# mobiusml/gemlite

Hardware: AMD Instinct MI355X
Metric: HBM GB/s (algorithmic bytes) vs roofline at M=1 [value], TFLOP/s vs bf16 MFMA roofline at M=256 [roofline.m256]; A16W4 gs=128 4096x4096 (higher is better)
Workload: dtype fp16; 1 GPU; A16W4 gs=128 4096x4096 M=1 fp16; step = 64 distinct layers (cache-cold rotation), hipGraph replay; replicas=1

## Files before the change

gemlite_amd/_hip.py:

```python
from __future__ import annotations

import ctypes as C
import os
import threading

import torch

_HERE = os.path.dirname(os.path.abspath(__file__))
LIB_PATH = os.path.join(_HERE, "csrc", "libgemlite_hip.so")
ABI_VERSION = 1

OK, ERR_BAD_ARGUMENT, ERR_UNSUPPORTED, ERR_BAD_SHAPE, ERR_WORKSPACE, ERR_LAUNCH, ERR_NO_DEVICE, ERR_NO_FUSED_QUANT = 0, -1, -2, -3, -4, -5, -6, -7


class ForwardArgs(C.Structure):

    _fields_ = [
        ("struct_size", C.c_uint32),
        ("matmul_type", C.c_int32),
        ("x", C.c_void_p),
        ("w_q", C.c_void_p),
        ("scales", C.c_void_p),
        ("zeros", C.c_void_p),
        ("scales_x", C.c_void_p),
        ("out", C.c_void_p),
        ("workspace", C.c_void_p),
        ("workspace_bytes", C.c_uint64),
        ("M", C.c_int64),
        ("N", C.c_int64),
        ("K", C.c_int64),
        ("W_nbits", C.c_int32),
        ("group_size", C.c_int32),
        ("unpack_mask", C.c_int32),
        ("elements_per_sample", C.c_int32),
        ("w_pack_bits", C.c_int32),
        ("w_dtype", C.c_int32),
        ("input_dtype", C.c_int32),
        ("output_dtype", C.c_int32),
        ("acc_dtype", C.c_int32),
        ("meta_dtype", C.c_int32),
        ("zeros_dtype", C.c_int32),
        ("channel_scale_mode", C.c_int32),
        ("W_group_mode", C.c_int32),
        ("zero_is_scalar", C.c_int32),
        ("data_contiguous", C.c_int32),
        ("type_id", C.c_int32),
        ("stride_xm", C.c_int64),
        ("stride_xk", C.c_int64),
        ("stride_wk", C.c_int64),
        ("stride_wn", C.c_int64),
        ("stride_om", C.c_int64),
        ("stride_on", C.c_int64),
        ("stride_meta_g", C.c_int64),
        ("stride_meta_n", C.c_int64),
        ("stride_sx_m", C.c_int64),
        ("tuning", C.c_int32 * 4),
    ]


class ForwardExt(C.Structure):

    _fields_ = [
        ("struct_size", C.c_uint32),
        ("bias_dtype", C.c_int32),
        ("bias", C.c_void_p),
    ]


class QuantizeArgs(C.Structure):

    _fields_ = [
        ("struct_size", C.c_uint32),
        ("w_dtype", C.c_int32),
        ("w", C.c_void_p),
        ("N", C.c_int64),
        ("K", C.c_int64),
        ("ld_w", C.c_int64),
        ("W_nbits", C.c_int32),
        ("group_size", C.c_int32),
        ("pack_bits", C.c_int32),
        ("meta_dtype", C.c_int32),
        ("q_out", C.c_void_p),
        ("ld_q", C.c_int64),
        ("scales", C.c_void_p),
        ("zeros", C.c_void_p),
        ("stride_meta_g", C.c_int64),
        ("stride_meta_n", C.c_int64),
        ("fold_zeros", C.c_int32),
        ("reserved", C.c_int32),
    ]


class QuantizeHqqArgs(C.Structure):

    _fields_ = [
        ("struct_size", C.c_uint32),
        ("iters", C.c_int32),
        ("q", QuantizeArgs),
        ("lp_norm", C.c_float),
        ("beta", C.c_float),
        ("kappa", C.c_float),
        ("reserved", C.c_int32),
    ]


class QuantizeMxArgs(C.Structure):

    _fields_ = [
        ("struct_size", C.c_uint32),
        ("w_dtype", C.c_int32),
        ("w", C.c_void_p),
        ("N", C.c_int64),
        ("K", C.c_int64),
        ("ld_w", C.c_int64),
        ("format", C.c_int32),
        ("pack_nibbles", C.c_int32),
        ("q_out", C.c_void_p),
        ("ld_q", C.c_int64),
        ("scales", C.c_void_p),
        ("stride_scale_g", C.c_int64),
        ("stride_scale_n", C.c_int64),
        ("reserved", C.c_int64),
    ]


class QuantizeRowsArgs(C.Structure):

    _fields_ = [
        ("struct_size", C.c_uint32),
        ("w_dtype", C.c_int32),
        ("w", C.c_void_p),
        ("N", C.c_int64),
        ("K", C.c_int64),
        ("ld_w", C.c_int64),
        ("format", C.c_int32),
        ("scale_rule", C.c_int32),
        ("q_out", C.c_void_p),
        ("ld_q", C.c_int64),
        ("scales", C.c_void_p),
        ("stride_s", C.c_int64),
        ("scale_dtype", C.c_int32),
        ("reserved", C.c_int32),
    ]


QUANT_ROWS_WAVE_MAX_K = 1024
QUANT_ROWS_RESIDENT_MAX_K = 16384


class DequantizeArgs(C.Structure):

    _fields_ = [
        ("struct_size", C.c_uint32),
        ("out_dtype", C.c_int32),
        ("w_q", C.c_void_p),
        ("scales", C.c_void_p),
        ("zeros", C.c_void_p),
        ("out", C.c_void_p),
        ("N", C.c_int64),
        ("K", C.c_int64),
        ("stride_wk", C.c_int64),
        ("stride_wn", C.c_int64),
        ("stride_meta_g", C.c_int64),
        ("stride_meta_n", C.c_int64),
        ("ld_out", C.c_int64),
        ("W_nbits", C.c_int32),
        ("group_size", C.c_int32),
        ("elements_per_sample", C.c_int32),
        ("w_pack_bits", C.c_int32),
        ("w_dtype", C.c_int32),
        ("input_dtype", C.c_int32),
        ("meta_dtype", C.c_int32),
        ("zeros_dtype", C.c_int32),
        ("zero_is_scalar", C.c_int32),
        ("W_group_mode", C.c_int32),
        ("channel_scale_mode", C.c_int32),
        ("post_scale", C.c_float),
        ("reserved", C.c_int64),
    ]


BIAS_NOT_ADDED = 1

_lib = None
_lib_lock = threading.Lock()


class GemliteHipError(RuntimeError):
    pass


def load():
    global _lib
    if _lib is not None:
        return _lib
    with _lib_lock:
        if _lib is not None:
            return _lib
        if not os.path.exists(LIB_PATH):
            raise GemliteHipError(
                f"{LIB_PATH} not found: build it with `python -c 'import __graft_entry__ as g; g.build()'` "
                "or `make -C gemlite_amd/csrc`.  gemlite_amd has no non-HIP fallback."
            )
        lib = C.CDLL(LIB_PATH)
        lib.gemlite_hip_abi_version.restype = C.c_int
        lib.gemlite_hip_build_info.restype = C.c_char_p
        lib.gemlite_hip_status_string.restype = C.c_char_p
        lib.gemlite_hip_status_string.argtypes = [C.c_int]
        lib.gemlite_hip_last_hip_error.restype = C.c_int
        for name in ("gemlite_hip_query", "gemlite_hip_forward"):
            getattr(lib, name).restype = C.c_int
        lib.gemlite_hip_query.argtypes = [C.POINTER(ForwardArgs)]
        lib.gemlite_hip_forward.argtypes = [C.POINTER(ForwardArgs), C.c_void_p]
        lib.gemlite_hip_workspace_bytes.restype = C.c_uint64
        lib.gemlite_hip_workspace_bytes.argtypes = [C.POINTER(ForwardArgs)]
        lib.gemlite_hip_kernel_name.restype = C.c_char_p
        lib.gemlite_hip_kernel_name.argtypes = [C.POINTER(ForwardArgs)]
        lib.gemlite_hip_set_profile_events.restype = None
        lib.gemlite_hip_set_profile_events.argtypes = [C.c_void_p, C.c_void_p]
        lib.gemlite_hip_launch_noop.restype = C.c_int
        lib.gemlite_hip_launch_noop.argtypes = [C.c_int32, C.c_int32, C.c_void_p]
        lib.gemlite_hip_capture_group_max.restype = C.c_int
        lib.gemlite_hip_capture_group_max.argtypes = []
        lib.gemlite_hip_capture_group_stats.restype = None
        lib.gemlite_hip_capture_group_stats.argtypes = [C.POINTER(C.c_uint64), C.POINTER(C.c_uint64)]
        lib.gemlite_hip_capture_group_compatible.restype = C.c_int
        lib.gemlite_hip_capture_group_compatible.argtypes = [C.POINTER(ForwardArgs), C.POINTER(ForwardArgs)]
        lib.gemlite_hip_capture_group_grid_y.restype = C.c_int
        lib.gemlite_hip_capture_group_grid_y.argtypes = [C.c_int32, C.c_int32]
        lib.gemlite_hip_capture_group_wave_split.restype = None
        lib.gemlite_hip_capture_group_wave_split.argtypes = [C.c_int32, C.c_int32, C.POINTER(C.c_int32 * 3)]
        lib.gemlite_hip_capture_group_last_form.restype = C.c_int
        lib.gemlite_hip_capture_group_last_form.argtypes = []
        lib.gemlite_hip_capture_group_geometry.restype = C.c_int
        lib.gemlite_hip_capture_group_geometry.argtypes = [C.c_int32, C.c_int32, C.c_int32, C.c_int32, C.c_int32, C.POINTER(C.c_int32 * 4)]
        lib.gemlite_hip_capture_group_tile_of.restype = C.c_int
        lib.gemlite_hip_capture_group_tile_of.argtypes = [C.c_int32, C.c_int32, C.c_int32, C.c_int32]
        lib.gemlite_hip_capture_group_form.restype = C.c_int
        lib.gemlite_hip_capture_group_form.argtypes = [C.c_int32, C.c_int32, C.c_int64]
        lib.gemlite_hip_capture_group_shared_x_lds_bytes.restype = C.c_int64
        lib.gemlite_hip_capture_group_shared_x_lds_bytes.argtypes = [C.c_int64]
        lib.gemlite_hip_forward_ex.restype = C.c_int
        lib.gemlite_hip_forward_ex.argtypes = [C.POINTER(ForwardArgs), C.POINTER(ForwardExt), C.c_void_p]
        lib.gemlite_hip_bias_fused.restype = C.c_int
        lib.gemlite_hip_bias_fused.argtypes = [C.POINTER(ForwardArgs), C.POINTER(ForwardExt)]
        lib.gemlite_hip_kernel_name_ex.restype = C.c_char_p
        lib.gemlite_hip_kernel_name_ex.argtypes = [C.POINTER(ForwardArgs), C.POINTER(ForwardExt)]
        lib.gemlite_hip_capture_group_compatible_ex.restype = C.c_int
        lib.gemlite_hip_capture_group_compatible_ex.argtypes = [C.POINTER(ForwardArgs), C.POINTER(ForwardExt), C.POINTER(ForwardArgs),
                                                                 C.POINTER(ForwardExt)]
        lib.gemlite_hip_scale_activations_per_token.restype = C.c_int
        lib.gemlite_hip_scale_activations_per_token.argtypes = [
            C.c_void_p, C.c_void_p, C.c_void_p, C.c_int64, C.c_int64, C.c_int64, C.c_int32, C.c_int32, C.c_void_p]
        for name in ("gemlite_hip_scale_activations_mxfp8", "gemlite_hip_scale_activations_mxfp4",
                     "gemlite_hip_scale_activations_nvfp4"):
            getattr(lib, name).restype = C.c_int
            getattr(lib, name).argtypes = [C.c_void_p, C.c_void_p, C.c_void_p, C.c_int64, C.c_int64, C.c_int64, C.c_int32,
                                           C.c_void_p]
        lib.gemlite_hip_pack_over_cols.restype = C.c_int
        lib.gemlite_hip_pack_over_cols.argtypes = [
            C.c_void_p, C.c_void_p, C.c_int64, C.c_int64, C.c_int64, C.c_int32, C.c_int32, C.c_void_p]
        lib.gemlite_hip_unpack_over_cols.restype = C.c_int
        lib.gemlite_hip_unpack_over_cols.argtypes = [
            C.c_void_p, C.c_void_p, C.c_int64, C.c_int64, C.c_int32, C.c_int32, C.c_void_p]
        lib.gemlite_hip_quantize_groups.restype = C.c_int
        lib.gemlite_hip_quantize_groups.argtypes = [C.POINTER(QuantizeArgs), C.c_void_p]
        lib.gemlite_hip_quantize_groups_hqq.restype = C.c_int
        lib.gemlite_hip_quantize_groups_hqq.argtypes = [C.POINTER(QuantizeHqqArgs), C.c_void_p]
        lib.gemlite_hip_quantize_mx.restype = C.c_int
        lib.gemlite_hip_quantize_mx.argtypes = [C.POINTER(QuantizeMxArgs), C.c_void_p]
        lib.gemlite_hip_quantize_rows.restype = C.c_int
        lib.gemlite_hip_quantize_rows.argtypes = [C.POINTER(QuantizeRowsArgs), C.c_void_p]
        lib.gemlite_hip_dequantize.restype = C.c_int
        lib.gemlite_hip_dequantize.argtypes = [C.POINTER(DequantizeArgs), C.c_void_p]
        if lib.gemlite_hip_abi_version() != ABI_VERSION:
            raise GemliteHipError("libgemlite_hip.so ABI version mismatch; rebuild it")
        _lib = lib
    return _lib


EXPORTED_SYMBOLS = (
    "gemlite_hip_abi_version", "gemlite_hip_build_info", "gemlite_hip_status_string", "gemlite_hip_last_hip_error",
    "gemlite_hip_query", "gemlite_hip_workspace_bytes", "gemlite_hip_forward", "gemlite_hip_kernel_name",
    "gemlite_hip_set_profile_events", "gemlite_hip_launch_noop", "gemlite_hip_scale_activations_per_token",
    "gemlite_hip_scale_activations_mxfp8", "gemlite_hip_scale_activations_mxfp4", "gemlite_hip_scale_activations_nvfp4",
    "gemlite_hip_pack_over_cols",
    "gemlite_hip_unpack_over_cols",
    "gemlite_hip_capture_group_max", "gemlite_hip_capture_group_stats", "gemlite_hip_capture_group_compatible",
    "gemlite_hip_capture_group_grid_y", "gemlite_hip_capture_group_wave_split",
    "gemlite_hip_capture_group_last_form", "gemlite_hip_capture_group_form", "gemlite_hip_capture_group_shared_x_lds_bytes",
    "gemlite_hip_capture_group_geometry", "gemlite_hip_capture_group_tile_of",
    "gemlite_hip_forward_ex", "gemlite_hip_bias_fused", "gemlite_hip_kernel_name_ex", "gemlite_hip_capture_group_compatible_ex",
    "gemlite_hip_quantize_groups", "gemlite_hip_quantize_mx", "gemlite_hip_dequantize", "gemlite_hip_quantize_groups_hqq",
    "gemlite_hip_quantize_rows",
)


def forward_ext(bias_ptr: int, bias_dtype: int) -> ForwardExt:
    e = ForwardExt()
    e.struct_size = C.sizeof(ForwardExt)
    e.bias_dtype = int(bias_dtype)
    e.bias = bias_ptr
    return e


def status_string(code: int) -> str:
    return load().gemlite_hip_status_string(int(code)).decode()


def raise_for_status(code: int, what: str):
    if code == OK:
        return
    msg = f"{what}: {status_string(code)}"
    if code == ERR_UNSUPPORTED or code == ERR_BAD_SHAPE:
        raise NotImplementedError(msg)
    if code == ERR_LAUNCH:
        msg += f" (hipError_t={load().gemlite_hip_last_hip_error()})"
    err = GemliteHipError(msg)
    err.status = code
    raise err


def require_gpu_tensor(t: torch.Tensor, name: str):
    if not t.is_cuda:
        raise GemliteHipError(
            f"gemlite_amd: `{name}` lives on {t.device}; the HIP backend only runs on an MI355X device "
            "(there is deliberately no CPU fallback)")


_workspaces: dict = {}
_ws_lock = threading.Lock()


def workspace(device: torch.device, stream_handle: int, nbytes: int) -> torch.Tensor:
    key = (device.index if device.index is not None else torch.cuda.current_device(), int(stream_handle))
    ws = _workspaces.get(key)
    if ws is None or ws.numel() < nbytes:
        with _ws_lock:
            ws = _workspaces.get(key)
            if ws is None or ws.numel() < nbytes:
                size = max(int(nbytes), 1 << 20)
                size = 1 << (size - 1).bit_length()
                ws = torch.zeros(size, dtype=torch.uint8, device=device)
                _workspaces[key] = ws
    return ws


class on_device:
    __slots__ = ("_guard",)

    def __init__(self, device: torch.device):
        idx = device.index
        self._guard = torch.cuda.device(idx) if (idx is not None and idx != torch.cuda.current_device()) else None

    def __enter__(self):
        if self._guard is not None:
            self._guard.__enter__()
        return self

    def __exit__(self, *exc):
        if self._guard is not None:
            self._guard.__exit__(*exc)
        return False


def current_stream_handle(device: torch.device) -> int:
    return torch.cuda.current_stream(device).cuda_stream
```

gemlite_amd/csrc/api.hip:

```cpp
#include <hip/hip_runtime.h>
#include <stdio.h>
#include <string.h>

#include <atomic>
#include <mutex>
#include <set>
#include <string>

#include "gl_common.h"
#include "gl_coopquant.h"

namespace gl {
bool plan_gemv_wn(const gemlite_hip_forward_args& a, WnParams& p, LaunchPlan& lp);
bool plan_gemv_mfma(const gemlite_hip_forward_args& a, WnParams& p, LaunchPlan& lp);
bool plan_gemv_a8wn(const gemlite_hip_forward_args& a, WnParams& p, LaunchPlan& lp, bool fq = false);
bool plan_a8wn_rows(const gemlite_hip_forward_args& a, WnParams& p, LaunchPlan& lp);
bool plan_gemm_wn_stream(const gemlite_hip_forward_args& a, WnParams& p, LaunchPlan& lp);
bool plan_gemm_wn_direct(const gemlite_hip_forward_args& a, WnParams& p, LaunchPlan& lp);
bool plan_gemm_wn_rows(const gemlite_hip_forward_args& a, WnParams& p, LaunchPlan& lp);
bool plan_gemm_a8w8(const gemlite_hip_forward_args& a, LaunchPlan& lp);
bool plan_gemm_a8w8_mma(const gemlite_hip_forward_args& a, GenericParams& g, LaunchPlan& lp);
bool plan_a8w8_rows(const gemlite_hip_forward_args& a, LaunchPlan& lp, bool fq = false);
bool plan_a16w8_rows(const gemlite_hip_forward_args& a, LaunchPlan& lp);
bool a16w8_rows_lds_pays(const gemlite_hip_forward_args& a);
bool plan_gemm_a8w8_sq(const gemlite_hip_forward_args& a, GenericParams& g, LaunchPlan& lp);
bool plan_gemm_a8w8_sq128(const gemlite_hip_forward_args& a, GenericParams& g, LaunchPlan& lp);
bool plan_gemm_wn_tiled(const gemlite_hip_forward_args& a, WnParams& p, LaunchPlan& lp);
bool plan_gemm_wn_mma(const gemlite_hip_forward_args& a, WnParams& p, LaunchPlan& lp);
bool plan_gemm_mx_mma(const gemlite_hip_forward_args& a, GenericParams& g, LaunchPlan& lp);
bool plan_gemm_mx_sq(const gemlite_hip_forward_args& a, GenericParams& g, LaunchPlan& lp);
bool plan_gemm_wn_mma_mx(const gemlite_hip_forward_args& a, WnParams& p, LaunchPlan& lp, int mode = 0);
bool plan_mx_gemv(const gemlite_hip_forward_args& a, GenericParams& g, LaunchPlan& lp);
bool plan_gemm_mx_tile(const gemlite_hip_forward_args& a, GenericParams& g, LaunchPlan& lp);
const void* mx_generic_kernel_fn();
const void* act_quant_mx_kernel_fn(int mode);
bool plan_mx_rows(const gemlite_hip_forward_args& a, GenericParams& g, LaunchPlan& lp, bool any_m = false, bool fq = false);
bool plan_nvfp4_rows(const gemlite_hip_forward_args& a, GenericParams& g, LaunchPlan& lp, bool fq = false);
const void* nvfp4_expand_f16_kernel_fn();
const void* generic_kernel_fn();
const void* kmajor_kernel_fn(int mb);
const void* kmajor_w8a16_kernel_fn(int mb);
const void* kmajor_fused_quant_kernel_fn(int qdt);
const void* a8w8_decode_kernel_fn(int qdt, bool fused);
const void* a16w8_decode_kernel_fn(int x_dt, int w_dt);
const void* act_quant_kernel_fn();
const void* act_quant_vec_kernel_fn(int in_dt, int out_dt, int64_t K, int64_t stride_xm, const void* x, const void* y);
const void* pack_kernel_fn();
const void* pack32_kernel_fn();
const void* unpack_kernel_fn();
const void* quantize_groups_kernel_fn(bool onepass);
const void* quantize_hqq_kernel_fn(bool onepass);
const void* quantize_mx_kernel_fn(int format);
const void* quantize_rows_kernel_fn(int format, int64_t K);
const void* dequantize_words_kernel_fn(int nbits);
const void* dequantize_rows_kernel_fn(int fmt);
const void* dequantize_any_kernel_fn();
int capture_group_limit();
void capture_group_stats(uint64_t* seen, uint64_t* joined);
bool capture_group_compatible(const gemlite_hip_forward_args& a, const LaunchPlan& la, const gemlite_hip_forward_args& b, const LaunchPlan& lb);
bool capture_group_try_join(const gemlite_hip_forward_args& a, const LaunchPlan& lp, hipStream_t st, int resident, int dev);
bool capture_group_shared_x_enabled();
int capture_group_last_form();
Decode3TilesWanted capture_group_tiles_wanted(int tiles, int members, int resident);
int ensure_lds(const void* fn, size_t lds, int dev);
void capture_group_note_launch(const gemlite_hip_forward_args& a, const LaunchPlan& lp, hipStream_t st);

}

using namespace gl;

const char* gl::pw_label(const char* name, int pack_bits) {
    if (pack_bits == 32) return name;
    static std::mutex mu;
    static std::set<std::string>* names = new std::set<std::string>();
    std::string s(name);
    s.insert(s.size() - 1, pack_bits == 8 ? ",b8" : ",b16");
    std::lock_guard<std::mutex> lock(mu);
    return names->insert(s).first->c_str();
}

const char* gl::bias_label(const char* name) {
    static std::mutex mu;
    static std::set<std::string>* names = new std::set<std::string>();
    std::string s(name);
    s.insert(s.size() - 1, ",bias");
    std::lock_guard<std::mutex> lock(mu);
    return names->insert(s).first->c_str();
}

static thread_local int tl_last_hip_error = 0;
static thread_local void* tl_evt_start = nullptr;
static thread_local void* tl_evt_stop = nullptr;

static int dtype_size(int dt) {
    switch (dt) {
        case GEMLITE_DT_FP32: case GEMLITE_DT_INT32: case GEMLITE_DT_UINT32: return 4;
        case GEMLITE_DT_FP16: case GEMLITE_DT_BF16: case GEMLITE_DT_INT16: case GEMLITE_DT_UINT16: return 2;
        case GEMLITE_DT_INT64: return 8;
        case GEMLITE_DT_FP8E4: case GEMLITE_DT_FP8E5: case GEMLITE_DT_INT8: case GEMLITE_DT_UINT8: return 1;
        default: return 0;
    }
}

enum Kind { K_NONE = 0, K_GEMV_WN, K_STREAM_WN, K_TILED_WN, K_KMAJOR, K_A8_MMA, K_A8_FQ, K_NV_MMA, K_GENERIC };

struct Resolved {
    Kind kind = K_NONE;
    LaunchPlan lp{};
    WnParams wn{};
    GenericParams gp{};
    int status = GEMLITE_OK;
    uint64_t nv_x16_bytes = 0;
};

static Epilogue make_epilogue(const gemlite_hip_forward_args& a) {
    Epilogue e{};
    e.out = a.out;
    e.scales_w = a.scales;
    e.scales_x = (const float*)a.scales_x;
    e.stride_om = a.stride_om;
    e.stride_on = a.stride_on;
    e.stride_sx_m = a.stride_sx_m;
    e.out_dt = a.output_dtype;
    e.meta_dt = a.meta_dtype;
    e.c_mode = a.channel_scale_mode;
    return e;
}

static bool is_mx_input(int dt);
static bool wants_fused_quant(const gemlite_hip_forward_args* a) {
    if (is_mx_input(a->type_id / 100)) return false;
    return a->M >= 1 && a->elements_per_sample == 1 && !a->scales_x &&
           (a->channel_scale_mode == 2 || a->channel_scale_mode == 3) && a->W_group_mode == 0 &&
           (a->input_dtype == GEMLITE_DT_FP16 || a->input_dtype == GEMLITE_DT_BF16) &&
           (a->w_dtype == GEMLITE_DT_INT8 || a->w_dtype == GEMLITE_DT_FP8E4 || a->w_dtype == GEMLITE_DT_FP8E5);
}

static int fused_quant_packed_dtype(const gemlite_hip_forward_args* a) {
    if (a->M != 1 || a->elements_per_sample <= 1 || a->scales_x) return 0;
    if (!(a->channel_scale_mode == 2 || a->channel_scale_mode == 3)) return 0;
    if (!(a->input_dtype == GEMLITE_DT_FP16 || a->input_dtype == GEMLITE_DT_BF16)) return 0;
    const int layer_dt = a->type_id / 100;
    return (layer_dt == GEMLITE_DT_FP8E4 || layer_dt == GEMLITE_DT_INT8) && a->type_id % 100 == a->W_nbits ? layer_dt : 0;
}

static bool is_mx_input(int dt);
static int fused_quant_mx_dtype(const gemlite_hip_forward_args* a) {
    if (a->M != 1 || a->scales_x || !(a->channel_scale_mode == 4 || a->channel_scale_mode == 2)) return 0;
    if (!(a->input_dtype == GEMLITE_DT_FP16 || a->input_dtype == GEMLITE_DT_BF16)) return 0;
    const int layer_dt = a->type_id / 100;
    if (a->channel_scale_mode == 2 && layer_dt != GEMLITE_DT_MXFP8) return 0;
    return (layer_dt == GEMLITE_DT_MXFP8 || layer_dt == GEMLITE_DT_MXFP4 || layer_dt == GEMLITE_DT_NVFP4) && a->type_id % 100 == a->W_nbits ? layer_dt : 0;
}

static bool is_mx_input(int dt) { return dt >= GEMLITE_DT_MXFP16 && dt <= GEMLITE_DT_NVFP4; }

static int validate_mx(const gemlite_hip_forward_args* a) {
    const bool nv = a->input_dtype == GEMLITE_DT_NVFP4;
    if (a->group_size != (nv ? 16 : 32)) return GEMLITE_ERR_UNSUPPORTED;
    if (a->K % 32 != 0) return GEMLITE_ERR_BAD_SHAPE;
    if (!a->scales) return GEMLITE_ERR_BAD_ARGUMENT;
    if (!(a->output_dtype == GEMLITE_DT_FP32 || a->output_dtype == GEMLITE_DT_FP16 || a->output_dtype == GEMLITE_DT_BF16))
        return GEMLITE_ERR_UNSUPPORTED;
    const bool w8 = a->W_nbits == 8 && a->elements_per_sample == 1 && a->w_dtype == GEMLITE_DT_FP8E4;
    const bool w4 = a->W_nbits == 4 && a->elements_per_sample == 2 && a->w_pack_bits == 8;
    if (!w8 && !w4) return GEMLITE_ERR_UNSUPPORTED;
    const bool x16 = a->input_dtype == GEMLITE_DT_MXFP16 || a->input_dtype == GEMLITE_DT_MXBF16;
    if ((a->input_dtype == GEMLITE_DT_MXFP4 || nv) && !w4) return GEMLITE_ERR_UNSUPPORTED;
    if (x16 ? a->channel_scale_mode != 0 : !(a->channel_scale_mode == 4 || (a->channel_scale_mode == 2 && !nv))) return GEMLITE_ERR_UNSUPPORTED;
    if (!x16 && !a->scales_x) return GEMLITE_ERR_BAD_ARGUMENT;
    if (a->stride_xk != 1) return GEMLITE_ERR_UNSUPPORTED;
    if (a->M > 65535 && a->M > 0x7FFFFFFF) return GEMLITE_ERR_BAD_SHAPE;
    return GEMLITE_OK;
}

static int validate(const gemlite_hip_forward_args* a) {
    if (!a || a->struct_size != sizeof(gemlite_hip_forward_args)) return GEMLITE_ERR_BAD_ARGUMENT;
    if (!a->x || !a->w_q || !a->out) return GEMLITE_ERR_BAD_ARGUMENT;
    if (a->M <= 0 || a->N <= 0 || a->K <= 0) return GEMLITE_ERR_BAD_ARGUMENT;
    if (a->M > 0x7FFFFFFF || a->N > 0x7FFFFFFF || a->K > 0x7FFFFFFF) return GEMLITE_ERR_BAD_SHAPE;
    if (is_mx_input(a->input_dtype)) return validate_mx(a);
    if (const int mxdt = fused_quant_mx_dtype(a)) {
        gemlite_hip_forward_args b = *a;
        b.input_dtype = mxdt;
        b.scales_x = (const void*)(uintptr_t)0x1000;
        return validate_mx(&b);
    }
    if (a->W_group_mode < 0 || a->W_group_mode > 4) return GEMLITE_ERR_UNSUPPORTED;
    if (a->channel_scale_mode < 0 || a->channel_scale_mode > 3) return GEMLITE_ERR_UNSUPPORTED;
    if (a->elements_per_sample < 1) return GEMLITE_ERR_BAD_ARGUMENT;
    if (a->K % a->elements_per_sample != 0) return GEMLITE_ERR_BAD_SHAPE;
    if (a->input_dtype == GEMLITE_DT_FP8E4NUZ || a->input_dtype == GEMLITE_DT_FP8E5NUZ) return GEMLITE_ERR_UNSUPPORTED;
    if (a->input_dtype > GEMLITE_DT_FP8E5NUZ) return GEMLITE_ERR_UNSUPPORTED;
    if (dtype_size(a->input_dtype) == 0) return GEMLITE_ERR_UNSUPPORTED;
    if (!(a->output_dtype == GEMLITE_DT_FP32 || a->output_dtype == GEMLITE_DT_FP16 || a->output_dtype == GEMLITE_DT_BF16))
        return GEMLITE_ERR_UNSUPPORTED;
    const bool need_s = a->W_group_mode >= 2 || a->channel_scale_mode == 1 || a->channel_scale_mode == 3;
    const bool need_z = a->W_group_mode == 1 || a->W_group_mode >= 3;
    if (need_s && !a->scales) return GEMLITE_ERR_BAD_ARGUMENT;
    if (need_z && !a->zeros) return GEMLITE_ERR_BAD_ARGUMENT;
    if ((a->channel_scale_mode == 2 || a->channel_scale_mode == 3) && !a->scales_x && !wants_fused_quant(a) && !fused_quant_packed_dtype(a)) return GEMLITE_ERR_BAD_ARGUMENT;
    if (a->elements_per_sample > 1) {
        if (a->w_pack_bits != 8 && a->w_pack_bits != 16 && a->w_pack_bits != 32 && a->w_pack_bits != 64)
            return GEMLITE_ERR_BAD_ARGUMENT;
        if (a->W_nbits * a->elements_per_sample != a->w_pack_bits) return GEMLITE_ERR_BAD_ARGUMENT;
    } else if (dtype_size(a->w_dtype) == 0) {
        return GEMLITE_ERR_UNSUPPORTED;
    }
    const bool grouped = a->W_group_mode >= 2 || (need_z && !a->zero_is_scalar);
    if (grouped && a->group_size <= 0) return GEMLITE_ERR_BAD_SHAPE;
    if (a->input_dtype == GEMLITE_DT_INT8 && a->W_group_mode >= 2) return GEMLITE_ERR_UNSUPPORTED;
    return GEMLITE_OK;
}

static GenericParams mx_params(const gemlite_hip_forward_args& a);
static void resolve_mx_plan(const gemlite_hip_forward_args& a, Resolved& r, const GenericParams& g);
static void resolve_mx(const gemlite_hip_forward_args& a, Resolved& r) {
    GenericParams g = mx_params(a);
    r.gp = g;
    resolve_mx_plan(a, r, g);
}
static GenericParams mx_params(const gemlite_hip_forward_args& a) {
    GenericParams g{};
    g.x = a.x; g.w = a.w_q; g.scales = a.scales; g.zeros = nullptr;
    g.epi = make_epilogue(a);
    if (a.channel_scale_mode == 4) g.epi.c_mode = 0;
    g.M = (int)a.M; g.N = (int)a.N; g.K = (int)a.K;
    g.nbits = a.W_nbits; g.e = a.elements_per_sample; g.pack_bits = a.w_pack_bits;
    g.w_dt = a.w_dtype; g.x_dt = a.input_dtype;
    g.group_size = a.group_size;
    g.stride_xm = a.stride_xm; g.stride_xk = a.stride_xk; g.stride_wk = a.stride_wk; g.stride_wn = a.stride_wn;
    g.stride_meta_g = a.stride_meta_g; g.stride_meta_n = a.stride_meta_n;
    g.mx_x = a.input_dtype == GEMLITE_DT_MXFP16 ? MX_F16 : (a.input_dtype == GEMLITE_DT_MXBF16 ? MX_BF16 : (a.input_dtype == GEMLITE_DT_MXFP8 ? MX_FP8 : MX_FP4));
    g.mx_w = a.W_nbits == 8 ? MX_FP8 : MX_FP4;
    g.mx_scale_e4m3 = a.input_dtype == GEMLITE_DT_NVFP4 ? 1 : 0;
    g.sx_blocks = a.channel_scale_mode == 4 ? a.scales_x : nullptr;
    g.stride_sx_blk_m = a.stride_sx_m;
    g.mx_post = a.input_dtype == GEMLITE_DT_NVFP4 ? 0.0025f : 1.0f;
    g.splitk = 1;
    return g;
}
static void resolve_mx_plan(const gemlite_hip_forward_args& a, Resolved& r, const GenericParams& g) {
    if ((a.tuning[0] == 4 || (a.tuning[0] == 0 && a.tuning[1] == 0 && a.tuning[2] == 0)) && plan_mx_rows(a, r.gp, r.lp)) { r.kind = K_KMAJOR; return; }
    const bool mx16 = a.input_dtype == GEMLITE_DT_MXFP16 || a.input_dtype == GEMLITE_DT_MXBF16;
    const bool a16_over = mx16 && a.M >= 2 && a.M <= 64 && a.N % 128 == 0 && a.K % 128 == 0 &&
                          (int64_t)a.M * a.N * a.K > ((int64_t)a.N * a.K <= (32ll << 20) ? 570000000ll : 250000000ll);
    if (mx16 && a.M <= 64 && (a.tuning[0] == 4 || (a.tuning[0] == 0 && a.tuning[1] == 0 && a.tuning[2] == 0 && !a16_over)) &&
        plan_a16w8_rows(a, r.lp)) { r.kind = K_KMAJOR; return; }
    const bool sq_few = a.M >= 2 && a.M <= 64 && ((g.mx_x == MX_FP4 && g.mx_w == MX_FP4) || a.N / 64 >= 128);
    const bool mx_w4 = g.mx_w == MX_FP4;
    const int64_t sq_tiles = (a.N / 64) * ((a.M + 63) / 64);
    const int64_t sq_slots = (sq_tiles + 511) / 512 * 512;
    bool slices_fill = false;
    for (int64_t sk = 1, t128 = (a.N / 128) * ((a.M + 127) / 128), cus = gl::resident_block_limit(); sk <= 3 && sk * 1024 <= a.K && !slices_fill; ++sk) {
        const int64_t rounds = (t128 * sk + cus - 1) / cus;
        slices_fill = rounds <= 2 && t128 * sk * 10 >= rounds * cus * 9;
    }
    const bool long_k_slices = a.M > 128 && a.K > 8192 && a.N % 128 == 0 && sq_tiles > 256 && sq_tiles <= 720 && sq_tiles * 10 < sq_slots * 7 && slices_fill &&
                               (!mx_w4 || ((int64_t)a.N * a.K > (1ll << 26) && g.mx_x == MX_FP8));
    const bool sq_auto = sq_few || (a.M > 64 && !long_k_slices && (a.M <= 512 || (a.M <= 1024 && (!mx_w4 || (int64_t)a.N * a.K <= (1ll << 24)))));
    if ((a.tuning[0] == 6 || (a.tuning[0] == 0 && a.tuning[1] == 0 && a.tuning[2] == 0 && sq_auto)) && plan_gemm_mx_sq(a, r.gp, r.lp)) { r.kind = K_A8_MMA; return; }
    if ((a.tuning[0] == 5 || (a.tuning[0] == 0 && !a16_over)) && a.tuning[1] == 0 && a.tuning[2] == 0 && plan_mx_gemv(a, r.gp, r.lp)) { r.kind = K_KMAJOR; return; }
    if (plan_gemm_mx_tile(a, r.gp, r.lp)) { r.kind = K_A8_MMA; return; }
    if ((a.tuning[0] == 0 || a.tuning[0] == 2) && plan_gemm_mx_mma(a, r.gp, r.lp)) { r.kind = K_A8_MMA; return; }
    if ((a.tuning[0] == 0 || a.tuning[0] == 2) && (a.input_dtype == GEMLITE_DT_MXFP16 || a.input_dtype == GEMLITE_DT_MXBF16)) {
        WnParams p{};
        p.x = a.x; p.w = (const uint32_t*)a.w_q; p.scales = a.scales; p.zeros = nullptr;
        p.epi = g.epi;
        p.epi.meta_dt = p.epi.out_dt;
        p.M = (int)a.M; p.N = (int)a.N; p.K = (int)a.K;
        p.group_size = 32;
        p.stride_xm = a.stride_xm; p.stride_xk = a.stride_xk; p.stride_wk = 1;
        p.flags = caller_flags(a);
        if (plan_gemm_wn_mma_mx(a, p, r.lp)) { r.kind = K_TILED_WN; r.wn = p; return; }
    }
    if (a.tuning[0] == 0 && plan_mx_rows(a, r.gp, r.lp, true)) { r.kind = K_KMAJOR; return; }
    if ((a.tuning[0] == 0 || a.tuning[0] == 4) && a.tuning[1] == 0 && a.tuning[2] == 0 && plan_nvfp4_rows(a, r.gp, r.lp)) { r.kind = K_KMAJOR; return; }
    if (a.input_dtype == GEMLITE_DT_NVFP4 && a.channel_scale_mode == 4 && (a.tuning[0] == 0 || a.tuning[0] == 2) &&
        ((uintptr_t)a.x % 8) == 0 && a.stride_xm % 8 == 0 && a.K % 128 == 0 && (int64_t)a.M * a.K < (1ll << 30)) {
        gemlite_hip_forward_args b = a;
        b.input_dtype = GEMLITE_DT_MXFP16;
        b.x = (const void*)(uintptr_t)0x1000;
        b.stride_xm = a.K;
        WnParams p{};
        p.x = nullptr; p.w = (const uint32_t*)a.w_q; p.scales = a.scales; p.zeros = nullptr;
        p.epi = g.epi;
        p.epi.c_mode = 2;
        p.epi.scales_x = nullptr;
        p.epi.stride_sx_m = 1;
        p.epi.meta_dt = p.epi.out_dt;
        p.M = (int)a.M; p.N = (int)a.N; p.K = (int)a.K;
        p.group_size = 16;
        p.stride_xm = a.K; p.stride_xk = 1; p.stride_wk = 1;
        p.flags = caller_flags(a);
        if (plan_gemm_wn_mma_mx(b, p, r.lp, 1)) {
            r.kind = K_NV_MMA;
            r.wn = p;
            r.nv_x16_bytes = (uint64_t)(((int64_t)a.M * a.K * 2 + 255) & ~(int64_t)255);
            r.lp.ws_bytes = COUNTER_BYTES + r.lp.slab_bytes + r.nv_x16_bytes + (uint64_t)((a.M * 4 + 255) & ~(int64_t)255);
            return;
        }
    }
    if (a.tuning[0] == 0 && a.tuning[1] == 0 && a.tuning[2] == 0) {
        gemlite_hip_forward_args f = a;
        f.tuning[0] = 4;
        if (a16_over && plan_a16w8_rows(f, r.lp)) { r.kind = K_KMAJOR; return; }
        if (a.input_dtype == GEMLITE_DT_NVFP4 && plan_nvfp4_rows(f, r.gp, r.lp)) { r.kind = K_KMAJOR; return; }
    }
    if (a.M > 65535) { r.status = GEMLITE_ERR_BAD_SHAPE; return; }
    r.kind = K_GENERIC;
    r.lp.fn = mx_generic_kernel_fn();
    r.lp.name = "mx_generic_kernel";
    r.lp.grid = dim3((unsigned)((a.N + 255) / 256), (unsigned)a.M, 1);
    r.lp.block = dim3(256, 1, 1);
}

static bool a8w8_sq_pays(const gemlite_hip_forward_args& a) {
    if (a.N % 64 != 0) return false;
    if (a.M <= 64) return a.M >= 2 && a.N / 64 >= 128 && a.N / 64 <= 512;
    const int64_t tiles = (a.N / 64) * ((a.M + 63) / 64);
    if (a.K >= 14336 && a.M <= 128 && tiles <= 128 && a.N % 128 == 0) return false;
    return tiles <= 256 || (tiles <= 512 && a.K <= 8192);
}

static bool rows5_narrow_layer_pays(int64_t M, int64_t tiles, int64_t K) {
    if (tiles < 64) return false;
    if (K <= 4096) return M >= (K <= 2048 ? 4 : 8);
    return M >= (tiles >= 128 ? 16 : 17) && M <= 32;
}
static bool rows5_pays_w2(int64_t M, int64_t N, int64_t K, int gs_shift) {
    if (M < 2 || M > 64 || N % 16 != 0 || K % 512 != 0 || K > 16384) return false;
    const int64_t tiles = N / 16;
    if (tiles > gl::resident_block_limit()) return false;
    const bool g64_two_tiles = gs_shift == 6 && M >= 17 && M <= 32;
    if (tiles < 192 && !(g64_two_tiles && tiles >= 32) && !rows5_narrow_layer_pays(M, tiles, K)) return false;
    if (gs_shift == 6 && M > 32) return false;
    if (gs_shift < 6) return false;
    if (M < (K <= 2048 ? 8 : 2)) return false;
    const int64_t bytes = tiles * ((M + 15) / 16 * 16) * K * 2;
    return bytes <= (192ll << 20) || (M <= 32 && bytes <= (256ll << 20));
}
static bool rows5_pays(int64_t M, int64_t N, int64_t K, int gs_shift) {
    if (M < 2 || M > 64 || N % 16 != 0 || K > 12288) return false;
    const int64_t tiles = N / 16, resident = gl::resident_block_limit();
    if (tiles > resident) {
        if (N % 32 != 0 || tiles / 2 > resident || gs_shift < 6) return false;
        if (K <= 2048 ? M < 8 : (M < 17 || M > 32)) return false;
        if (gs_shift == 6 && (K > 4096 || M > 32)) return false;
        return (tiles / 2) * ((M + 15) / 16 * 16) * K * 2 <= (176ll << 20);
    }
    const bool g64_two_tiles = gs_shift == 6 && M >= 17 && M <= 32;
    if (tiles < 192 && !(g64_two_tiles && tiles >= 32) && !rows5_narrow_layer_pays(M, tiles, K)) return false;
    const int64_t min_m = (K > 2048 && K <= 4096) ? 8 : 2;
    if (M < min_m) return false;
    return tiles * ((M + 15) / 16 * 16) * K * 2 <= (176ll << 20);
}

static bool a8w8_sq128_pays(const gemlite_hip_forward_args& a) {
    if (a.M <= 64 || a.N % 128 != 0) return false;
    const int64_t tiles = (a.N / 128) * ((a.M + 127) / 128);
    if (a.K < 4096) return tiles >= 136 && tiles <= gl::resident_block_limit() && (a.N / 64) * ((a.M + 63) / 64) > 512;
    return tiles >= 144 && tiles <= gl::resident_block_limit();
}

static void resolve(const gemlite_hip_forward_args& a, Resolved& r) {
    r.status = validate(&a);
    if (r.status != GEMLITE_OK) return;
    if (is_mx_input(a.input_dtype)) { resolve_mx(a, r); return; }
    if (const int mxdt = fused_quant_mx_dtype(&a)) {
        r.status = GEMLITE_ERR_NO_FUSED_QUANT;
        if (a.tuning[0] != 0 || a.tuning[1] != 0 || a.tuning[2] != 0 || a.matmul_type != GEMLITE_MATMUL_AUTO) return;
        if (a.stride_xk != 1 || ((uintptr_t)a.x % 16) != 0) return;
        gemlite_hip_forward_args b = a;
        b.input_dtype = mxdt;
        b.x = (const void*)(uintptr_t)0x1000;
        b.scales_x = (const void*)(uintptr_t)0x1000;
        b.stride_xm = mxdt == GEMLITE_DT_MXFP8 ? a.K : a.K / 2;
        b.stride_sx_m = mxdt == GEMLITE_DT_NVFP4 ? a.K / 16 : a.K / 32;
        GenericParams g = mx_params(b);
        LaunchPlan lp{};
        if (!(mxdt == GEMLITE_DT_NVFP4 ? plan_nvfp4_rows(b, g, lp, true) : plan_mx_rows(b, g, lp, false, true))) return;
        g.x = a.x;
        g.x_dt = a.input_dtype;
        g.sx_blocks = a.channel_scale_mode == 4 ? a.x : nullptr;
        r.status = GEMLITE_OK;
        r.kind = K_KMAJOR; r.gp = g; r.lp = lp;
        return;
    }
    const bool packed = a.elements_per_sample > 1;
    const bool x16 = a.input_dtype == GEMLITE_DT_FP16 || a.input_dtype == GEMLITE_DT_BF16;
    const bool per_group_meta = a.W_group_mode >= 2 || ((a.W_group_mode == 1) && !a.zero_is_scalar &&
                                                        !(a.channel_scale_mode == 1 || a.channel_scale_mode == 3));
    const int eff_group = per_group_meta ? a.group_size : (int)a.K;

    if (const int qdt = fused_quant_packed_dtype(&a)) {
        r.status = GEMLITE_ERR_NO_FUSED_QUANT;
        if (a.tuning[0] != 0 || a.tuning[1] != 0 || a.tuning[2] != 0 || a.matmul_type != GEMLITE_MATMUL_AUTO) return;
        if (a.stride_xk != 1 || ((uintptr_t)a.x % 16) != 0 || a.output_dtype != a.input_dtype || a.w_pack_bits != 32 || a.stride_wn != 1 || a.stride_on != 1) return;
        const bool pgm = a.W_group_mode >= 2 || ((a.W_group_mode == 1) && !a.zero_is_scalar);
        const int eg = pgm ? a.group_size : (int)a.K;
        if (eg <= 0 || a.K % eg != 0 || (a.stride_meta_n != 1 && pgm)) return;
        gemlite_hip_forward_args b = a;
        b.input_dtype = qdt;
        b.x = (const void*)(uintptr_t)0x1000;
        b.scales_x = (const void*)(uintptr_t)0x1000;
        b.stride_xm = a.K;
        WnParams p{};
        p.x = a.x; p.w = (const uint32_t*)a.w_q; p.scales = a.scales; p.zeros = a.zeros;
        p.epi = make_epilogue(a);
        p.M = 1; p.N = (int)a.N; p.K = (int)a.K;
        p.group_size = eg;
        p.w_mode = a.W_group_mode;
        p.meta_dt = a.meta_dtype; p.zeros_dt = a.zeros_dtype; p.zero_is_scalar = a.zero_is_scalar;
        p.stride_xm = a.K; p.stride_xk = 1; p.stride_wk = a.stride_wk;
        p.stride_meta_g = (pgm && eg < a.K) ? a.stride_meta_g : 0;
        p.flags = caller_flags(a);
        p.gs_shift = eg >= a.K ? 31 : ((eg & (eg - 1)) == 0 ? __builtin_ctz((unsigned)eg) : -1);
        LaunchPlan lp{};
        if (p.gs_shift < 0 || !plan_gemv_a8wn(b, p, lp, true)) return;
        r.status = GEMLITE_OK;
        r.kind = K_GEMV_WN; r.wn = p; r.lp = lp;
        return;
    }
    const bool x8 = a.input_dtype == GEMLITE_DT_FP8E4 || a.input_dtype == GEMLITE_DT_INT8;
    if (packed && (a.w_pack_bits == 32 || a.w_pack_bits == 16 || a.w_pack_bits == 8) && (x16 || x8) && a.stride_wn == 1 && a.stride_xk == 1 && a.stride_on == 1 &&
        (a.stride_meta_n == 1 || !per_group_meta) && (a.K % eff_group == 0)) {
        WnParams p{};
        p.x = a.x; p.w = (const uint32_t*)a.w_q; p.scales = a.scales; p.zeros = a.zeros;
        p.epi = make_epilogue(a);
        p.M = (int)a.M; p.N = (int)a.N; p.K = (int)a.K;
        p.group_size = eff_group;
        p.w_mode = a.W_group_mode;
        p.meta_dt = a.meta_dtype; p.zeros_dt = a.zeros_dtype; p.zero_is_scalar = a.zero_is_scalar;
        p.stride_xm = a.stride_xm; p.stride_xk = a.stride_xk; p.stride_wk = a.stride_wk;
        p.stride_meta_g = (per_group_meta && eff_group < a.K) ? a.stride_meta_g : 0;
        p.flags = caller_flags(a);
        p.gs_shift = eff_group >= a.K ? 31
                     : ((eff_group > 0 && (eff_group & (eff_group - 1)) == 0) ? __builtin_ctz((unsigned)eff_group) : -1);
        const int mt = a.matmul_type;
        const bool want_gemv = (mt == GEMLITE_MATMUL_GEMV || mt == GEMLITE_MATMUL_GEMV_REVSPLITK ||
                                mt == GEMLITE_MATMUL_GEMV_SPLITK || (mt == GEMLITE_MATMUL_AUTO && a.M <= 1));
        LaunchPlan lp{};
        if (p.gs_shift < 0) {
            if (eff_group % 32 == 0 && eff_group > 32 && a.K % eff_group == 0 && (int64_t)a.K * eff_group < (1ll << 40) &&
                a.tuning[0] == 0 && (mt == GEMLITE_MATMUL_AUTO || mt == GEMLITE_MATMUL_GEMM || mt == GEMLITE_MATMUL_GEMM_SPLITK)) {
                const uint32_t d = (uint32_t)(eff_group / 32);
                p.gs_magic = (uint32_t)(((1ull << 32) + d - 1) / d);
                if (want_gemv && a.tuning[1] == 0 && a.tuning[2] == 0 && plan_gemv_wn(a, p, lp)) { r.kind = K_GEMV_WN; r.wn = p; r.lp = lp; return; }
                if (plan_gemm_wn_mma(a, p, lp)) { r.kind = K_TILED_WN; r.wn = p; r.lp = lp; return; }
            }
            goto coverage;
        }
        if (x8 && (want_gemv || mt == GEMLITE_MATMUL_AUTO) && a.tuning[1] == 0 && a.tuning[2] == 0 &&
            (a.tuning[0] == 4 || (a.tuning[0] == 0 && a.M >= 2)) && plan_a8wn_rows(a, p, lp)) {
            r.kind = K_GEMV_WN; r.wn = p; r.lp = lp; return;
        }
        if (x8 && a.M <= (a.tuning[0] == 7 ? 4 : 1) && (want_gemv || mt == GEMLITE_MATMUL_AUTO) && (a.tuning[0] == 0 || a.tuning[0] == 7) && a.tuning[1] == 0 && a.tuning[2] == 0 &&
            plan_gemv_a8wn(a, p, lp)) {
            r.kind = K_GEMV_WN; r.wn = p; r.lp = lp; return;
        }
        if (x16 && (a.W_nbits == 4 || a.W_nbits == 2) && (mt == GEMLITE_MATMUL_AUTO || mt == GEMLITE_MATMUL_GEMM_SPLITK || (mt == GEMLITE_MATMUL_GEMM && a.tuning[0] == 9)) &&
            !(caller_flags(a) & GEMLITE_TF_NO_ROWS_KERNEL) && (a.tuning[0] == 9 || (a.tuning[0] == 0 && a.tuning[1] == 0 && a.tuning[2] == 0 && a.M >= 2))) {
            const bool g32_tiles = p.gs_shift == 5 && a.N % 128 == 0 && a.K % 256 == 0 &&
                                   (a.M > 32 || (a.M > 16 && a.K >= 2048 && a.N / 16 > gl::resident_block_limit()));
            const bool only_here = (p.gs_shift == 5 && !g32_tiles) || a.N % 64 != 0;
            const bool in_budget = a.W_nbits == 4 ? rows5_pays(a.M, a.N, a.K, p.gs_shift) : rows5_pays_w2(a.M, a.N, a.K, p.gs_shift);
            bool tiles_take = false;
            if (g32_tiles) {
                WnParams pt = p;
                LaunchPlan lt{};
                tiles_take = plan_gemm_wn_mma(a, pt, lt);
            }
            if (a.tuning[0] == 9 || only_here || (in_budget && !g32_tiles) || (g32_tiles && !tiles_take)) {
                WnParams pr = p;
                LaunchPlan lr{};
                if (plan_gemm_wn_rows(a, pr, lr)) { r.kind = K_STREAM_WN; r.wn = pr; r.lp = lr; return; }
            }
        }
        if (x16 && a.W_nbits == 4 && a.M >= 2 && a.M <= 4 && mt == GEMLITE_MATMUL_AUTO && a.tuning[0] == 0 && a.tuning[1] == 0 && a.tuning[2] == 0 &&
            !(caller_flags(a) & GEMLITE_TF_FORCE_MFMA_GEMV) && a.K >= 12288 && a.N <= 8192 && a.N % 64 == 0 && a.N / 64 >= 40) {
            gemlite_hip_forward_args a2 = a;
            a2.tuning[0] = 4;
            a2.tuning[1] = a.N / 64 >= 128 ? 2 : 4;
            WnParams pd = p;
            LaunchPlan ld{};
            if (plan_gemm_wn_direct(a2, pd, ld)) { r.kind = K_STREAM_WN; r.wn = pd; r.lp = ld; return; }
        }
        if (x16 && !(caller_flags(a) & GEMLITE_TF_NO_MFMA_GEMV) && a.tuning[1] == 0 &&
            ((want_gemv && a.M == 1 && mt != GEMLITE_MATMUL_GEMV_SPLITK) || (a.M >= 2 && a.M <= 4 && mt == GEMLITE_MATMUL_AUTO))) {
            WnParams pm = p;
            LaunchPlan lm{};
            if (plan_gemv_mfma(a, pm, lm)) {
                const int cols = (int)(a.N / lm.grid.x);
                (void)cols;
                const bool wins = a.M >= 2 ? (a.W_nbits != 4 || a.N < 12288) : (a.W_nbits == 2 && a.K % 1024 != 0);
                if ((caller_flags(a) & GEMLITE_TF_FORCE_MFMA_GEMV) || a.tuning[0] != 0 || wins) { r.kind = K_GEMV_WN; r.wn = pm; r.lp = lm; return; }
            }
        }
        if (want_gemv && plan_gemv_wn(a, p, lp)) { r.kind = K_GEMV_WN; r.wn = p; r.lp = lp; return; }
        if (!want_gemv) {
            const bool want_tiled = (mt == GEMLITE_MATMUL_GEMM || (mt == GEMLITE_MATMUL_AUTO && a.M > 32));
            if (want_tiled && a.tuning[0] == 0 && plan_gemm_wn_mma(a, p, lp)) { r.kind = K_TILED_WN; r.wn = p; r.lp = lp; return; }
            if (want_tiled && a.tuning[0] != 1 && plan_gemm_wn_tiled(a, p, lp)) { r.kind = K_TILED_WN; r.wn = p; r.lp = lp; return; }
            const bool long_k = mt == GEMLITE_MATMUL_AUTO && a.W_nbits == 4 && a.tuning[0] == 0 && a.tuning[2] == 0 &&
                                a.M > 16 && a.K >= 8192;
            if (long_k && plan_gemm_wn_mma(a, p, lp)) { r.kind = K_TILED_WN; r.wn = p; r.lp = lp; return; }
            if (a.M <= 32 && a.tuning[2] != 1 && a.tuning[0] != 3 && plan_gemm_wn_direct(a, p, lp)) { r.kind = K_STREAM_WN; r.wn = p; r.lp = lp; return; }
            if (mt == GEMLITE_MATMUL_AUTO && a.M > 16 && a.K >= 2048 && a.tuning[0] == 0 && a.tuning[1] == 0 && a.tuning[2] == 0 && !(caller_flags(a) & GEMLITE_TF_NO_ROWS_KERNEL) &&
                plan_gemm_wn_mma(a, p, lp)) { r.kind = K_TILED_WN; r.wn = p; r.lp = lp; return; }
            if (a.tuning[0] != 3 && plan_gemm_wn_stream(a, p, lp)) { r.kind = K_STREAM_WN; r.wn = p; r.lp = lp; return; }
            if (plan_gemm_wn_mma(a, p, lp)) { r.kind = K_TILED_WN; r.wn = p; r.lp = lp; return; }
        }
        if (want_gemv && mt == GEMLITE_MATMUL_AUTO && plan_gemm_wn_stream(a, p, lp)) {
            r.kind = K_STREAM_WN; r.wn = p; r.lp = lp; return;
        }
        if (want_gemv && plan_gemm_wn_mma(a, p, lp)) { r.kind = K_TILED_WN; r.wn = p; r.lp = lp; return; }
    }

coverage:
    GenericParams g{};
    g.x = a.x; g.w = a.w_q; g.scales = a.scales; g.zeros = a.zeros;
    g.epi = make_epilogue(a);
    g.M = (int)a.M; g.N = (int)a.N; g.K = (int)a.K;
    g.nbits = a.W_nbits; g.e = a.elements_per_sample; g.pack_bits = a.w_pack_bits;
    g.w_dt = a.w_dtype; g.x_dt = a.input_dtype;
    g.group_size = eff_group; g.w_mode = a.W_group_mode;
    g.meta_dt = a.meta_dtype; g.zeros_dt = a.zeros_dtype; g.zero_is_scalar = a.zero_is_scalar;
    g.int_acc = (a.input_dtype == GEMLITE_DT_INT8 && (packed || a.w_dtype == GEMLITE_DT_INT8)) ? 1 : 0;
    g.stride_xm = a.stride_xm; g.stride_xk = a.stride_xk; g.stride_wk = a.stride_wk; g.stride_wn = a.stride_wn;
    g.stride_meta_g = per_group_meta ? a.stride_meta_g : 0;
    g.stride_meta_n = per_group_meta ? a.stride_meta_n : ((a.W_group_mode == 1 && !a.zero_is_scalar) ? 1 : 0);
    r.gp = g;
    if (wants_fused_quant(&a) && a.M >= 2) {
        r.status = GEMLITE_ERR_NO_FUSED_QUANT;
        if (a.tuning[0] != 0 || a.tuning[1] != 0 || a.tuning[2] != 0 || a.matmul_type != GEMLITE_MATMUL_AUTO) return;
        if (a.M > cq::MAX_ROWS || a.stride_xk != 1 || a.K % 16 != 0 || a.stride_xm % 8 != 0 || ((uintptr_t)a.x % 16) != 0) return;
        gemlite_hip_forward_args b = a;
        b.input_dtype = a.w_dtype;
        b.x = (const void*)(uintptr_t)0x1000;
        b.scales_x = (const void*)(uintptr_t)0x1000;
        b.stride_xm = a.K;
        b.stride_sx_m = 1;
        LaunchPlan lp{};
        GenericParams gq = g;
        if (a.M > 64 || !plan_a8w8_rows(b, lp, true)) return;
        gq.x = nullptr; gq.x_dt = a.w_dtype; gq.stride_xm = a.K; gq.stride_xk = 1;
        gq.int_acc = a.w_dtype == GEMLITE_DT_INT8 ? 1 : 0;
        gq.epi.scales_x = nullptr; gq.epi.stride_sx_m = 1;
        gq.cq_x = a.x; gq.cq_stride_xm = a.stride_xm; gq.cq_xdt = a.input_dtype;
        gq.flags = caller_flags(a);
        r.status = GEMLITE_OK;
        r.kind = K_A8_FQ;
        r.gp = gq;
        r.lp = lp;
        return;
    }
    if (wants_fused_quant(&a)) {
        if (a.stride_wk != 1 || a.stride_xk != 1 || a.K % 16 != 0 || a.stride_wn % 16 != 0 || a.K > 65536 ||
            (((uintptr_t)a.w_q | (uintptr_t)a.x) % 16) != 0) { r.status = GEMLITE_ERR_NO_FUSED_QUANT; return; }
        r.kind = K_KMAJOR;
        const bool dec_ok = a.tuning[0] != 7 && a.K % 1024 == 0 && a.N % 16 == 0 && (a.w_dtype == GEMLITE_DT_INT8 || a.N <= 4096 || a.tuning[0] == 8);
        if (dec_ok && a.stride_on == 1 && a.K <= 61440) {
            r.lp.fn = a8w8_decode_kernel_fn(a.w_dtype, true);
            r.lp.name = "a8w8_decode_fused_quant_kernel<tile16,16w>";
            r.lp.grid = dim3((unsigned)(a.N / 16), 1, 1);
            r.lp.block = dim3(1024, 1, 1);
            r.lp.lds_bytes = (size_t)a.K + 64;
            return;
        }
        r.lp.fn = kmajor_fused_quant_kernel_fn(a.w_dtype);
        r.lp.name = "kmajor_fused_quant_kernel";
        r.lp.grid = dim3((unsigned)((a.N + 7) / 8), 1, 1);
        r.lp.block = dim3(512, 1, 1);
        r.lp.lds_bytes = (size_t)((a.K + 15) & ~15) + 64;
        return;
    }
    if (!packed && (a.tuning[0] == 4 || (a.tuning[0] == 0 && a.tuning[1] == 0 && a.tuning[2] == 0 && a.M >= 2)) &&
        a.matmul_type != GEMLITE_MATMUL_GEMV && a.matmul_type != GEMLITE_MATMUL_GEMV_SPLITK &&
        a.matmul_type != GEMLITE_MATMUL_GEMV_REVSPLITK && plan_a8w8_rows(a, r.lp)) {
        r.kind = K_KMAJOR;
        return;
    }
    if (!packed && a.matmul_type != GEMLITE_MATMUL_GEMV && a.matmul_type != GEMLITE_MATMUL_GEMV_SPLITK &&
        a.matmul_type != GEMLITE_MATMUL_GEMV_REVSPLITK &&
        (a.tuning[0] == 10 || (a.tuning[0] == 0 && a.tuning[1] == 0 && a.tuning[2] == 0 && !(caller_flags(a) & GEMLITE_TF_A8W8_WEIGHTS_FROM_MEMORY) && a8w8_sq128_pays(a))) && plan_gemm_a8w8_sq128(a, r.gp, r.lp)) {
        r.kind = K_A8_MMA;
        return;
    }
    if (!packed && a.matmul_type != GEMLITE_MATMUL_GEMV && a.matmul_type != GEMLITE_MATMUL_GEMV_SPLITK &&
        a.matmul_type != GEMLITE_MATMUL_GEMV_REVSPLITK &&
        (a.tuning[0] == 5 || (a.tuning[0] == 0 && a.tuning[1] == 0 && a.tuning[2] == 0 && !(caller_flags(a) & GEMLITE_TF_A8W8_WEIGHTS_FROM_MEMORY) && a8w8_sq_pays(a))) && plan_gemm_a8w8_sq(a, r.gp, r.lp)) {
        r.kind = K_A8_MMA;
        return;
    }
    if (!packed && (a.tuning[0] == 0 || a.tuning[0] == 6) && a.matmul_type != GEMLITE_MATMUL_GEMV && a.matmul_type != GEMLITE_MATMUL_GEMV_SPLITK &&
        a.matmul_type != GEMLITE_MATMUL_GEMV_REVSPLITK && plan_gemm_a8w8_mma(a, r.gp, r.lp)) {
        r.kind = K_A8_MMA;
        return;
    }
    if (!packed && a.tuning[0] != 1 && a.matmul_type != GEMLITE_MATMUL_GEMV && a.matmul_type != GEMLITE_MATMUL_GEMV_SPLITK &&
        a.matmul_type != GEMLITE_MATMUL_GEMV_REVSPLITK && plan_gemm_a8w8(a, r.lp)) {
        r.kind = K_KMAJOR;
        return;
    }
    if (!packed && (a.W_group_mode == 0 || (a.W_group_mode == 2 && eff_group >= a.K && a.scales)) && a.stride_wk == 1 &&
        a.stride_xk == 1 && (a.input_dtype == GEMLITE_DT_FP16 || a.input_dtype == GEMLITE_DT_BF16) &&
        (a.w_dtype == GEMLITE_DT_INT8 || a.w_dtype == GEMLITE_DT_FP8E4 || a.w_dtype == GEMLITE_DT_FP8E5) &&
        a.K % 16 == 0 && a.stride_wn % 16 == 0 && (a.stride_xm * 2) % 16 == 0 && (((uintptr_t)a.w_q | (uintptr_t)a.x) % 16 == 0)) {
        r.kind = K_KMAJOR;
        if (a.M == 1 && a.tuning[0] == 0 && a.K % 1024 == 0 && a.K <= 30720 && a.N % 16 == 0) {
            r.lp.fn = a16w8_decode_kernel_fn(a.input_dtype, a.w_dtype);
            r.lp.name = "a16w8_decode_kernel<tile16,16w>";
            r.lp.grid = dim3((unsigned)(a.N / 16), 1, 1);
            r.lp.block = dim3(1024, 1, 1);
            r.lp.lds_bytes = (size_t)a.K * 2;
            return;
        }
        if (a.tuning[0] == 0 && a16w8_rows_lds_pays(a) && plan_a16w8_rows(a, r.lp)) return;
        if ((a.tuning[0] == 2 || ((a.M > 64 || (a.M >= 2 && (int64_t)a.M * a.N * a.K > 850000000ll)) && a.tuning[0] == 0)) &&
            !(a.W_group_mode == 2 && a.channel_scale_mode != 0)) {
            WnParams p{};
            p.x = a.x; p.w = (const uint32_t*)a.w_q; p.scales = a.scales; p.zeros = nullptr;
            p.epi = make_epilogue(a);
            if (a.W_group_mode == 2) { p.epi.c_mode = 1; p.epi.scales_w = a.scales; }
            p.M = (int)a.M; p.N = (int)a.N; p.K = (int)a.K;
            p.group_size = 32;
            p.stride_xm = a.stride_xm; p.stride_xk = a.stride_xk; p.stride_wk = 1;
            p.flags = caller_flags(a);
            if (plan_gemm_wn_mma_mx(a, p, r.lp, 2)) { r.kind = K_TILED_WN; r.wn = p; return; }
        }
        if (a.tuning[0] != 7 && plan_a16w8_rows(a, r.lp)) return;
        const int mb = a.M == 1 ? 1 : 4;
        r.lp.fn = kmajor_w8a16_kernel_fn(mb);
        r.lp.name = "kmajor_w8a16_kernel";
        r.lp.grid = dim3((unsigned)((a.N + 3) / 4), (unsigned)((a.M + mb - 1) / mb), 1);
        r.lp.block = dim3(256, 1, 1);
        return;
    }
    const int esz = dtype_size(a.w_dtype);
    if (!packed && a.W_group_mode == 0 && a.stride_wk == 1 && a.stride_xk == 1 && a.w_dtype == a.input_dtype &&
        esz > 0 && (a.K % (16 / esz) == 0) && ((a.stride_wn * esz) % 16 == 0) && ((a.stride_xm * esz) % 16 == 0) &&
        (((uintptr_t)a.w_q | (uintptr_t)a.x) % 16 == 0) &&
        !(a.M > 1 && (a.w_dtype == GEMLITE_DT_FP8E4 || a.w_dtype == GEMLITE_DT_FP8E5))) {
        const int mb = a.M == 1 ? 1 : 4;
        r.kind = K_KMAJOR;
        if (a.M == 1 && esz == 1 && a.tuning[0] != 7 && a.K % 1024 == 0 && a.N % 16 == 0 &&
            (a.w_dtype == GEMLITE_DT_INT8 || ((a.w_dtype == GEMLITE_DT_FP8E4 || a.w_dtype == GEMLITE_DT_FP8E5) && (a.N <= 4096 || a.tuning[0] == 8)))) {
            r.lp.fn = a8w8_decode_kernel_fn(a.w_dtype, false);
            r.lp.name = "a8w8_decode_kernel<tile16,16w>";
            r.lp.grid = dim3((unsigned)(a.N / 16), 1, 1);
            r.lp.block = dim3(1024, 1, 1);
            return;
        }
        r.lp.fn = kmajor_kernel_fn(mb);
        r.lp.name = "kmajor_matmul_kernel";
        r.lp.grid = dim3((unsigned)((a.N + 3) / 4), (unsigned)((a.M + mb - 1) / mb), 1);
        r.lp.block = dim3(256, 1, 1);
        return;
    }
    if (a.M > 65535) { r.status = GEMLITE_ERR_BAD_SHAPE; return; }
    r.kind = K_GENERIC;
    r.lp.fn = generic_kernel_fn();
    r.lp.name = "generic_matmul_kernel";
    r.lp.grid = dim3((unsigned)((a.N + 255) / 256), (unsigned)a.M, 1);
    r.lp.block = dim3(256, 1, 1);
}

static int launch(const void* fn, dim3 grid, dim3 block, void** kargs, size_t lds, hipStream_t stream) {
    hipError_t err;
    if (tl_evt_start || tl_evt_stop) {
        err = hipExtLaunchKernel(fn, grid, block, kargs, lds, stream, (hipEvent_t)tl_evt_start, (hipEvent_t)tl_evt_stop, 0);
        tl_evt_start = tl_evt_stop = nullptr;
    } else {
        err = hipLaunchKernel(fn, grid, block, kargs, lds, stream);
    }
    if (err != hipSuccess) {
        tl_last_hip_error = (int)err;
        (void)hipGetLastError();
        return GEMLITE_ERR_LAUNCH;
    }
    return GEMLITE_OK;
}

static std::atomic<int> g_cu_by_dev[64];
static thread_local int tl_plan_dev = -1;
int gl::resident_block_limit() {
    if (tl_plan_dev < 0) return 256;
    const int n = g_cu_by_dev[tl_plan_dev & 63].load(std::memory_order_relaxed);
    return n > 0 ? n : 256;
}

static int check_device(int* dev_out) {
    int dev = -1;
    if (hipGetDevice(&dev) != hipSuccess || dev < 0) { (void)hipGetLastError(); return GEMLITE_ERR_NO_DEVICE; }
    *dev_out = dev;
    static std::atomic<int> state[64];
    const int slot = dev & 63;
    int st = state[slot].load(std::memory_order_relaxed);
    if (st == 0) {
        hipDeviceProp_t prop;
        st = (hipGetDeviceProperties(&prop, dev) == hipSuccess && strncmp(prop.gcnArchName, "gfx950", 6) == 0) ? 1 : 2;
        if (st == 1 && prop.multiProcessorCount > 0) g_cu_by_dev[slot].store(prop.multiProcessorCount, std::memory_order_relaxed);
        state[slot].store(st, std::memory_order_relaxed);
    }
    return st == 1 ? GEMLITE_OK : GEMLITE_ERR_NO_DEVICE;
}

int gl::ensure_lds(const void* fn, size_t lds, int dev) {
    if (lds <= 65536) return GEMLITE_OK;
    struct Done { const void* fn; int dev; };
    static thread_local Done done[32] = {};
    for (const Done& d : done) if (d.fn == fn && d.dev == dev) return GEMLITE_OK;
    hipError_t err = hipFuncSetAttribute(fn, hipFuncAttributeMaxDynamicSharedMemorySize, (int)lds);
    if (err != hipSuccess) { tl_last_hip_error = (int)err; (void)hipGetLastError(); return GEMLITE_ERR_LAUNCH; }
    static thread_local int next = 0;
    done[next] = Done{fn, dev};
    next = (next + 1) & 31;
    return GEMLITE_OK;
}

__global__ void gemlite_noop_kernel() {}

static int validate_ext(const gemlite_hip_forward_ext* e) {
    if (e && e->struct_size != sizeof(gemlite_hip_forward_ext)) return GEMLITE_ERR_BAD_ARGUMENT;
    return GEMLITE_OK;
}

static bool apply_bias(const gemlite_hip_forward_args& a, const gemlite_hip_forward_ext* e, Resolved& r) {
    if (!e || !e->bias || r.status != GEMLITE_OK) return false;
    LaunchPlan& lp = r.lp;
    if ((lp.arg_kind != 1 && lp.arg_kind != 2) || !lp.fn_bias || lp.fn != lp.bias_of) return false;
    if (e->bias_dtype != a.output_dtype || (a.output_dtype != GEMLITE_DT_FP16 && a.output_dtype != GEMLITE_DT_BF16)) return false;
    if (((uintptr_t)e->bias & 1u) != 0) return false;
    if (lp.arg_kind == 1 && (lp.d3.modes & 64u)) return false;
    lp.fn = lp.fn_bias;
    lp.name = bias_label(lp.name);
    lp.bias = (const uint16_t*)e->bias;
    return true;
}

extern "C" {

int gemlite_hip_abi_version(void) { return GEMLITE_HIP_ABI_VERSION; }

const char* gemlite_hip_build_info(void) {
    return "libgemlite_hip gfx950 (CDNA4) abi=1 kernels: gemv_wn, gemv_decode, gemv_mfma, gemv_a8wn, gemm_wn_rows, gemm_wn_direct, gemm_wn_stream, gemm_wn_mma, gemm_wn_tiled, gemm_a8w8, "
           "gemm_mx, mx_rows, nvfp4_f16, kmajor, generic, act_quant_per_token, act_quant_mx, pack/unpack_over_cols, quantize_groups, quantize_mx, dequantize, quantize_hqq, quantize_rows"
#ifdef GL_AB_KERNELS
           " +ab_kernels"
#endif
        ;
}

const char* gemlite_hip_status_string(int status) {
    switch (status) {
        case GEMLITE_OK: return "ok";
        case GEMLITE_ERR_BAD_ARGUMENT: return "bad argument (null pointer, non-positive size or ABI struct_size mismatch)";
        case GEMLITE_ERR_UNSUPPORTED: return "unsupported dtype / bit-width / mode combination";
        case GEMLITE_ERR_BAD_SHAPE: return "bad shape (K not divisible by elements_per_sample / group_size, or too large)";
        case GEMLITE_ERR_WORKSPACE: return "workspace missing or too small";
        case GEMLITE_ERR_LAUNCH: return "HIP launch failed (see gemlite_hip_last_hip_error)";
        case GEMLITE_ERR_NO_DEVICE: return "current device is not gfx950";
        case GEMLITE_ERR_NO_FUSED_QUANT: return "no kernel with in-launch activation quantisation for this shape: quantise x first and pass scales_x";
        default: return "unknown status";
    }
}

int gemlite_hip_last_hip_error(void) { return tl_last_hip_error; }

int gemlite_hip_query(const gemlite_hip_forward_args* args) {
    const int v = validate(args);
    if (v != GEMLITE_OK) return v;
    Resolved r;
    resolve(*args, r);
    return r.status;
}

uint64_t gemlite_hip_workspace_bytes(const gemlite_hip_forward_args* args) {
    if (validate(args) != GEMLITE_OK) return 0;
    Resolved r;
    resolve(*args, r);
    return r.status == GEMLITE_OK ? r.lp.ws_bytes : 0;
}

const char* gemlite_hip_kernel_name(const gemlite_hip_forward_args* args) {
    if (validate(args) != GEMLITE_OK) return "invalid";
    Resolved r;
    resolve(*args, r);
    return r.status == GEMLITE_OK ? r.lp.name : "unsupported";
}

void gemlite_hip_set_profile_events(void* start_event, void* stop_event) {
    tl_evt_start = start_event;
    tl_evt_stop = stop_event;
}

int gemlite_hip_capture_group_max(void) { return capture_group_limit(); }

void gemlite_hip_capture_group_stats(uint64_t* seen, uint64_t* joined) { capture_group_stats(seen, joined); }

int gemlite_hip_capture_group_grid_y(int32_t tiles, int32_t members) {
    return (tiles > 0 && members > 0) ? decode3_group_grid_y(tiles, members, 256) : 0;
}

void gemlite_hip_capture_group_wave_split(int32_t layers_in_block, int32_t wave, int32_t out[3]) {
    if (!out) return;
    Decode3WaveSplit s{-1, 0, 0};
    if (layers_in_block >= 1 && layers_in_block <= DECODE3_GMAX && wave >= 0 && wave < 16) s = decode3_wave_split(layers_in_block, wave);
    out[0] = s.layer; out[1] = s.v0; out[2] = s.v1;
}

int gemlite_hip_capture_group_last_form(void) { return capture_group_last_form(); }

int gemlite_hip_capture_group_geometry(int32_t tiles, int32_t members, int32_t resident, int32_t tb_want, int32_t span_want, int32_t out[4]) {
    if (!out || tiles < 1 || members < 1 || members > DECODE3_GMAX || resident < 1 || tb_want < 0 || tb_want > 4 || tb_want == 3) return -1;
    Decode3TilesWanted want{tb_want, span_want != 0};
    if (tb_want == 0) want = capture_group_tiles_wanted(tiles, members, resident);
    const Decode3GroupGeometry geo = decode3_group_geometry(tiles, members, resident, want.tb, want.span);
    out[0] = geo.tb; out[1] = geo.grid_x; out[2] = geo.grid_y; out[3] = geo.span ? 1 : 0;
    return 0;
}

int gemlite_hip_capture_group_tile_of(int32_t tiles, int32_t tb, int32_t span, int32_t block) {
    if (tiles < 1 || (tb != 1 && tb != 2 && tb != 4) || tiles % tb || block < 0 || block >= tiles / tb) return -1;
    return decode3_group_first_tile(block, tiles / tb, tb, span != 0, (tiles & 15) == 0);
}

int gemlite_hip_capture_group_form(int32_t members, int32_t same_x, int64_t K) {
    if (members < 1 || members > DECODE3_GMAX || K <= 0 || (K & 255)) return -1;
    return decode3_group_form(members, same_x != 0, K / 256, capture_group_shared_x_enabled());
}

int64_t gemlite_hip_capture_group_shared_x_lds_bytes(int64_t K) {
    return (K > 0 && !(K & 255)) ? decode3_shared_x_lds_bytes(K / 256) : 0;
}

int gemlite_hip_capture_group_compatible(const gemlite_hip_forward_args* a, const gemlite_hip_forward_args* b) {
    if (validate(a) != GEMLITE_OK || validate(b) != GEMLITE_OK) return 0;
    Resolved ra, rb;
    resolve(*a, ra);
    resolve(*b, rb);
    if (ra.status != GEMLITE_OK || rb.status != GEMLITE_OK) return 0;
    return capture_group_compatible(*a, ra.lp, *b, rb.lp) ? 1 : 0;
}

int gemlite_hip_bias_fused(const gemlite_hip_forward_args* args, const gemlite_hip_forward_ext* ext) {
    const int v = validate(args);
    if (v != GEMLITE_OK) return v;
    if (validate_ext(ext) != GEMLITE_OK) return GEMLITE_ERR_BAD_ARGUMENT;
    Resolved r;
    resolve(*args, r);
    if (r.status != GEMLITE_OK) return r.status;
    return apply_bias(*args, ext, r) ? 1 : 0;
}

const char* gemlite_hip_kernel_name_ex(const gemlite_hip_forward_args* args, const gemlite_hip_forward_ext* ext) {
    if (validate(args) != GEMLITE_OK || validate_ext(ext) != GEMLITE_OK) return "invalid";
    Resolved r;
    resolve(*args, r);
    (void)apply_bias(*args, ext, r);
    return r.status == GEMLITE_OK ? r.lp.name : "unsupported";
}

int gemlite_hip_capture_group_compatible_ex(const gemlite_hip_forward_args* a, const gemlite_hip_forward_ext* ea,
                                             const gemlite_hip_forward_args* b, const gemlite_hip_forward_ext* eb) {
    if (validate(a) != GEMLITE_OK || validate(b) != GEMLITE_OK || validate_ext(ea) != GEMLITE_OK || validate_ext(eb) != GEMLITE_OK) return 0;
    Resolved ra, rb;
    resolve(*a, ra);
    resolve(*b, rb);
    if (ra.status != GEMLITE_OK || rb.status != GEMLITE_OK) return 0;
    (void)apply_bias(*a, ea, ra);
    (void)apply_bias(*b, eb, rb);
    return capture_group_compatible(*a, ra.lp, *b, rb.lp) ? 1 : 0;
}

int gemlite_hip_launch_noop(int32_t blocks, int32_t threads, void* stream) {
    if (blocks <= 0 || threads <= 0 || threads > 1024) return GEMLITE_ERR_BAD_ARGUMENT;
    void* none[1] = {nullptr};
    return launch((const void*)gemlite_noop_kernel, dim3((unsigned)blocks, 1, 1), dim3((unsigned)threads, 1, 1), none, 0,
                  (hipStream_t)stream);
}

static int launch_resolved(const gemlite_hip_forward_args* args, Resolved& r, int dev, int resident, hipStream_t st);

int gemlite_hip_forward(const gemlite_hip_forward_args* args, void* stream) { return gemlite_hip_forward_ex(args, nullptr, stream); }

int gemlite_hip_forward_ex(const gemlite_hip_forward_args* args, const gemlite_hip_forward_ext* ext, void* stream) {
    const int v = validate(args);
    if (v != GEMLITE_OK) return v;
    if (validate_ext(ext) != GEMLITE_OK) return GEMLITE_ERR_BAD_ARGUMENT;
    int dev = 0;
    const int dv = check_device(&dev);
    Resolved r;
    tl_plan_dev = dv == GEMLITE_OK ? dev : -1;
    resolve(*args, r);
    const int resident = gl::resident_block_limit();
    tl_plan_dev = -1;
    if (r.status != GEMLITE_OK) return r.status;
    if (dv != GEMLITE_OK) return dv;
    const bool bias_left = ext && ext->bias && !apply_bias(*args, ext, r);
    const int rc = launch_resolved(args, r, dev, resident, (hipStream_t)stream);
    return (rc == GEMLITE_OK && bias_left) ? GEMLITE_BIAS_NOT_ADDED : rc;
}

static int launch_resolved(const gemlite_hip_forward_args* args, Resolved& r, int dev, int resident, hipStream_t st) {
    if (r.kind == K_GEMV_WN || r.kind == K_STREAM_WN || r.kind == K_TILED_WN) {
        if (r.lp.ws_bytes > 0) {
            if (!args->workspace || args->workspace_bytes < r.lp.ws_bytes) return GEMLITE_ERR_WORKSPACE;
            r.wn.counters = (unsigned*)args->workspace;
            r.wn.slabs = (float*)((char*)args->workspace + COUNTER_BYTES);
        } else if (args->workspace && args->workspace_bytes >= COUNTER_BYTES) {
            r.wn.counters = (unsigned*)args->workspace;
        }
        const int e = ensure_lds(r.lp.fn, r.lp.lds_bytes, dev);
        if (e != GEMLITE_OK) return e;
        if (r.lp.arg_kind == 1) {
            Decode3Args& d = r.lp.d3;
            d.counters = r.wn.counters;
            Decode3BiasTail btail{r.lp.bias};
            void* dargs[] = {(void*)&d.w, (void*)&d.x, (void*)&d.s, (void*)&d.z, (void*)&d.out, (void*)&d.sw4, (void*)&d.mstride2,
                             (void*)&d.nch_total, (void*)&d.modes, r.lp.bias ? (void*)&btail : (void*)&d.counters};
            const bool plain = tl_evt_start || tl_evt_stop;
            if (!plain && capture_group_try_join(*args, r.lp, st, resident, dev)) return GEMLITE_OK;
            const int rc = launch(r.lp.fn, r.lp.grid, r.lp.block, dargs, 0, st);
            if (!plain && rc == GEMLITE_OK) capture_group_note_launch(*args, r.lp, st);
            return rc;
        }
        if (r.lp.arg_kind == 2) {
            Rows5Args& d = r.lp.r5;
            void* dargs[] = {(void*)&d.w, (void*)&d.x, (void*)&d.s, (void*)&d.z, (void*)&d.out, (void*)&d.sw4, (void*)&d.mstride2,
                             (void*)&d.nch_total, (void*)&d.modes, (void*)&d.M, (void*)&d.sxm2, (void*)&d.som, (void*)&r.lp.bias};
            const bool plain = tl_evt_start || tl_evt_stop;
            if (!plain && capture_group_try_join(*args, r.lp, st, resident, dev)) return GEMLITE_OK;
            const int rc = launch(r.lp.fn, r.lp.grid, r.lp.block, dargs, r.lp.lds_bytes, st);
            if (!plain && rc == GEMLITE_OK) capture_group_note_launch(*args, r.lp, st);
            return rc;
        }
        void* kargs[] = {(void*)&r.wn};
        return launch(r.lp.fn, r.lp.grid, r.lp.block, kargs, r.lp.lds_bytes, st);
    }
    if (r.kind == K_A8_MMA) {
        if (r.lp.ws_bytes > 0) {
            if (!args->workspace || args->workspace_bytes < r.lp.ws_bytes) return GEMLITE_ERR_WORKSPACE;
            r.gp.counters = (unsigned*)args->workspace;
            r.gp.slabs = (float*)((char*)args->workspace + COUNTER_BYTES);
        }
        const int e = ensure_lds(r.lp.fn, r.lp.lds_bytes, dev);
        if (e != GEMLITE_OK) return e;
        void* kargs[] = {(void*)&r.gp};
        return launch(r.lp.fn, r.lp.grid, r.lp.block, kargs, r.lp.lds_bytes, st);
    }
    if (r.kind == K_NV_MMA) {
        if (!args->workspace || args->workspace_bytes < r.lp.ws_bytes) return GEMLITE_ERR_WORKSPACE;
        char* base = (char*)args->workspace;
        uint16_t* x16 = (uint16_t*)(base + COUNTER_BYTES + r.lp.slab_bytes);
        float* post = (float*)((char*)x16 + r.nv_x16_bytes);
        r.wn.counters = (unsigned*)base;
        r.wn.slabs = (float*)(base + COUNTER_BYTES);
        r.wn.x = x16;
        r.wn.epi.scales_x = post;
        const uint8_t* xq = (const uint8_t*)args->x;
        const uint8_t* sx = (const uint8_t*)args->scales_x;
        int M = (int)args->M, K = (int)args->K;
        int64_t sxm = args->stride_xm, ssm = args->stride_sx_m;
        float post_v = r.gp.mx_post;
        void* eargs[] = {(void*)&xq, (void*)&sx, (void*)&x16, (void*)&post, (void*)&M, (void*)&K, (void*)&sxm, (void*)&ssm, (void*)&post_v};
        const int64_t nblk = ((int64_t)M * (K / 16) + 255) / 256;
        void* es = tl_evt_start; void* ee = tl_evt_stop;
        tl_evt_stop = nullptr;
        int rc = launch(nvfp4_expand_f16_kernel_fn(), dim3((unsigned)nblk, 1, 1), dim3(256, 1, 1), eargs, 0, st);
        if (rc != GEMLITE_OK) return rc;
        (void)es;
        tl_evt_start = nullptr; tl_evt_stop = ee;
        const int e = ensure_lds(r.lp.fn, r.lp.lds_bytes, dev);
        if (e != GEMLITE_OK) return e;
        void* kargs[] = {(void*)&r.wn};
        return launch(r.lp.fn, r.lp.grid, r.lp.block, kargs, r.lp.lds_bytes, st);
    }
    if (r.kind == K_A8_FQ) {
        if (!args->workspace || args->workspace_bytes < r.lp.ws_bytes) return GEMLITE_ERR_WORKSPACE;
        char* payload = (char*)args->workspace + COUNTER_BYTES;
        r.gp.counters = (unsigned*)args->workspace;
        r.gp.x = payload;
        r.gp.epi.scales_x = (const float*)(payload + cq::xq_bytes(args->M, args->K));
        const int e = ensure_lds(r.lp.fn, r.lp.lds_bytes, dev);
        if (e != GEMLITE_OK) return e;
        void* kargs[] = {(void*)&r.gp};
        return launch(r.lp.fn, r.lp.grid, r.lp.block, kargs, r.lp.lds_bytes, st);
    }
    void* kargs[] = {(void*)&r.gp};
    {
        const int e = ensure_lds(r.lp.fn, r.lp.lds_bytes, dev);
        if (e != GEMLITE_OK) return e;
    }
    return launch(r.lp.fn, r.lp.grid, r.lp.block, kargs, r.lp.lds_bytes, st);
}

int gemlite_hip_scale_activations_per_token(const void* x, void* y, float* scales, int64_t M, int64_t K,
                                            int64_t stride_xm, int32_t in_dtype, int32_t out_dtype, void* stream) {
    if (!x || !y || !scales || M <= 0 || K <= 0) return GEMLITE_ERR_BAD_ARGUMENT;
    if (!(in_dtype == GEMLITE_DT_FP16 || in_dtype == GEMLITE_DT_BF16 || in_dtype == GEMLITE_DT_FP32)) return GEMLITE_ERR_UNSUPPORTED;
    if (!(out_dtype == GEMLITE_DT_INT8 || out_dtype == GEMLITE_DT_FP8E4 || out_dtype == GEMLITE_DT_FP8E5)) return GEMLITE_ERR_UNSUPPORTED;
    if (M > 0x7FFFFFFF) return GEMLITE_ERR_BAD_SHAPE;
    int in_dt = in_dtype, out_dt = out_dtype;
    if (const void* vec = act_quant_vec_kernel_fn(in_dt, out_dt, K, stride_xm, x, y)) {
        int k32 = (int)K;
        void* vargs[] = {(void*)&x, (void*)&y, (void*)&scales, (void*)&k32, (void*)&stride_xm};
        return launch(vec, dim3((unsigned)M, 1, 1), dim3(256, 1, 1), vargs, 0, (hipStream_t)stream);
    }
    void* kargs[] = {(void*)&x, (void*)&y, (void*)&scales, (void*)&K, (void*)&stride_xm, (void*)&in_dt, (void*)&out_dt};
    return launch(act_quant_kernel_fn(), dim3((unsigned)M, 1, 1), dim3(256, 1, 1), kargs, 0, (hipStream_t)stream);
}

static int scale_activations_mx(int mode, const void* x, void* y, uint8_t* scales, int64_t M, int64_t K, int64_t stride_xm,
                                int32_t in_dtype, void* stream) {
    const int64_t G = mode == 2 ? 16 : 32;
    if (!x || !y || !scales || M <= 0 || K <= 0) return GEMLITE_ERR_BAD_ARGUMENT;
    if (!(in_dtype == GEMLITE_DT_FP16 || in_dtype == GEMLITE_DT_BF16 || in_dtype == GEMLITE_DT_FP32)) return GEMLITE_ERR_UNSUPPORTED;
    if (K % 32 != 0) return GEMLITE_ERR_BAD_SHAPE;
    if (((uintptr_t)y % 16) != 0) return GEMLITE_ERR_BAD_ARGUMENT;
    int64_t m_pad = (M + G - 1) / G * G;
    const int64_t total = m_pad * (K / G);
    if (total > 0x7FFFFFFFll * 256) return GEMLITE_ERR_BAD_SHAPE;
    int in_dt = in_dtype;
    void* kargs[] = {(void*)&x, (void*)&y, (void*)&scales, (void*)&M, (void*)&m_pad, (void*)&K, (void*)&stride_xm, (void*)&in_dt};
    return launch(act_quant_mx_kernel_fn(mode), dim3((unsigned)((total + 255) / 256), 1, 1), dim3(256, 1, 1), kargs, 0, (hipStream_t)stream);
}

int gemlite_hip_scale_activations_mxfp8(const void* x, void* y, uint8_t* scales, int64_t M, int64_t K, int64_t stride_xm,
                                        int32_t in_dtype, void* stream) {
    return scale_activations_mx(0, x, y, scales, M, K, stride_xm, in_dtype, stream);
}
int gemlite_hip_scale_activations_mxfp4(const void* x, uint8_t* y, uint8_t* scales, int64_t M, int64_t K, int64_t stride_xm,
                                        int32_t in_dtype, void* stream) {
    return scale_activations_mx(1, x, y, scales, M, K, stride_xm, in_dtype, stream);
}
int gemlite_hip_scale_activations_nvfp4(const void* x, uint8_t* y, uint8_t* scales, int64_t M, int64_t K, int64_t stride_xm,
                                        int32_t in_dtype, void* stream) {
    return scale_activations_mx(2, x, y, scales, M, K, stride_xm, in_dtype, stream);
}

static int check_pack(int64_t N, int64_t K, int32_t nbits, int32_t pack_bits) {
    if (N <= 0 || K <= 0) return GEMLITE_ERR_BAD_ARGUMENT;
    if (!(nbits == 1 || nbits == 2 || nbits == 4 || nbits == 8)) return GEMLITE_ERR_UNSUPPORTED;
    if (!(pack_bits == 8 || pack_bits == 16 || pack_bits == 32 || pack_bits == 64) || pack_bits < nbits) return GEMLITE_ERR_UNSUPPORTED;
    if (K % (pack_bits / nbits) != 0) return GEMLITE_ERR_BAD_SHAPE;
    if ((K / (pack_bits / nbits)) * N > 0x7FFFFFFFll * 256) return GEMLITE_ERR_BAD_SHAPE;
    return GEMLITE_OK;
}

int gemlite_hip_pack_over_cols(const uint8_t* w_q, void* out, int64_t N, int64_t K, int64_t ld_in, int32_t W_nbits,
                               int32_t pack_bits, void* stream) {
    if (!w_q || !out) return GEMLITE_ERR_BAD_ARGUMENT;
    const int c = check_pack(N, K, W_nbits, pack_bits);
    if (c != GEMLITE_OK) return c;
    const int64_t total = (K / (pack_bits / W_nbits)) * N;
    int nb = W_nbits, pb = pack_bits;
    if (pack_bits == 32 && K % (32 / W_nbits) == 0 && (N + 63) / 64 <= 0x7FFFFFFF && (K + 255) / 256 <= 65535) {
        void* targs[] = {(void*)&w_q, (void*)&out, (void*)&N, (void*)&K, (void*)&ld_in, (void*)&nb};
        return launch(pack32_kernel_fn(), dim3((unsigned)((N + 63) / 64), (unsigned)((K + 255) / 256), 1), dim3(256, 1, 1), targs, 0, (hipStream_t)stream);
    }
    void* kargs[] = {(void*)&w_q, (void*)&out, (void*)&N, (void*)&K, (void*)&ld_in, (void*)&nb, (void*)&pb};
    return launch(pack_kernel_fn(), dim3((unsigned)((total + 255) / 256), 1, 1), dim3(256, 1, 1), kargs, 0, (hipStream_t)stream);
}

int gemlite_hip_unpack_over_cols(const void* packed, uint8_t* out, int64_t N, int64_t K, int32_t W_nbits,
                                 int32_t pack_bits, void* stream) {
    if (!packed || !out) return GEMLITE_ERR_BAD_ARGUMENT;
    const int c = check_pack(N, K, W_nbits, pack_bits);
    if (c != GEMLITE_OK) return c;
    const int64_t total = (K / (pack_bits / W_nbits)) * N;
    int nb = W_nbits, pb = pack_bits;
    void* kargs[] = {(void*)&packed, (void*)&out, (void*)&N, (void*)&K, (void*)&nb, (void*)&pb};
    return launch(unpack_kernel_fn(), dim3((unsigned)((total + 255) / 256), 1, 1), dim3(256, 1, 1), kargs, 0, (hipStream_t)stream);
}

static int quantize_groups_launch(const gemlite_hip_quantize_args* a, const QuantHqqParams* h, void* stream) {
    if (!a || a->struct_size != sizeof(gemlite_hip_quantize_args)) return GEMLITE_ERR_BAD_ARGUMENT;
    if (!a->w || !a->q_out || !a->scales || !a->zeros) return GEMLITE_ERR_BAD_ARGUMENT;
    if (a->N <= 0 || a->K <= 0 || a->group_size <= 0 || a->ld_w < a->K) return GEMLITE_ERR_BAD_ARGUMENT;
    const int nb = a->W_nbits;
    if (!(nb == 1 || nb == 2 || nb == 4 || nb == 8)) return GEMLITE_ERR_UNSUPPORTED;
    if (!(a->pack_bits == 0 || a->pack_bits == 32)) return GEMLITE_ERR_UNSUPPORTED;
    if (!(a->w_dtype == GEMLITE_DT_FP32 || a->w_dtype == GEMLITE_DT_FP16 || a->w_dtype == GEMLITE_DT_BF16)) return GEMLITE_ERR_UNSUPPORTED;
    if (!(a->meta_dtype == GEMLITE_DT_FP16 || a->meta_dtype == GEMLITE_DT_BF16)) return GEMLITE_ERR_UNSUPPORTED;
    if (a->pack_bits == 0 && a->ld_q < a->K) return GEMLITE_ERR_BAD_ARGUMENT;
    const int64_t g = a->group_size;
    if (g % 32 != 0 || a->K % g != 0) return GEMLITE_ERR_BAD_SHAPE;
    if (a->pack_bits == 32 && a->K % (32 / nb) != 0) return GEMLITE_ERR_BAD_SHAPE;
    int64_t gcd = g, t = 256;
    while (t) { const int64_t r = gcd % t; gcd = t; t = r; }
    QuantGroupsParams p;
    p.w = a->w; p.q_out = a->q_out; p.scales = a->scales; p.zeros = a->zeros;
    p.N = a->N; p.K = a->K; p.ld_w = a->ld_w; p.ld_q = a->ld_q;
    p.stride_meta_g = a->stride_meta_g; p.stride_meta_n = a->stride_meta_n;
    p.span = g / gcd * 256;
    p.w_dt = a->w_dtype; p.meta_dt = a->meta_dtype; p.nbits = nb; p.group = (int)g;
    p.pack32 = a->pack_bits == 32; p.fold = a->fold_zeros != 0;
    const int64_t gx = (a->N + 63) / 64, gy = (a->K + p.span - 1) / p.span;
    if (gx > 0x7FFFFFFF || gy > 65535) return GEMLITE_ERR_BAD_SHAPE;
    if (h) {
        void* hargs[] = {(void*)&p, (void*)h};
        return launch(quantize_hqq_kernel_fn(p.span == 256), dim3((unsigned)gx, (unsigned)gy, 1), dim3(256, 1, 1), hargs, 0, (hipStream_t)stream);
    }
    void* kargs[] = {(void*)&p};
    return launch(quantize_groups_kernel_fn(p.span == 256), dim3((unsigned)gx, (unsigned)gy, 1), dim3(256, 1, 1), kargs, 0, (hipStream_t)stream);
}

int gemlite_hip_quantize_groups(const gemlite_hip_quantize_args* a, void* stream) { return quantize_groups_launch(a, nullptr, stream); }

int gemlite_hip_quantize_groups_hqq(const gemlite_hip_quantize_hqq_args* a, void* stream) {
    if (!a || a->struct_size != sizeof(gemlite_hip_quantize_hqq_args)) return GEMLITE_ERR_BAD_ARGUMENT;
    if (a->iters < 0 || a->iters > 100) return GEMLITE_ERR_BAD_ARGUMENT;
    const float inf = __builtin_inff();
    if (!(a->lp_norm > 0.f && a->lp_norm <= 1.f) || !(a->beta > 0.f && a->beta < inf) || !(a->kappa > 0.f && a->kappa < inf)) return GEMLITE_ERR_BAD_ARGUMENT;
    const QuantHqqParams h{a->iters, a->lp_norm, a->beta, a->kappa};
    return quantize_groups_launch(&a->q, &h, stream);
}

int gemlite_hip_quantize_mx(const gemlite_hip_quantize_mx_args* a, void* stream) {
    if (!a || a->struct_size != sizeof(gemlite_hip_quantize_mx_args)) return GEMLITE_ERR_BAD_ARGUMENT;
    if (!a->w || !a->q_out || !a->scales) return GEMLITE_ERR_BAD_ARGUMENT;
    if (a->N <= 0 || a->K <= 0 || a->ld_w < a->K) return GEMLITE_ERR_BAD_ARGUMENT;
    if (a->format < 0 || a->format > 2) return GEMLITE_ERR_UNSUPPORTED;
    if (!(a->w_dtype == GEMLITE_DT_FP32 || a->w_dtype == GEMLITE_DT_FP16 || a->w_dtype == GEMLITE_DT_BF16)) return GEMLITE_ERR_UNSUPPORTED;
    if (!(a->pack_nibbles == 0 || a->pack_nibbles == 1) || (a->pack_nibbles == 1 && a->format == 0)) return GEMLITE_ERR_UNSUPPORTED;
    if (a->ld_q < (a->pack_nibbles ? a->K / 2 : a->K)) return GEMLITE_ERR_BAD_ARGUMENT;
    if (a->K % 32 != 0) return GEMLITE_ERR_BAD_SHAPE;
    QuantMxParams p;
    p.w = a->w; p.q_out = (uint8_t*)a->q_out; p.scales = (uint8_t*)a->scales;
    p.N = a->N; p.K = a->K; p.ld_w = a->ld_w; p.ld_q = a->ld_q;
    p.stride_scale_g = a->stride_scale_g; p.stride_scale_n = a->stride_scale_n;
    p.w_dt = a->w_dtype; p.pack = a->pack_nibbles;
    const int64_t gx = (a->N + 63) / 64, gy = (a->K + 255) / 256;
    if (gx > 0x7FFFFFFF || gy > 65535) return GEMLITE_ERR_BAD_SHAPE;
    void* kargs[] = {(void*)&p};
    return launch(quantize_mx_kernel_fn(a->format), dim3((unsigned)gx, (unsigned)gy, 1), dim3(256, 1, 1), kargs, 0, (hipStream_t)stream);
}

int gemlite_hip_quantize_rows(const gemlite_hip_quantize_rows_args* a, void* stream) {
    if (!a || a->struct_size != sizeof(gemlite_hip_quantize_rows_args)) return GEMLITE_ERR_BAD_ARGUMENT;
    if (!a->w || !a->q_out || !a->scales) return GEMLITE_ERR_BAD_ARGUMENT;
    if (a->N <= 0 || a->K <= 0 || a->ld_w < a->K || a->ld_q < a->K || a->stride_s <= 0) return GEMLITE_ERR_BAD_ARGUMENT;
    if (a->format < 0 || a->format > 2 || !(a->scale_rule == 0 || a->scale_rule == 1)) return GEMLITE_ERR_UNSUPPORTED;
    if (!(a->w_dtype == GEMLITE_DT_FP32 || a->w_dtype == GEMLITE_DT_FP16 || a->w_dtype == GEMLITE_DT_BF16)) return GEMLITE_ERR_UNSUPPORTED;
    if (!(a->scale_dtype == GEMLITE_DT_FP32 || a->scale_dtype == GEMLITE_DT_FP16 || a->scale_dtype == GEMLITE_DT_BF16)) return GEMLITE_ERR_UNSUPPORTED;
    if (a->N > 0x7FFFFFFF) return GEMLITE_ERR_BAD_SHAPE;
    QuantRowsParams p;
    p.w = a->w; p.q_out = (uint8_t*)a->q_out; p.scales = a->scales;
    p.N = a->N; p.K = a->K; p.ld_w = a->ld_w; p.ld_q = a->ld_q; p.stride_s = a->stride_s;
    p.w_dt = a->w_dtype; p.scale_dt = a->scale_dtype; p.rule = a->scale_rule;
    const int64_t gx = a->K <= GEMLITE_QUANT_ROWS_WAVE_MAX_K ? (a->N + 3) / 4 : a->N;
    void* kargs[] = {(void*)&p};
    return launch(quantize_rows_kernel_fn(a->format, a->K), dim3((unsigned)gx, 1, 1), dim3(256, 1, 1), kargs, 0, (hipStream_t)stream);
}

int gemlite_hip_dequantize(const gemlite_hip_dequantize_args* a, void* stream) {
    if (!a || a->struct_size != sizeof(gemlite_hip_dequantize_args)) return GEMLITE_ERR_BAD_ARGUMENT;
    if (!a->w_q || !a->out) return GEMLITE_ERR_BAD_ARGUMENT;
    if (a->N <= 0 || a->K <= 0 || a->group_size <= 0 || a->elements_per_sample <= 0 || a->ld_out < a->K) return GEMLITE_ERR_BAD_ARGUMENT;
    if (!(a->out_dtype == GEMLITE_DT_FP16 || a->out_dtype == GEMLITE_DT_BF16 || a->out_dtype == GEMLITE_DT_FP32)) return GEMLITE_ERR_UNSUPPORTED;
    const int e = a->elements_per_sample, nb = a->W_nbits;
    DequantParams p{};
    bool grouped = false;
    if (is_mx_input(a->input_dtype)) {
        const bool nv = a->input_dtype == GEMLITE_DT_NVFP4;
        if (!a->scales) return GEMLITE_ERR_BAD_ARGUMENT;
        if (nb == 8) {
            if (nv || a->input_dtype == GEMLITE_DT_MXFP4 || e != 1 || a->w_dtype != GEMLITE_DT_FP8E4) return GEMLITE_ERR_UNSUPPORTED;
            p.fmt = DQ_MXFP8;
        } else if (nb == 4) {
            if (!(e == 1 || (e == 2 && a->w_pack_bits == 8))) return GEMLITE_ERR_UNSUPPORTED;
            p.fmt = nv ? DQ_NVFP4 : DQ_MXFP4;
        } else {
            return GEMLITE_ERR_UNSUPPORTED;
        }
        if (a->group_size != (nv ? 16 : 32)) return GEMLITE_ERR_UNSUPPORTED;
        if (a->K % 32 != 0) return GEMLITE_ERR_BAD_SHAPE;
        p.w_dt = e == 1 && nb == 8 ? GEMLITE_DT_FP8E4 : GEMLITE_DT_UINT8;
        p.pack_bits = e == 2 ? 8 : 0;
        p.group = a->group_size;
    } else {
        if (a->W_group_mode < 0 || a->W_group_mode > 4) return GEMLITE_ERR_UNSUPPORTED;
        if (a->channel_scale_mode < 0 || a->channel_scale_mode > 3) return GEMLITE_ERR_UNSUPPORTED;
        p.w_mode = a->W_group_mode;
        p.chan = a->channel_scale_mode == 1 || a->channel_scale_mode == 3;
        const bool need_s = p.w_mode >= 2 || p.chan, need_z = p.w_mode == 1 || p.w_mode >= 3;
        if ((need_s && !a->scales) || (need_z && !a->zeros)) return GEMLITE_ERR_BAD_ARGUMENT;
        if (e > 1) {
            if (a->w_pack_bits == 64) return GEMLITE_ERR_UNSUPPORTED;
            if (!(nb == 1 || nb == 2 || nb == 4 || nb == 8)) return GEMLITE_ERR_UNSUPPORTED;
            if (!(a->w_pack_bits == 8 || a->w_pack_bits == 16 || a->w_pack_bits == 32) || nb * e != a->w_pack_bits) return GEMLITE_ERR_BAD_ARGUMENT;
        } else {
            const int dt = a->w_dtype;
            if (!(dt == GEMLITE_DT_INT8 || dt == GEMLITE_DT_UINT8 || dt == GEMLITE_DT_FP8E4 || dt == GEMLITE_DT_FP8E5 || dt == GEMLITE_DT_FP16 ||
                  dt == GEMLITE_DT_BF16 || dt == GEMLITE_DT_FP32))
                return GEMLITE_ERR_UNSUPPORTED;
        }
        const auto meta_ok = [](int dt) { return dt == GEMLITE_DT_FP16 || dt == GEMLITE_DT_BF16 || dt == GEMLITE_DT_FP32; };
        if (need_s && !meta_ok(a->meta_dtype)) return GEMLITE_ERR_UNSUPPORTED;
        if (need_z && !(a->zero_is_scalar ? (a->zeros_dtype == GEMLITE_DT_INT32 || meta_ok(a->zeros_dtype)) : meta_ok(a->zeros_dtype))) return GEMLITE_ERR_UNSUPPORTED;
        if (a->K % e != 0) return GEMLITE_ERR_BAD_SHAPE;
        grouped = p.w_mode >= 2 || (need_z && !a->zero_is_scalar);
        if (grouped && a->K % a->group_size != 0) return GEMLITE_ERR_BAD_SHAPE;
        p.fmt = DQ_INT;
        p.w_dt = a->w_dtype;
        p.pack_bits = e > 1 ? a->w_pack_bits : 0;
        p.group = grouped ? a->group_size : (int)(a->K > 0x7FFFFFFF ? 0x7FFFFFFF : a->K);
    }
    if (a->N > 0x7FFFFFFFll * 64 || a->K > 65535ll * 256) return GEMLITE_ERR_BAD_SHAPE;
    p.w = a->w_q; p.scales = a->scales; p.zeros = a->zeros; p.out = a->out;
    p.N = a->N; p.K = a->K; p.stride_wk = a->stride_wk; p.stride_wn = a->stride_wn;
    p.stride_meta_g = a->stride_meta_g; p.stride_meta_n = a->stride_meta_n; p.ld_out = a->ld_out;
    p.nbits = nb; p.e = e;
    p.meta_dt = a->meta_dtype; p.zeros_dt = a->zeros_dtype; p.zero_is_scalar = a->zero_is_scalar != 0;
    p.out_dt = a->out_dtype; p.post = a->post_scale;

    const int osz = a->out_dtype == GEMLITE_DT_FP32 ? 4 : 2;
    const bool out_vec = ((uintptr_t)a->out % 16 == 0) && ((a->ld_out * osz) % 16 == 0) && a->K % 8 == 0;
    const void* fn = nullptr;
    if (out_vec && p.fmt == DQ_INT && e > 1 && a->w_pack_bits == 32 && a->stride_wn == 1 && a->stride_wk >= a->N && (uintptr_t)a->w_q % 4 == 0 &&
        (!grouped || a->group_size % 8 == 0)) {
        fn = dequantize_words_kernel_fn(nb);
    } else if (out_vec && a->stride_wk == 1) {
        const bool bytes8 = (uintptr_t)a->w_q % 8 == 0 && a->stride_wn % 8 == 0, bytes4 = (uintptr_t)a->w_q % 4 == 0 && a->stride_wn % 4 == 0;
        if (p.fmt == DQ_INT) {
            const int dt = a->w_dtype;
            const bool one_byte = e == 1 && (dt == GEMLITE_DT_INT8 || dt == GEMLITE_DT_UINT8 || dt == GEMLITE_DT_FP8E4 || dt == GEMLITE_DT_FP8E5);
            if (one_byte && bytes8 && a->stride_wn >= a->K && (!grouped || a->group_size % 8 == 0)) fn = dequantize_rows_kernel_fn(DQ_INT);
        } else if (e == 2 ? (bytes4 && a->stride_wn >= a->K / 2) : (bytes8 && a->stride_wn >= a->K)) {
            fn = dequantize_rows_kernel_fn(p.fmt);
        }
    }
    void* kargs[] = {(void*)&p};
    if (fn) return launch(fn, dim3((unsigned)((a->N + 63) / 64), (unsigned)((a->K + 255) / 256), 1), dim3(256, 1, 1), kargs, 0, (hipStream_t)stream);
    const int64_t blocks = (a->N * a->K + 255) / 256;
    if (blocks > 0x7FFFFFFF) return GEMLITE_ERR_BAD_SHAPE;
    return launch(dequantize_any_kernel_fn(), dim3((unsigned)blocks, 1, 1), dim3(256, 1, 1), kargs, 0, (hipStream_t)stream);
}

}
```

gemlite_amd/csrc/capture_group.hip:

```cpp
#include <atomic>
#include <cstdlib>
#include <cstring>

#include "gl_common.h"

namespace gl {

const void* gemv_w4_decode3_fn(int tag, bool nt);
const void* gemv_w4_decode3_group_fn(int tag);
const void* gemv_w4_decode3_bias_fn(int tag, bool nt);
const void* gemv_w4_decode3_bias_group_fn(int tag);
const void* gemv_w4_decode3_group_sx_fn(int tag, bool biased);
int ensure_lds(const void* fn, size_t lds, int dev);

namespace {

struct Span {
    uintptr_t lo, hi;
};
struct Footprint {
    Span rd[5];
    Span wr;
};

bool overlap(const Span& a, const Span& b) { return a.lo < b.hi && b.lo < a.hi && a.lo != a.hi && b.lo != b.hi; }

int elt_bytes(int dt) {
    switch (dt) {
        case GEMLITE_DT_FP16: case GEMLITE_DT_BF16: case GEMLITE_DT_INT16: case GEMLITE_DT_UINT16: return 2;
        case GEMLITE_DT_FP32: case GEMLITE_DT_INT32: case GEMLITE_DT_UINT32: return 4;
        default: return 8;
    }
}

Span span2d(const void* p, int64_t esz, int64_t n0, int64_t s0, int64_t n1, int64_t s1) {
    if (!p || n0 <= 0 || n1 <= 0) return Span{0, 0};
    const int64_t e0 = (n0 - 1) * s0, e1 = (n1 - 1) * s1;
    const int64_t lo = (e0 < 0 ? e0 : 0) + (e1 < 0 ? e1 : 0), hi = (e0 > 0 ? e0 : 0) + (e1 > 0 ? e1 : 0) + 1;
    return Span{(uintptr_t)p + (uintptr_t)(lo * esz), (uintptr_t)p + (uintptr_t)(hi * esz)};
}

Footprint footprint(const gemlite_hip_forward_args& a, const LaunchPlan& lp) {
    Footprint f;
    const int64_t e = a.elements_per_sample > 0 ? a.elements_per_sample : 1, gs = a.group_size > 0 ? a.group_size : 1;
    f.rd[0] = span2d(a.x, elt_bytes(a.input_dtype), a.M, a.stride_xm, a.K, a.stride_xk);
    f.rd[1] = span2d(a.w_q, a.w_pack_bits > 0 ? a.w_pack_bits / 8 : elt_bytes(a.w_dtype), (a.K + e - 1) / e, a.stride_wk, a.N, a.stride_wn);
    f.rd[2] = span2d(a.scales, elt_bytes(a.meta_dtype), (a.K + gs - 1) / gs, a.stride_meta_g, a.N, a.stride_meta_n);
    f.rd[3] = a.zero_is_scalar ? span2d(a.zeros, 8, 1, 0, 1, 0)
                               : span2d(a.zeros, elt_bytes(a.zeros_dtype), (a.K + gs - 1) / gs, a.stride_meta_g, a.N, a.stride_meta_n);
    f.rd[4] = span2d(lp.bias, 2, 1, 0, a.N, 1);
    f.wr = span2d(a.out, elt_bytes(a.output_dtype), a.M, a.stride_om, a.N, a.stride_on);
    return f;
}

bool independent(const Footprint& a, const Footprint& b) {
    if (overlap(a.wr, b.wr)) return false;
    for (int i = 0; i < 5; ++i)
        if (overlap(b.wr, a.rd[i]) || overlap(a.wr, b.rd[i])) return false;
    return true;
}

bool same_launch(const LaunchPlan& a, const LaunchPlan& b) {
    if (a.arg_kind == 2 && b.arg_kind == 2)
        return a.fn == b.fn && a.grid.x == b.grid.x && a.grid.y == 1 && b.grid.y == 1 && a.grid.z == 1 && b.grid.z == 1 &&
               a.block.x == b.block.x && a.lds_bytes == b.lds_bytes && a.r5.sw4 == b.r5.sw4 && a.r5.mstride2 == b.r5.mstride2 &&
               a.r5.nch_total == b.r5.nch_total && a.r5.modes == b.r5.modes && a.r5.M == b.r5.M && a.r5.sxm2 == b.r5.sxm2 &&
               a.r5.som == b.r5.som;
    return a.arg_kind == 1 && b.arg_kind == 1 && a.fn == b.fn && a.grid.x == b.grid.x && a.grid.y == 1 && b.grid.y == 1 && a.grid.z == 1 &&
           b.grid.z == 1 && a.block.x == b.block.x && a.d3.sw4 == b.d3.sw4 && a.d3.mstride2 == b.d3.mstride2 &&
           a.d3.nch_total == b.d3.nch_total && a.d3.modes == b.d3.modes && !(a.d3.modes & 64u);
}

const void* rows_group_fn_of(const LaunchPlan& lp) {
    if (lp.arg_kind != 2) return nullptr;
    return lp.bias ? (lp.fn == lp.fn_bias ? lp.fn_bias_group : nullptr) : (lp.fn == lp.bias_of ? lp.fn_group : nullptr);
}

const void* group_fn_of(const void* fn) {
    for (int tag = 0; tag < 2; ++tag)
        for (int nt = 0; nt < 2; ++nt)
            if (fn == gemv_w4_decode3_fn(tag, nt != 0)) return gemv_w4_decode3_group_fn(tag);
    for (int tag = 0; tag < 2; ++tag)
        for (int nt = 0; nt < 2; ++nt)
            if (fn == gemv_w4_decode3_bias_fn(tag, nt != 0)) return gemv_w4_decode3_bias_group_fn(tag);
    return nullptr;
}

const void* group_sx_fn_of(const void* fn) {
    for (int tag = 0; tag < 2; ++tag)
        for (int nt = 0; nt < 2; ++nt) {
            if (fn == gemv_w4_decode3_fn(tag, nt != 0)) return gemv_w4_decode3_group_sx_fn(tag, false);
            if (fn == gemv_w4_decode3_bias_fn(tag, nt != 0)) return gemv_w4_decode3_group_sx_fn(tag, true);
        }
    return nullptr;
}

int env_int(const char* name, int absent) {
    const char* v = getenv(name);
    return (v && *v) ? atoi(v) : absent;
}

std::atomic<uint64_t> g_seen{0}, g_joined{0};

struct Group {
    bool open = false;
    bool capturing = false;
    unsigned long long cap_id = 0;
    hipGraph_t graph = nullptr;
    hipGraphNode_t node = nullptr;
    LaunchPlan lp{};
    const void* fn_group = nullptr;
    const void* fn_group_sx = nullptr;
    bool same_x = true;
    Decode3GroupTable tab{};
    Decode3BiasGroupTable tabb{};
    Rows5GroupTable rtab{};
    Rows5BiasGroupTable rtabb{};
    Footprint fp[DECODE3_GMAX];
    int members = 0;
};
thread_local Group tl_group;
thread_local int tl_last_form = 0;

bool capture_state(hipStream_t st, unsigned long long* id, hipGraph_t* graph, hipGraphNode_t* only_dep) {
    hipStreamCaptureStatus status = hipStreamCaptureStatusNone;
    const hipGraphNode_t* deps = nullptr;
    size_t ndeps = 0;
    *graph = nullptr;
    if (hipStreamGetCaptureInfo_v2(st, &status, id, graph, &deps, &ndeps) != hipSuccess) {
        (void)hipGetLastError();
        return false;
    }
    if (status != hipStreamCaptureStatusActive || !*graph) return false;
    *only_dep = (ndeps == 1 && deps) ? deps[0] : nullptr;
    return true;
}

}

int capture_group_limit() {
    static const int limit = [] {
        if (env_int("GEMLITE_HIP_NO_CAPTURE_GROUPS", 0) != 0) return 1;
        const int n = env_int("GEMLITE_HIP_CAPTURE_GROUP_MAX", DECODE3_GMAX);
        return n < 1 ? 1 : (n > DECODE3_GMAX ? DECODE3_GMAX : n);
    }();
    return limit;
}

bool capture_group_rows_enabled() {
    static const bool on = env_int("GEMLITE_HIP_CAPTURE_GROUP_ROWS", 1) != 0;
    return on;
}

bool capture_group_shared_x_enabled() {
    static const bool on = env_int("GEMLITE_HIP_CAPTURE_GROUP_SHARED_X", 1) != 0;
    return on;
}

Decode3TilesWanted capture_group_tiles_wanted(int tiles, int members, int resident) {
    static const Decode3TilesWanted forced = [] {
        const char* v = getenv("GEMLITE_HIP_CAPTURE_GROUP_TILES");
        if (!v || !*v) return Decode3TilesWanted{0, false};
        const int tb = atoi(v);
        return Decode3TilesWanted{tb >= 4 ? 4 : (tb >= 2 ? 2 : 1), strchr(v, 's') != nullptr};
    }();
    return forced.tb ? forced : decode3_group_tiles_default(tiles, members, resident);
}

int capture_group_last_form() { return tl_last_form; }

void capture_group_stats(uint64_t* seen, uint64_t* joined) {
    if (seen) *seen = g_seen.load(std::memory_order_relaxed);
    if (joined) *joined = g_joined.load(std::memory_order_relaxed);
}

bool capture_group_compatible(const gemlite_hip_forward_args& a, const LaunchPlan& la, const gemlite_hip_forward_args& b, const LaunchPlan& lb) {
    if (!same_launch(la, lb)) return false;
    if (la.arg_kind == 2 ? rows_group_fn_of(la) == nullptr : group_fn_of(la.fn) == nullptr) return false;
    return independent(footprint(a, la), footprint(b, lb));
}

bool capture_group_try_join(const gemlite_hip_forward_args& a, const LaunchPlan& lp, hipStream_t st, int resident, int dev) {
    Group& g = tl_group;
    g.capturing = false;
    const bool rows = lp.arg_kind == 2;
    if (capture_group_limit() < 2 || (rows ? !capture_group_rows_enabled() : (lp.d3.modes & 64u) != 0)) return false;
    unsigned long long id = 0;
    hipGraph_t graph = nullptr;
    hipGraphNode_t dep = nullptr;
    if (!capture_state(st, &id, &graph, &dep)) {
        g.open = false;
        return false;
    }
    g.capturing = true;
    g_seen.fetch_add(1, std::memory_order_relaxed);
    if (!g.open || g.cap_id != id || g.graph != graph || !dep || dep != g.node || g.members >= capture_group_limit() || !same_launch(g.lp, lp))
        return false;
    const Footprint fb = footprint(a, lp);
    for (int i = 0; i < g.members; ++i)
        if (!independent(g.fp[i], fb)) return false;
    const bool biased = g.lp.bias != nullptr;
    if (rows) {
        if (ensure_lds(g.fn_group, g.lp.lds_bytes, dev) != GEMLITE_OK) {
            g.open = false;
            return false;
        }
        Rows5Member& rm = biased ? g.rtabb.m[g.members - 1] : g.rtab.m[g.members - 1];
        if (biased) g.rtabb.bias[g.members] = lp.bias;
        rm.w = lp.r5.w; rm.x = lp.r5.x; rm.s = lp.r5.s; rm.z = lp.r5.z; rm.out = lp.r5.out;
        Rows5Args& r = g.lp.r5;
        void* rargs[] = {(void*)&r.w, (void*)&r.x, (void*)&r.s, (void*)&r.z, (void*)&r.out, (void*)&r.sw4, (void*)&r.mstride2, (void*)&r.nch_total,
                         (void*)&r.modes, (void*)&r.M, (void*)&r.sxm2, (void*)&r.som, biased ? (void*)&g.rtabb : (void*)&g.rtab};
        hipKernelNodeParams rp;
        memset(&rp, 0, sizeof(rp));
        rp.func = (void*)g.fn_group;
        rp.gridDim = dim3(g.lp.grid.x, (unsigned)(g.members + 1), 1);
        rp.blockDim = g.lp.block;
        rp.sharedMemBytes = (unsigned)g.lp.lds_bytes;
        rp.kernelParams = rargs;
        rp.extra = nullptr;
        if (hipGraphKernelNodeSetParams(g.node, &rp) != hipSuccess) {
            (void)hipGetLastError();
            g.open = false;
            return false;
        }
        g.fp[g.members++] = fb;
        tl_last_form = 3;
        g_joined.fetch_add(1, std::memory_order_relaxed);
        return true;
    }
    Decode3Member& m = biased ? g.tabb.m[g.members - 1] : g.tab.m[g.members - 1];
    if (biased) g.tabb.bias[g.members] = lp.bias;
    m.w = lp.d3.w; m.x = lp.d3.x; m.s = lp.d3.s; m.z = lp.d3.z; m.out = lp.d3.out;
    Decode3Args& d = g.lp.d3;
    const int members = g.members + 1, tiles = (int)g.lp.grid.x;
    const Decode3TilesWanted want = capture_group_tiles_wanted(tiles, members, resident);
    const Decode3GroupGeometry geo = decode3_group_geometry(tiles, members, resident, want.tb, want.span);
    uint32_t modes = decode3_group_modes(d.modes, members, geo.grid_y, geo.tb, geo.span);
    void* kargs[] = {(void*)&d.w, (void*)&d.x, (void*)&d.s, (void*)&d.z, (void*)&d.out, (void*)&d.sw4, (void*)&d.mstride2,
                     (void*)&d.nch_total, (void*)&modes, biased ? (void*)&g.tabb : (void*)&g.tab};
    const bool same_x = g.same_x && lp.d3.x == d.x;
    int form = decode3_group_form(members, same_x, d.nch_total, capture_group_shared_x_enabled() && g.fn_group_sx != nullptr);
    const size_t lds = form == 2 ? (size_t)decode3_shared_x_lds_bytes(d.nch_total) : 0;
    if (form == 2 && ensure_lds(g.fn_group_sx, (size_t)DECODE3_SHARED_X_MAX_LDS, dev) != GEMLITE_OK) form = 1;
    hipKernelNodeParams np;
    memset(&np, 0, sizeof(np));
    np.func = (void*)(form == 2 ? g.fn_group_sx : g.fn_group);
    np.gridDim = dim3((unsigned)geo.grid_x, (unsigned)geo.grid_y, 1);
    np.blockDim = g.lp.block;
    np.sharedMemBytes = form == 2 ? (unsigned)lds : 0;
    np.kernelParams = kargs;
    np.extra = nullptr;
    if (hipGraphKernelNodeSetParams(g.node, &np) != hipSuccess) {
        (void)hipGetLastError();
        g.open = false;
        return false;
    }
    g.fp[g.members++] = fb;
    g.same_x = same_x;
    tl_last_form = form;
    g_joined.fetch_add(1, std::memory_order_relaxed);
    return true;
}

void capture_group_note_launch(const gemlite_hip_forward_args& a, const LaunchPlan& lp, hipStream_t st) {
    Group& g = tl_group;
    if (!g.capturing) return;
    g.capturing = false;
    g.open = false;
    const void* fn_group = lp.arg_kind == 2 ? rows_group_fn_of(lp) : group_fn_of(lp.fn);
    if (!fn_group || (lp.arg_kind != 1 && lp.arg_kind != 2) || lp.grid.y != 1 || lp.grid.z != 1) return;
    unsigned long long id = 0;
    hipGraph_t graph = nullptr;
    hipGraphNode_t dep = nullptr;
    if (!capture_state(st, &id, &graph, &dep) || !dep) return;
    hipGraphNodeType type = hipGraphNodeTypeEmpty;
    if (hipGraphNodeGetType(dep, &type) != hipSuccess) { (void)hipGetLastError(); return; }
    if (type != hipGraphNodeTypeKernel) return;
    g.cap_id = id;
    g.graph = graph;
    g.node = dep;
    g.lp = lp;
    g.fn_group = fn_group;
    g.fn_group_sx = lp.arg_kind == 1 ? group_sx_fn_of(lp.fn) : nullptr;
    g.same_x = true;
    tl_last_form = 0;
    memset(&g.tab, 0, sizeof(g.tab));
    memset(&g.tabb, 0, sizeof(g.tabb));
    g.tabb.bias[0] = lp.bias;
    memset(&g.rtab, 0, sizeof(g.rtab));
    memset(&g.rtabb, 0, sizeof(g.rtabb));
    g.rtabb.bias[0] = lp.bias;
    g.fp[0] = footprint(a, lp);
    g.members = 1;
    g.open = true;
}

}
```

gemlite_amd/csrc/gemv_decode.hip:

```cpp
#include <type_traits>

#include "gl_common.h"
#include "gl_async.h"

#ifndef GL_DECODE3_ABLATION
#define GL_DECODE3_ABLATION 0
#endif
#ifndef GL_DECODE3_DOT2_ZERO
#define GL_DECODE3_DOT2_ZERO 0
#endif

namespace gl {

namespace dec3 {

template <int CTRL>
__device__ __forceinline__ uint32_t dpp_mov(uint32_t v) {
    return (uint32_t)__builtin_amdgcn_update_dpp(0, (int)v, CTRL, 0xF, 0xF, true);
}
template <int CTRL>
__device__ __forceinline__ float dpp_movf(float v) {
    return __builtin_bit_cast(float, dpp_mov<CTRL>(__builtin_bit_cast(uint32_t, v)));
}

constexpr uint32_t M_ZSCALAR = 16u, M_PAIR = 32u, M_PROBE = 64u;

}

template <typename Tail>
struct Decode3TailKind {
    static constexpr bool shared_x = std::is_same<Tail, Decode3GroupTableSX>::value || std::is_same<Tail, Decode3BiasGroupTableSX>::value;
    static constexpr bool grouped = std::is_same<Tail, Decode3GroupTable>::value || std::is_same<Tail, Decode3BiasGroupTable>::value || shared_x;
    static constexpr bool biased = std::is_same<Tail, Decode3BiasTail>::value || std::is_same<Tail, Decode3BiasGroupTable>::value ||
                                   std::is_same<Tail, Decode3BiasGroupTableSX>::value;
};

template <typename Tag, bool NT, typename Tail = unsigned*>
__global__ __launch_bounds__(1024, (Decode3TailKind<Tail>::grouped ? DECODE3_GROUP_WAVES_PER_SIMD : 1))
void gemv_w4_decode3_kernel(const char* wb, const char* xb, const char* sp, const char* zp, uint16_t* out,
                            uint32_t sw4, uint32_t mstride2, int nch_total, uint32_t modes,
                            const Tail counters) {
    using namespace dec3;
    constexpr bool GROUPED = Decode3TailKind<Tail>::grouped, BIASED = Decode3TailKind<Tail>::biased, SX = Decode3TailKind<Tail>::shared_x;
    using TR = F16Traits<Tag>;
    constexpr bool SUBN = TR::DT == GEMLITE_DT_FP16;
    constexpr int WP = SUBN ? 2 : 1;
    constexpr int R = 2, NW = 16, CHUNK = 32, TC = 16, CSTRIDE = NW * CHUNK;
    constexpr int RED = NW * 4 * TC;
    __shared__ __attribute__((aligned(16))) float red[(GROUPED && !SX ? DECODE3_GMAX : 1) * RED];

    const int tid = threadIdx.x, lane = tid & 63;
    const int wave = __builtin_amdgcn_readfirstlane(tid >> 6);
    const int c = lane & 3, g = lane >> 2;
    int tile = blockIdx.x;
    [[maybe_unused]] int g_members = 0, g_Y = 1, g_slots = 1, g_tbl = 0, g_tile0 = 0;
    [[maybe_unused]] Decode3WaveSplit g_split{0, 0, 16};
    if constexpr (GROUPED) {
        g_members = (int)((modes >> 16) & DECODE3_M_MEMBERS);
        g_Y = (int)(modes >> 24);
        g_tbl = (int)((modes >> DECODE3_M_TB_SHIFT) & 3u);
        g_slots = ((g_members - (int)blockIdx.y + g_Y - 1) / g_Y) << g_tbl;
        g_split = decode3_wave_split(g_slots, wave);
        const bool span = (modes & DECODE3_M_SPAN) != 0u;
        g_tile0 = decode3_group_first_tile(tile, span ? (int)gridDim.x : 0, 1 << g_tbl, span, (modes & M_PAIR) != 0u);
        tile = g_tile0 + ((g_split.layer < 0 ? 0 : g_split.layer) & ((1 << g_tbl) - 1));
    } else if (modes & M_PAIR) {
        const int xcd = tile & 7, idx = tile >> 3;
        tile = (((idx >> 1) << 3) + xcd) * 2 + (idx & 1);
    }
    const uint32_t n0 = (uint32_t)(tile * TC + c * 4);
    const int nchunks = (nch_total - wave + NW - 1) / NW;
    const int w_mode = (int)(modes & 15u), gs_shift = (int)((modes >> 8) & 255u);
    const bool need_s = w_mode >= 2, need_z = (w_mode == 1 || w_mode >= 3) && !(modes & M_ZSCALAR);

    const uint32_t row0 = (uint32_t)(wave * CHUNK + g * R);
    const uint32_t wo0 = row0 * sw4 + n0 * 4u;
    const uint32_t xo0 = (uint32_t)(wave * CHUNK) * 16u + (uint32_t)lane * 8u;

    struct Chunk { u32x4 w[R]; u32x2 s, z, xq; };
    auto load_chunk = [&](Chunk& ck, int chunk) {
        const uint32_t wo = wo0 + (uint32_t)(chunk * CSTRIDE) * sw4;
#pragma unroll
        for (int i = 0; i < R; ++i) {
            const u32x4* src = (const u32x4*)(wb + (wo + (uint32_t)i * sw4));
            ck.w[i] = NT ? __builtin_nontemporal_load(src) : *src;
        }
        ck.xq = *(const u32x2*)(xb + (xo0 + (uint32_t)(chunk * CSTRIDE) * 16u));
        const uint32_t row = row0 + (uint32_t)(chunk * CSTRIDE);
        const uint32_t mo = (uint32_t)((row * 8u) >> gs_shift) * mstride2 + n0 * 2u;
        ck.s = *(const u32x2*)((need_s ? sp : wb) + (need_s ? mo : 0u));
        ck.z = *(const u32x2*)((need_z ? zp : wb) + (need_z ? mo : 0u));
    };

    auto stamp = [&](int i) {
        if constexpr (!GROUPED && !BIASED) {
            if (__builtin_expect((modes & M_PROBE) != 0u, 0)) {
                if (counters && wave == 0 && lane == 0 && blockIdx.x < 1024)
                    ((unsigned long long*)(counters + MAX_SPLITK_COUNTERS))[blockIdx.x * 4 + i] = __builtin_amdgcn_s_memrealtime();
            }
        }
    };
    stamp(0);
    Chunk cur, nxt;
    if constexpr (!GROUPED) {
        if (nchunks > 0) load_chunk(cur, 0);
        if (nchunks > 1) load_chunk(nxt, 1);
    }
    stamp(1);

    float tot[4] = {0.f, 0.f, 0.f, 0.f};
    float scalar_zero = 0.f;
    if constexpr (!GROUPED) scalar_zero = (modes & M_ZSCALAR) ? (float)((const int32_t*)zp)[0] : 0.f;
    const float bz = (w_mode == 1 || w_mode == 3) ? -1.f : (w_mode == 4 ? 1.f : 0.f);
    const bool b_times_s = w_mode == 3;
    constexpr float QSCALE = SUBN ? 16777216.0f : 1.0f;
    uint32_t wmask[WP];
#pragma unroll
    for (int i = 0; i < WP; ++i) wmask[i] = (15u * 0x00010001u) << (4 * i);

    struct XStage { u32x4 p[R]; float sum; } xs;
    auto compute = [&](const Chunk& ck, auto full) {
        constexpr bool FULL = decltype(full)::value;
        float acc[WP][4];
#pragma unroll
        for (int wi = 0; wi < WP; ++wi)
#pragma unroll
            for (int j = 0; j < 4; ++j) acc[wi][j] = 0.f;
        float xsum = 0.f;
        uint32_t a0 = 0, a1 = 0, a2 = 0, a3 = 0, b0 = 0, b1 = 0, b2 = 0, b3 = 0;
        if constexpr (!SX) {
            a0 = dpp_mov<0x00>(ck.xq[0]), a1 = dpp_mov<0x00>(ck.xq[1]), a2 = dpp_mov<0x55>(ck.xq[0]), a3 = dpp_mov<0x55>(ck.xq[1]);
            b0 = dpp_mov<0xAA>(ck.xq[0]), b1 = dpp_mov<0xAA>(ck.xq[1]), b2 = dpp_mov<0xFF>(ck.xq[0]), b3 = dpp_mov<0xFF>(ck.xq[1]);
        }
#pragma unroll
        for (int i = 0; i < R; ++i) {
            const uint32_t d0 = i ? b0 : a0, d1 = i ? b1 : a1, d2 = i ? b2 : a2, d3 = i ? b3 : a3;
            uint32_t xr[4];
            if constexpr (SX) {
#pragma unroll
                for (int dd = 0; dd < 4; ++dd) xr[dd] = xs.p[i][dd];
            } else {
                xr[0] = __builtin_amdgcn_perm(d2, d0, 0x05040100u);
                xr[1] = __builtin_amdgcn_perm(d2, d0, 0x07060302u);
                xr[2] = __builtin_amdgcn_perm(d3, d1, 0x05040100u);
                xr[3] = __builtin_amdgcn_perm(d3, d1, 0x07060302u);
#pragma unroll
                for (int dd = 0; dd < 4; ++dd) xsum = TR::dot2(xr[dd], TR::ONES2, xsum);
            }
#pragma unroll
            for (int dd = 0; dd < 4; ++dd) {
                const int win = dd / WP, wi = dd % WP;
#pragma unroll
                for (int j = 0; j < 4; ++j) {
                    uint32_t h = (ck.w[i][j] >> (4 * WP * win)) & wmask[wi];
                    if constexpr (!SUBN) h |= TR::MAGIC2;
#if GL_DECODE3_DOT2_ZERO
                    if constexpr (SUBN && GROUPED) {
                        if (i == 0 && win == 0) {
                            asm("v_dot2_f32_f16 %0, %1, %2, 0" : "=v"(acc[wi][j]) : "v"(h), "v"(xr[dd]));
                            continue;
                        }
                    }
#endif
                    acc[wi][j] = TR::dot2(h, xr[dd], acc[wi][j]);
                }
            }
        }
        if constexpr (SX) xsum = xs.sum;
        const uint32_t s0 = ck.s[0], s1 = ck.s[1], z0 = ck.z[0], z1 = ck.z[1];
        float s[4] = {TR::to_float((uint16_t)(s0 & 0xFFFFu)), TR::to_float((uint16_t)(s0 >> 16)), TR::to_float((uint16_t)(s1 & 0xFFFFu)), TR::to_float((uint16_t)(s1 >> 16))};
        float z[4] = {TR::to_float((uint16_t)(z0 & 0xFFFFu)), TR::to_float((uint16_t)(z0 >> 16)), TR::to_float((uint16_t)(z1 & 0xFFFFu)), TR::to_float((uint16_t)(z1 >> 16))};
#pragma unroll
        for (int j = 0; j < 4; ++j) {
            if constexpr (!FULL) {
                if (!need_s) s[j] = 1.f;
                if (!need_z) z[j] = scalar_zero;
            }
            const float a = s[j] * QSCALE;
            const float b = bz * z[j] * (b_times_s ? s[j] : 1.f);
            float v = acc[0][j];
            if constexpr (WP > 1) v = __builtin_fmaf(acc[WP - 1][j], 1.0f / 16.0f, v);
            if constexpr (!SUBN) v -= TR::OFF * xsum;
            tot[j] += __builtin_fmaf(b, xsum, a * v);
        }
    };
    if constexpr (!GROUPED) {
#pragma unroll 1
        for (int ch = 0; ch < nchunks; ++ch) {
            compute(cur, std::false_type{});
            if (ch + 1 < nchunks) {
                cur = nxt;
                if (ch + 2 < nchunks) load_chunk(nxt, ch + 2);
            }
        }
        stamp(2);
        uint16_t braw = 0;
        if constexpr (BIASED) {
            if (wave == 0 && lane < 16) braw = counters.bias[tile * TC + lane];
        }

#pragma unroll
        for (int j = 0; j < 4; ++j) {
            float v = tot[j];
            v += dpp_movf<0x124>(v);
            v += dpp_movf<0x128>(v);
            tot[j] = v;
        }
        if ((lane & 12) == 0) *(f32x4*)(red + ((wave * 4 + (lane >> 4)) * TC + c * 4)) = (f32x4){tot[0], tot[1], tot[2], tot[3]};
        __syncthreads();
        if (wave == 0) {
            constexpr int PER = NW;
            const int o = lane & 15, part = lane >> 4;
            float v = 0.f;
#pragma unroll
            for (int r = 0; r < PER; ++r) v += red[(part * PER + r) * TC + o];
            v += __shfl_xor(v, 16);
            v += __shfl_xor(v, 32);
            uint16_t h = TR::from_float(v);
            if constexpr (BIASED) h = TR::from_float(TR::to_float(h) + TR::to_float(braw));
            if (lane < 16) out[tile * TC + o] = h;
        }
        stamp(3);
    } else {
        const int Y = g_Y, y = (int)blockIdx.y, slots = g_slots;
        const Decode3WaveSplit split = g_split;
        const int slot = split.layer < 0 ? 0 : split.layer, li = slot >> g_tbl, v0 = split.v0, v1 = split.v1;
        const int L = y + li * Y;
        const char *w_ = wb, *x_ = xb, *s_ = sp, *z_ = zp;
        if (L > 0) {
            const Decode3Member& m = counters.m[L - 1];
            w_ = m.w; x_ = m.x; s_ = m.s; z_ = m.z;
        }
        if (modes & M_ZSCALAR) scalar_zero = (float)((const int32_t*)z_)[0];
        const uint32_t vw0 = (uint32_t)(g * R) * sw4 + n0 * 4u, vw1 = vw0 + sw4, vx = (uint32_t)lane * 8u;
        const uint32_t vm = (gs_shift < 8 ? (uint32_t)(g * R * 8) >> gs_shift : 0u) * mstride2 + n0 * 2u;
        const uint32_t vs = need_s ? vm : 0u, vz = need_z ? vm : 0u, ms_s = need_s ? mstride2 : 0u, ms_z = need_z ? mstride2 : 0u;
        const char *sb = need_s ? s_ : w_, *zb = need_z ? z_ : w_;
        const int shl = gs_shift < 8 ? 8 - gs_shift : 0, shr = gs_shift > 8 ? gs_shift - 8 : 0;
        const uint32_t chunk_w = (uint32_t)CHUNK * sw4;
        const int nv = v1 - v0, rem = (nch_total & (NW - 1)) - v0;
        const int n = (nch_total / NW) * nv + (rem < 0 ? 0 : (rem > nv ? nv : rem));
        float* redg;
        uint32_t* xpairs = nullptr;
        float* xsums = nullptr;
        const int units = nch_total * 16;
        if constexpr (SX) {
            extern __shared__ __attribute__((aligned(16))) float d3_lds[];
            redg = d3_lds;
            xpairs = (uint32_t*)(d3_lds + DECODE3_GMAX * RED);
            xsums = (float*)(xpairs + units * 8);
        } else {
            redg = red;
        }
        float* rd = redg + slot * RED;

        constexpr int NLC = SX ? 4 : 5;
        int rv = v0, rgc = v0;
        auto request = [&](Chunk& ck, int ri) __attribute__((always_inline)) {
#if GL_DECODE3_ABLATION == 2
            const int keep = rgc;
            if (ri >= 2) rgc = v0;
#endif
            const char* wq = w_ + (uint32_t)rgc * chunk_w;
            gvw::gld128<NT>(ck.w[0], wq, vw0);
            gvw::gld128<NT>(ck.w[1], wq, vw1);
            if constexpr (!SX) gvw::gld64(ck.xq, x_ + (uint32_t)rgc * (uint32_t)(CHUNK * 16), vx);
            const uint32_t grp = ((uint32_t)rgc << shl) >> shr;
            gvw::gld64(ck.s, sb + grp * ms_s, vs);
            gvw::gld64(ck.z, zb + grp * ms_z, vz);
#if GL_DECODE3_ABLATION == 2
            rgc = keep;
#endif
            rgc += NW;
            if (rgc >= nch_total) rgc = ++rv;
        };
        auto tie_chunk = [&](Chunk& ck) __attribute__((always_inline)) {
            gvw::tie(ck.w[0]);
            gvw::tie(ck.w[1]);
            if constexpr (!SX) gvw::tie(ck.xq);
            gvw::tie(ck.s);
            gvw::tie(ck.z);
        };
        auto flush = [&](int v) {
#pragma unroll
            for (int j = 0; j < 4; ++j) {
                float t = tot[j];
                t += dpp_movf<0x124>(t);
                t += dpp_movf<0x128>(t);
                tot[j] = t;
            }
            if ((lane & 12) == 0) *(f32x4*)(rd + ((v * 4 + (lane >> 4)) * TC + c * 4)) = (f32x4){tot[0], tot[1], tot[2], tot[3]};
#pragma unroll
            for (int j = 0; j < 4; ++j) tot[j] = 0.f;
        };
        int cv = v0, cgc = v0;
        auto stage_unit = [&](int u, const u32x4& lo, const u32x4& hi) __attribute__((always_inline)) {
            u32x4 pr[R];
            float xsum = 0.f;
#pragma unroll
            for (int i = 0; i < R; ++i) {
                const u32x4& d = i ? hi : lo;
                pr[i][0] = __builtin_amdgcn_perm(d[2], d[0], 0x05040100u);
                pr[i][1] = __builtin_amdgcn_perm(d[2], d[0], 0x07060302u);
                pr[i][2] = __builtin_amdgcn_perm(d[3], d[1], 0x05040100u);
                pr[i][3] = __builtin_amdgcn_perm(d[3], d[1], 0x07060302u);
#pragma unroll
                for (int dd = 0; dd < 4; ++dd) xsum = TR::dot2(pr[i][dd], TR::ONES2, xsum);
            }
            if (u < units) {
                *(u32x4*)(xpairs + u * 8) = pr[0];
                *(u32x4*)(xpairs + u * 8 + 4) = pr[1];
                xsums[u] = xsum;
            }
        };
        auto stage_off = [&](int u) { return (uint32_t)(u < units ? u : units - 1) * 32u; };
        constexpr int STRIPS = (int)((DECODE3_SHARED_X_MAX_UNITS + 1023) / 1024);
        const uint32_t* xp_lane = xpairs + g * 8;
        const float* xs_lane = xsums + g;
        auto run = [&](auto full) {
            Chunk A, B;
            if constexpr (SX) {
                u32x4 lo[STRIPS], hi[STRIPS];
#pragma unroll
                for (int t = 0; t < STRIPS; ++t) {
                    if (wave * 64 + t * 1024 < units) {
                        const uint32_t so = stage_off(tid + t * 1024);
                        gvw::gld128<false>(lo[t], xb, so);
                        gvw::gld128<false>(hi[t], xb, so + 16u);
                    }
                }
                if (n > 0) request(A, 0);
                if (n > 1) request(B, 1);
                if (wave * 64 < units) {
                    if (n > 1) gvw::wait_vm<2 * NLC>(); else if (n > 0) gvw::wait_vm<NLC>(); else gvw::wait_vm<0>();
#pragma unroll
                    for (int t = 0; t < STRIPS; ++t) {
                        if (wave * 64 + t * 1024 < units) {
                            gvw::tie(lo[t]);
                            gvw::tie(hi[t]);
                            stage_unit(tid + t * 1024, lo[t], hi[t]);
                        }
                    }
                }
                __syncthreads();
            } else {
                if (n > 0) request(A, 0);
                if (n > 1) request(B, 1);
            }
            gvw::ring2_run_pre<NLC>(n, A, B, request, tie_chunk, [&](int) __attribute__((always_inline)) {
                if constexpr (SX) {
                    const uint32_t* xp = xp_lane + cgc * 128;
                    xs.p[0] = *(const u32x4*)xp;
                    xs.p[1] = *(const u32x4*)(xp + 4);
                    xs.sum = xs_lane[cgc * 16];
                }
            }, [&](const Chunk& ck, int) __attribute__((always_inline)) {
#if GL_DECODE3_ABLATION == 1
                uint32_t acc = ck.s[0] ^ ck.s[1] ^ ck.z[0] ^ ck.z[1];
#pragma unroll
                for (int j = 0; j < 4; ++j) acc ^= ck.w[0][j] ^ ck.w[1][j];
                if constexpr (SX) acc ^= xs.p[0][0] ^ xs.p[1][3] ^ __builtin_bit_cast(uint32_t, xs.sum); else acc ^= ck.xq[0] ^ ck.xq[1];
                tot[0] = __builtin_bit_cast(float, __builtin_bit_cast(uint32_t, tot[0]) ^ acc);
#else
                compute(ck, full);
#endif
                cgc += NW;
                if (cgc >= nch_total) {
                    flush(cv);
                    cgc = ++cv;
                }
            });
        };
        if (need_s && need_z) run(std::true_type{}); else run(std::false_type{});
        if (split.layer >= 0) {
#pragma unroll 1
            for (int v = cv; v < v1; ++v) flush(v);
        }

        const bool fin = wave < slots;
        const int ftile = g_tile0 + (wave & ((1 << g_tbl) - 1));
        uint16_t* o_ = out;
        uint16_t braw = 0;
        if (fin) {
            const int Lf = y + (wave >> g_tbl) * Y;
            if (Lf > 0) o_ = counters.m[Lf - 1].out;
            if constexpr (BIASED) {
                if (lane < 16) braw = counters.bias[Lf][ftile * TC + lane];
            }
        }
        __syncthreads();
        if (fin) {
            const float* rf = redg + wave * RED;
            constexpr int PER = NW;
            const int o = lane & 15, part = lane >> 4;
            float v = 0.f;
#pragma unroll
            for (int r = 0; r < PER; ++r) v += rf[(part * PER + r) * TC + o];
            v += __shfl_xor(v, 16);
            v += __shfl_xor(v, 32);
            uint16_t h = TR::from_float(v);
            if constexpr (BIASED) h = TR::from_float(TR::to_float(h) + TR::to_float(braw));
            if (lane < 16) o_[ftile * TC + o] = h;
        }
    }
}

const void* gemv_w4_decode3_fn(int tag, bool nt) {
    typedef void (*kfn)(const char*, const char*, const char*, const char*, uint16_t*, uint32_t, uint32_t, int, uint32_t, unsigned*);
    kfn k = tag == 0 ? (nt ? gemv_w4_decode3_kernel<half_tag, true> : gemv_w4_decode3_kernel<half_tag, false>)
                     : (nt ? gemv_w4_decode3_kernel<bf16_tag, true> : gemv_w4_decode3_kernel<bf16_tag, false>);
    return (const void*)k;
}

const void* gemv_w4_decode3_group_fn(int tag) {
    typedef void (*kfn)(const char*, const char*, const char*, const char*, uint16_t*, uint32_t, uint32_t, int, uint32_t, const Decode3GroupTable);
    kfn k = tag == 0 ? gemv_w4_decode3_kernel<half_tag, false, Decode3GroupTable> : gemv_w4_decode3_kernel<bf16_tag, false, Decode3GroupTable>;
    return (const void*)k;
}

const void* gemv_w4_decode3_group_sx_fn(int tag, bool biased) {
    typedef void (*kfn)(const char*, const char*, const char*, const char*, uint16_t*, uint32_t, uint32_t, int, uint32_t, const Decode3GroupTableSX);
    typedef void (*kfnb)(const char*, const char*, const char*, const char*, uint16_t*, uint32_t, uint32_t, int, uint32_t, const Decode3BiasGroupTableSX);
    if (biased) {
        kfnb k = tag == 0 ? gemv_w4_decode3_kernel<half_tag, false, Decode3BiasGroupTableSX> : gemv_w4_decode3_kernel<bf16_tag, false, Decode3BiasGroupTableSX>;
        return (const void*)k;
    }
    kfn k = tag == 0 ? gemv_w4_decode3_kernel<half_tag, false, Decode3GroupTableSX> : gemv_w4_decode3_kernel<bf16_tag, false, Decode3GroupTableSX>;
    return (const void*)k;
}

const void* gemv_w4_decode3_bias_fn(int tag, bool nt) {
    typedef void (*kfn)(const char*, const char*, const char*, const char*, uint16_t*, uint32_t, uint32_t, int, uint32_t, const Decode3BiasTail);
    kfn k = tag == 0 ? (nt ? gemv_w4_decode3_kernel<half_tag, true, Decode3BiasTail> : gemv_w4_decode3_kernel<half_tag, false, Decode3BiasTail>)
                     : (nt ? gemv_w4_decode3_kernel<bf16_tag, true, Decode3BiasTail> : gemv_w4_decode3_kernel<bf16_tag, false, Decode3BiasTail>);
    return (const void*)k;
}

const void* gemv_w4_decode3_bias_group_fn(int tag) {
    typedef void (*kfn)(const char*, const char*, const char*, const char*, uint16_t*, uint32_t, uint32_t, int, uint32_t, const Decode3BiasGroupTable);
    kfn k = tag == 0 ? gemv_w4_decode3_kernel<half_tag, false, Decode3BiasGroupTable> : gemv_w4_decode3_kernel<bf16_tag, false, Decode3BiasGroupTable>;
    return (const void*)k;
}

}
```

gemlite_amd/csrc/gl_common.h:

```cpp
#pragma once
#include <hip/hip_runtime.h>
#include <stdint.h>

#include "../../include/gemlite_hip.h"

namespace gl {

typedef _Float16 h2_t __attribute__((ext_vector_type(2)));
typedef __bf16 b2_t __attribute__((ext_vector_type(2)));
typedef _Float16 h8_t __attribute__((ext_vector_type(8)));
typedef __bf16 b8_t __attribute__((ext_vector_type(8)));
typedef float f32x4 __attribute__((ext_vector_type(4)));
typedef float f32x16 __attribute__((ext_vector_type(16)));
typedef uint32_t u32x4 __attribute__((ext_vector_type(4)));
typedef uint32_t u32x2 __attribute__((ext_vector_type(2)));
typedef int i32x16 __attribute__((ext_vector_type(16)));

struct half_tag {};
struct bf16_tag {};

template <typename Tag>
struct F16Traits;

template <>
struct F16Traits<half_tag> {
    static constexpr uint32_t MAGIC2 = 0x64006400u;
    static constexpr float OFF = 1024.0f;
    static constexpr int MAX_QBITS = 8;
    static constexpr uint32_t ONES2 = 0x3C003C00u;
    static constexpr int DT = GEMLITE_DT_FP16;
    typedef h8_t frag8;
    static __device__ __forceinline__ float dot2(uint32_t a, uint32_t b, float c) {
        return __builtin_amdgcn_fdot2(__builtin_bit_cast(h2_t, a), __builtin_bit_cast(h2_t, b), c, false);
    }
    static __device__ __forceinline__ float to_float(uint16_t v) {
        return (float)__builtin_bit_cast(_Float16, v);
    }
    static __device__ __forceinline__ uint16_t from_float(float f) {
        return __builtin_bit_cast(uint16_t, (_Float16)f);
    }
};

template <>
struct F16Traits<bf16_tag> {
    static constexpr uint32_t MAGIC2 = 0x43004300u;
    static constexpr float OFF = 128.0f;
    static constexpr int MAX_QBITS = 4;
    static constexpr uint32_t ONES2 = 0x3F803F80u;
    static constexpr int DT = GEMLITE_DT_BF16;
    typedef b8_t frag8;
    static __device__ __forceinline__ float dot2(uint32_t a, uint32_t b, float c) {
        return __builtin_amdgcn_fdot2_f32_bf16(__builtin_bit_cast(b2_t, a), __builtin_bit_cast(b2_t, b), c, false);
    }
    static __device__ __forceinline__ float to_float(uint16_t v) {
        return __builtin_bit_cast(float, (uint32_t)v << 16);
    }
    static __device__ __forceinline__ uint16_t from_float(float f) {
        return __builtin_bit_cast(uint16_t, (__bf16)f);
    }
};

#define GL_HD __host__ __device__ __forceinline__

GL_HD float fp8e4m3_to_float(uint8_t v) {
    const uint32_t s = (uint32_t)(v & 0x80) << 24;
    const uint32_t em = v & 0x7F;
    if (em == 0x7F) return __builtin_bit_cast(float, s | 0x7FC00000u);
    const uint32_t e = em >> 3, m = em & 7;
    if (e == 0) {
        const float f = (float)m * 0.001953125f;
        return s ? -f : f;
    }
    return __builtin_bit_cast(float, s | ((e + 120u) << 23) | (m << 20));
}

GL_HD float fp8e5m2_to_float(uint8_t v) {
    const uint16_t h = (uint16_t)v << 8;
    return (float)__builtin_bit_cast(_Float16, h);
}

GL_HD uint8_t float_to_fp8e4m3(float f) {
    uint32_t u = __builtin_bit_cast(uint32_t, f);
    const uint8_t s = (u >> 24) & 0x80;
    u &= 0x7FFFFFFFu;
    if (u > 0x7F800000u) return s | 0x7F;
    const float a = __builtin_bit_cast(float, u);
    if (a > 464.0f) return s | 0x7F;
    if (a < 0.015625f) {
        const float r = __builtin_rintf(a * 512.0f);
        return s | (uint8_t)r;
    }
    const uint32_t lsb = (u >> 20) & 1u;
    u += 0x7FFFFu + lsb;
    const uint32_t e = (u >> 23) - 120u, m = (u >> 20) & 7u;
    return s | (uint8_t)((e << 3) | m);
}

GL_HD uint8_t float_to_fp8e5m2(float f) {
    uint32_t u = __builtin_bit_cast(uint32_t, f);
    const uint8_t s = (u >> 24) & 0x80;
    u &= 0x7FFFFFFFu;
    if (u > 0x7F800000u) return s | 0x7F;
    const float a = __builtin_bit_cast(float, u);
    if (a >= 61440.0f) return s | 0x7C;
    if (a < 6.103515625e-05f) {
        const float r = __builtin_rintf(a * 65536.0f);
        return s | (uint8_t)r;
    }
    const uint32_t lsb = (u >> 21) & 1u;
    u += 0xFFFFFu + lsb;
    const uint32_t e = (u >> 23) - 112u, m = (u >> 21) & 3u;
    return s | (uint8_t)((e << 2) | m);
}

__device__ __forceinline__ float load_as_float(const void* p, int64_t i, int dt) {
    switch (dt) {
        case GEMLITE_DT_FP32: return ((const float*)p)[i];
        case GEMLITE_DT_FP16: return (float)((const _Float16*)p)[i];
        case GEMLITE_DT_BF16: return __builtin_bit_cast(float, (uint32_t)((const uint16_t*)p)[i] << 16);
        case GEMLITE_DT_INT8: return (float)((const int8_t*)p)[i];
        case GEMLITE_DT_UINT8: return (float)((const uint8_t*)p)[i];
        case GEMLITE_DT_INT32: return (float)((const int32_t*)p)[i];
        case GEMLITE_DT_FP8E4: return fp8e4m3_to_float(((const uint8_t*)p)[i]);
        case GEMLITE_DT_FP8E5: return fp8e5m2_to_float(((const uint8_t*)p)[i]);
        default: return 0.0f;
    }
}

__device__ __forceinline__ void store_from_float(void* p, int64_t i, int dt, float v) {
    switch (dt) {
        case GEMLITE_DT_FP32: ((float*)p)[i] = v; break;
        case GEMLITE_DT_FP16: ((_Float16*)p)[i] = (_Float16)v; break;
        case GEMLITE_DT_BF16: ((__bf16*)p)[i] = (__bf16)v; break;
        case GEMLITE_DT_INT32: ((int32_t*)p)[i] = (int32_t)__builtin_rintf(v); break;
        default: break;
    }
}

__device__ __forceinline__ f32x4 load_meta4(const void* p, int64_t i, int dt) {
    f32x4 r;
    if (dt == GEMLITE_DT_FP16) {
        for (int j = 0; j < 4; ++j) r[j] = (float)((const _Float16*)p)[i + j];
    } else if (dt == GEMLITE_DT_BF16) {
        const u32x2 v = *(const u32x2*)((const uint16_t*)p + i);
        r[0] = __builtin_bit_cast(float, v[0] << 16); r[1] = __builtin_bit_cast(float, v[0] & 0xFFFF0000u);
        r[2] = __builtin_bit_cast(float, v[1] << 16); r[3] = __builtin_bit_cast(float, v[1] & 0xFFFF0000u);
    } else if (dt == GEMLITE_DT_FP32) {
        r = *(const f32x4*)((const float*)p + i);
    } else {
        for (int j = 0; j < 4; ++j) r[j] = load_as_float(p, i + j, dt);
    }
    return r;
}

typedef unsigned short u16x2_t __attribute__((ext_vector_type(2)));
__device__ __forceinline__ uint32_t pk_umax16(uint32_t a, uint32_t b) {
    return __builtin_bit_cast(uint32_t, __builtin_elementwise_max(__builtin_bit_cast(u16x2_t, a), __builtin_bit_cast(u16x2_t, b)));
}
__device__ __forceinline__ uint32_t absmax16_acc(uint32_t m, const u32x4& d) {
    constexpr uint32_t ABS = 0x7FFF7FFFu;
    return pk_umax16(m, pk_umax16(pk_umax16(d[0] & ABS, d[1] & ABS), pk_umax16(d[2] & ABS, d[3] & ABS)));
}
__device__ __forceinline__ uint32_t absmax16_shfl(uint32_t m, int off) { return pk_umax16(m, (uint32_t)__shfl_xor((int)m, off)); }
template <int N>
__device__ __forceinline__ uint32_t absmax16_merge(const uint32_t* w) {
    if constexpr (N == 1) return w[0];
    else return pk_umax16(absmax16_merge<N / 2>(w), absmax16_merge<N - N / 2>(w + N / 2));
}
__device__ __forceinline__ float absmax16_value(uint32_t m, bool f16) {
    const uint32_t lo = m & 0xFFFFu, hi = m >> 16;
    const uint16_t h = (uint16_t)(lo > hi ? lo : hi);
    return f16 ? F16Traits<half_tag>::to_float(h) : F16Traits<bf16_tag>::to_float(h);
}
__device__ __forceinline__ float absmax_keep_nan(float a, float v) {
    const uint32_t x = __builtin_bit_cast(uint32_t, a), y = __builtin_bit_cast(uint32_t, v) & 0x7FFFFFFFu;
    return __builtin_bit_cast(float, x > y ? x : y);
}
__device__ __forceinline__ float token_scale_keep_nan(float amax, float qmax) {
    const float s = __fdiv_rn(amax, qmax);
    return s < 1e-6f ? 1e-6f : s;
}
__device__ __forceinline__ bool amax_not_finite(float amax) { return (__builtin_bit_cast(uint32_t, amax) & 0x7FFFFFFFu) >= 0x7F800000u; }

struct Epilogue {
    void* out;
    const void* scales_w;
    const float* scales_x;
    int64_t stride_om, stride_on, stride_sx_m;
    int out_dt, meta_dt, c_mode;
};

__device__ __forceinline__ float epilogue_scale(const Epilogue& e, float v, int64_t m, int64_t n) {
    if (e.c_mode == 1) {
        v *= load_as_float(e.scales_w, n, e.meta_dt);
    } else if (e.c_mode == 2) {
        v *= e.scales_x[m * e.stride_sx_m];
    } else if (e.c_mode == 3) {
        v *= e.scales_x[m * e.stride_sx_m] * load_as_float(e.scales_w, n, e.meta_dt);
    }
    return v;
}

__device__ __forceinline__ void epilogue_store(const Epilogue& e, float v, int64_t m, int64_t n) {
    store_from_float(e.out, m * e.stride_om + n * e.stride_on, e.out_dt, epilogue_scale(e, v, m, n));
}

template <typename Tag>
__device__ __forceinline__ f32x4 load4_t(const void* p, int64_t i) {
    const u32x2 v = *(const u32x2*)((const uint16_t*)p + i);
    f32x4 r;
    const uint32_t v0 = v[0], v1 = v[1];
    if constexpr (F16Traits<Tag>::DT == GEMLITE_DT_FP16) {
        r[0] = (float)__builtin_bit_cast(_Float16, (uint16_t)(v0 & 0xFFFFu));
        r[1] = (float)__builtin_bit_cast(_Float16, (uint16_t)(v0 >> 16));
        r[2] = (float)__builtin_bit_cast(_Float16, (uint16_t)(v1 & 0xFFFFu));
        r[3] = (float)__builtin_bit_cast(_Float16, (uint16_t)(v1 >> 16));
    } else {
        r[0] = __builtin_bit_cast(float, v0 << 16); r[1] = __builtin_bit_cast(float, v0 & 0xFFFF0000u);
        r[2] = __builtin_bit_cast(float, v1 << 16); r[3] = __builtin_bit_cast(float, v1 & 0xFFFF0000u);
    }
    return r;
}

template <typename Tag>
__device__ __forceinline__ void store_out_t(const Epilogue& e, float v, int64_t m, int64_t n) {
    using TR = F16Traits<Tag>;
    auto sw = [&]() -> float { return e.meta_dt == TR::DT ? TR::to_float(((const uint16_t*)e.scales_w)[n]) : load_as_float(e.scales_w, n, e.meta_dt); };
    if (e.c_mode == 1) {
        v *= sw();
    } else if (e.c_mode == 2) {
        v *= e.scales_x[m * e.stride_sx_m];
    } else if (e.c_mode == 3) {
        v *= e.scales_x[m * e.stride_sx_m] * sw();
    }
    ((uint16_t*)e.out)[m * e.stride_om + n] = TR::from_float(v);
}

template <typename Tag>
__device__ __forceinline__ void store_out4_t(const Epilogue& e, f32x4 v, int64_t m, int64_t n0) {
    using TR = F16Traits<Tag>;
    if (e.c_mode == 1 || e.c_mode == 3) {
        const f32x4 sw = load4_t<Tag>(e.scales_w, n0);
        v *= sw;
    }
    if (e.c_mode == 2 || e.c_mode == 3) {
        const float sx = e.scales_x[m * e.stride_sx_m];
        v *= (f32x4){sx, sx, sx, sx};
    }
    u32x2 o;
    o[0] = (uint32_t)TR::from_float(v[0]) | ((uint32_t)TR::from_float(v[1]) << 16);
    o[1] = (uint32_t)TR::from_float(v[2]) | ((uint32_t)TR::from_float(v[3]) << 16);
    *(u32x2*)((uint16_t*)e.out + m * e.stride_om + n0) = o;
}

__device__ __forceinline__ void store_out4_any(const Epilogue& e, f32x4 v, int64_t m, int64_t n0) {
    f32x4 sw = {1.f, 1.f, 1.f, 1.f};
    if (e.c_mode == 1 || e.c_mode == 3) {
        if (e.meta_dt == GEMLITE_DT_FP32) sw = *(const f32x4*)((const float*)e.scales_w + n0);
        else if (e.meta_dt == GEMLITE_DT_FP16) sw = load4_t<half_tag>(e.scales_w, n0);
        else sw = load4_t<bf16_tag>(e.scales_w, n0);
    }
    if (e.c_mode == 2 || e.c_mode == 3) {
        const float sx = e.scales_x[m * e.stride_sx_m];
        sw = e.c_mode == 3 ? (f32x4){sx * sw[0], sx * sw[1], sx * sw[2], sx * sw[3]} : (f32x4){sx, sx, sx, sx};
    }
    if (e.c_mode != 0) v *= sw;
    if (e.out_dt == GEMLITE_DT_FP32) {
        *(f32x4*)((float*)e.out + m * e.stride_om + n0) = v;
        return;
    }
    u32x2 o;
    if (e.out_dt == GEMLITE_DT_FP16) {
        o[0] = (uint32_t)F16Traits<half_tag>::from_float(v[0]) | ((uint32_t)F16Traits<half_tag>::from_float(v[1]) << 16);
        o[1] = (uint32_t)F16Traits<half_tag>::from_float(v[2]) | ((uint32_t)F16Traits<half_tag>::from_float(v[3]) << 16);
    } else {
        o[0] = (uint32_t)F16Traits<bf16_tag>::from_float(v[0]) | ((uint32_t)F16Traits<bf16_tag>::from_float(v[1]) << 16);
        o[1] = (uint32_t)F16Traits<bf16_tag>::from_float(v[2]) | ((uint32_t)F16Traits<bf16_tag>::from_float(v[3]) << 16);
    }
    *(u32x2*)((uint16_t*)e.out + m * e.stride_om + n0) = o;
}


__device__ __forceinline__ float dequant_f32(float q, float s, float z, int w_mode) {
    switch (w_mode) {
        case 1: return q - z;
        case 2: return q * s;
        case 3: return (q - z) * s;
        case 4: return __builtin_fmaf(q, s, z);
        default: return q;
    }
}

__device__ __forceinline__ void group_affine(float s, float z, int w_mode, float& a, float& b) {
    switch (w_mode) {
        case 1: a = 1.0f; b = -z; break;
        case 2: a = s; b = 0.0f; break;
        case 3: a = s; b = -z * s; break;
        case 4: a = s; b = z; break;
        default: a = 1.0f; b = 0.0f; break;
    }
}

constexpr int COUNTER_WORDS = 65536;
constexpr int PROBE_WORDS = 4096;
constexpr int MAX_SPLITK_COUNTERS = COUNTER_WORDS - PROBE_WORDS;
constexpr uint64_t COUNTER_BYTES = (uint64_t)COUNTER_WORDS * 4;

constexpr int K_ORDER_ON = 1 << 30;
constexpr int K_ORDER_GROUP_SHIFT = 24;
constexpr int K_ORDER_GROUPS_OF_1 = 1 << K_ORDER_GROUP_SHIFT;
static inline int caller_flags(const gemlite_hip_forward_args& a) { return a.tuning[3] & GEMLITE_TF_PUBLIC_MASK; }
#if defined(GL_MMA_EXPERIMENTS) || defined(GL_TILED_EXPERIMENTS)
static inline int dev_ablation() { const char* s = getenv("GEMLITE_DEV_ABLATION"); return s ? atoi(s) : 0; }
#endif

__device__ __forceinline__ void slab_store(float* p, float v) {
    __hip_atomic_store(p, v, __ATOMIC_RELAXED, __HIP_MEMORY_SCOPE_AGENT);
}
__device__ __forceinline__ float slab_load(const float* p) {
    return __hip_atomic_load(p, __ATOMIC_RELAXED, __HIP_MEMORY_SCOPE_AGENT);
}

__device__ __forceinline__ bool splitk_arrive_is_last(unsigned* counter, unsigned nslices, unsigned* lds_flag) {
    asm volatile("s_waitcnt vmcnt(0)" ::: "memory");
    __syncthreads();
    if (threadIdx.x == 0) {
        *lds_flag = __hip_atomic_fetch_add(counter, 1u, __ATOMIC_RELAXED, __HIP_MEMORY_SCOPE_AGENT);
    }
    __syncthreads();
    return *lds_flag == nslices - 1u;
}
__device__ __forceinline__ void splitk_reset(unsigned* counter) {
    __hip_atomic_store(counter, 0u, __ATOMIC_RELAXED, __HIP_MEMORY_SCOPE_AGENT);
}

struct WnParams {
    const void* x;
    const uint32_t* w;
    const void* scales;
    const void* zeros;
    Epilogue epi;
    float* slabs;
    unsigned* counters;
    int M, N, K;
    int group_size;
    int w_mode;
    int meta_dt, zeros_dt;
    int zero_is_scalar;
    int splitk;
    int rows_per_slice;
    int64_t stride_xm, stride_xk, stride_wk, stride_meta_g;
    int64_t stride_wn_b, stride_meta_n;
    int combine;
    int flags;
    int gs_shift;
    uint32_t gs_magic;
};

__device__ __forceinline__ int group_of(int k, int gs_shift) { return k >> gs_shift; }
__device__ __forceinline__ int group_of(int k, int gs_shift, uint32_t gs_magic) {
    return gs_shift >= 0 ? (k >> gs_shift) : (int)__umulhi((uint32_t)k >> 5, gs_magic);
}

template <typename Buf, typename Load>
__device__ __forceinline__ void pipeline2_prime(int n, Buf& A, Buf& B, Load&& load) {
    load(A, 0);
    if (n > 1) load(B, 1);
}
template <typename Buf, typename Load, typename Compute>
__device__ __forceinline__ void pipeline2_run(int n, Buf& A, Buf& B, Load&& load, Compute&& compute) {
    int i = 0;
    for (; i + 4 <= n; i += 2) {
        compute(A, i);
        load(A, i + 2);
        compute(B, i + 1);
        load(B, i + 3);
    }
    const int rem = n - i;
    compute(A, i);
    if (rem >= 2) {
        if (rem == 3) load(A, i + 2);
        compute(B, i + 1);
        if (rem == 3) compute(A, i + 2);
    }
}

struct GenericParams {
    const void* x;
    const void* w;
    const void* scales;
    const void* zeros;
    Epilogue epi;
    int M, N, K;
    int nbits, e, pack_bits;
    int w_dt;
    int x_dt;
    int group_size, w_mode, meta_dt, zeros_dt, zero_is_scalar;
    int int_acc;
    int64_t stride_xm, stride_xk, stride_wk, stride_wn, stride_meta_g, stride_meta_n;
    float* slabs;
    unsigned* counters;
    int splitk;
    int flags;
    const void* sx_blocks;
    int64_t stride_sx_blk_m;
    int mx_x, mx_w, mx_scale_e4m3;
    float mx_post;
    const void* cq_x;
    int64_t cq_stride_xm;
    int cq_xdt;
};
enum { MX_F16 = 1, MX_BF16 = 2, MX_FP8 = 3, MX_FP4 = 4 };

__device__ __forceinline__ void load8_as_float(const void* w, int w_dt, int64_t ld_w, bool vec, int64_t n, int64_t k, float (&v)[8]) {
    const int64_t off = n * ld_w + k;
    if (w_dt == GEMLITE_DT_FP32) {
        const float* s = (const float*)w + off;
        if (vec) {
            const f32x4 a = *(const f32x4*)s, b = *(const f32x4*)(s + 4);
            v[0] = a[0]; v[1] = a[1]; v[2] = a[2]; v[3] = a[3];
            v[4] = b[0]; v[5] = b[1]; v[6] = b[2]; v[7] = b[3];
        } else {
#pragma unroll
            for (int e = 0; e < 8; ++e) v[e] = s[e];
        }
    } else {
        const uint16_t* s = (const uint16_t*)w + off;
        uint32_t d[4];
        if (vec) {
            const u32x4 a = *(const u32x4*)s;
            d[0] = a[0]; d[1] = a[1]; d[2] = a[2]; d[3] = a[3];
        } else {
#pragma unroll
            for (int e = 0; e < 4; ++e) d[e] = (uint32_t)s[2 * e] | ((uint32_t)s[2 * e + 1] << 16);
        }
        const bool f16 = w_dt == GEMLITE_DT_FP16;
#pragma unroll
        for (int e = 0; e < 8; ++e) {
            const uint16_t h = (uint16_t)(d[e >> 1] >> (16 * (e & 1)));
            v[e] = f16 ? F16Traits<half_tag>::to_float(h) : F16Traits<bf16_tag>::to_float(h);
        }
    }
}

struct QuantMxParams {
    const void* w;
    uint8_t* q_out;
    uint8_t* scales;
    int64_t N, K, ld_w, ld_q, stride_scale_g, stride_scale_n;
    int w_dt, pack;
};

struct QuantRowsParams {
    const void* w;
    uint8_t* q_out;
    void* scales;
    int64_t N, K, ld_w, ld_q, stride_s;
    int w_dt, scale_dt, rule;
};

struct QuantGroupsParams {
    const void* w;
    void* q_out;
    void* scales;
    void* zeros;
    int64_t N, K, ld_w, ld_q, stride_meta_g, stride_meta_n;
    int64_t span;
    int w_dt, meta_dt, nbits, group, pack32, fold;
};

struct QuantHqqParams {
    int iters;
    float lp_norm, beta, kappa;
};

enum { DQ_INT = 0, DQ_MXFP8 = 1, DQ_MXFP4 = 2, DQ_NVFP4 = 3 };
struct DequantParams {
    const void* w;
    const void* scales;
    const void* zeros;
    void* out;
    int64_t N, K, stride_wk, stride_wn, stride_meta_g, stride_meta_n, ld_out;
    int nbits, e, pack_bits;
    int w_dt, meta_dt, zeros_dt, zero_is_scalar, group, w_mode;
    int chan;
    int fmt;
    int out_dt;
    float post;
};

int resident_block_limit();
const char* pw_label(const char* name, int pack_bits);
const char* bias_label(const char* name);

struct Decode3Args {
    const char *w, *x, *s, *z;
    uint16_t* out;
    uint32_t sw4, mstride2;
    int nch_total;
    uint32_t modes;
    unsigned* counters;
};

constexpr int DECODE3_GMAX = 16;
struct Decode3Member {
    const char *w, *x, *s, *z;
    uint16_t* out;
};
struct Decode3GroupTable {
    Decode3Member m[DECODE3_GMAX - 1];
};
struct Decode3BiasTail {
    const uint16_t* bias;
};
struct Decode3BiasGroupTable {
    Decode3Member m[DECODE3_GMAX - 1];
    const uint16_t* bias[DECODE3_GMAX];
};
struct Decode3GroupTableSX {
    Decode3Member m[DECODE3_GMAX - 1];
};
struct Decode3BiasGroupTableSX {
    Decode3Member m[DECODE3_GMAX - 1];
    const uint16_t* bias[DECODE3_GMAX];
};
constexpr int64_t DECODE3_RED_BYTES = (int64_t)DECODE3_GMAX * 16 * 4 * 16 * 4, DECODE3_LDS_LIMIT = 160 * 1024;
constexpr int64_t DECODE3_SHARED_X_MAX_UNITS = ((DECODE3_LDS_LIMIT - DECODE3_RED_BYTES) / 36) & ~(int64_t)15;
constexpr int64_t DECODE3_SHARED_X_MAX_LDS = DECODE3_RED_BYTES + DECODE3_SHARED_X_MAX_UNITS * 36;
constexpr int DECODE3_SHARED_X_MIN_MEMBERS = 3;
inline int64_t decode3_shared_x_lds_bytes(int64_t nch_total) {
    return (nch_total > 0 && nch_total * 16 <= DECODE3_SHARED_X_MAX_UNITS) ? DECODE3_RED_BYTES + nch_total * 16 * 36 : 0;
}
inline int decode3_group_form(int members, bool same_x, int64_t nch_total, bool shared_x_enabled) {
    if (members < 2) return 0;
    return (shared_x_enabled && same_x && members >= DECODE3_SHARED_X_MIN_MEMBERS && decode3_shared_x_lds_bytes(nch_total) > 0) ? 2 : 1;
}
constexpr uint32_t DECODE3_M_MEMBERS = 31u, DECODE3_M_TB_SHIFT = 21u, DECODE3_M_SPAN = 1u << 23;
inline uint32_t decode3_group_modes(uint32_t modes, int members, int grid_y, int tb = 1, bool span = false) {
    return (modes & 0xFFFFu) | ((uint32_t)members << 16) | ((tb == 4 ? 2u : (tb == 2 ? 1u : 0u)) << DECODE3_M_TB_SHIFT) | (span ? DECODE3_M_SPAN : 0u) |
           ((uint32_t)grid_y << 24);
}
GL_HD int decode3_group_grid_y(int64_t tiles, int members, int64_t resident) {
    const int64_t y = tiles > 0 ? resident / tiles : 1;
    return (int)(y < 1 ? 1 : (y > members ? (members > 1 ? members : 1) : y));
}
struct Decode3WaveSplit {
    int layer;
    int v0, v1;
};
GL_HD Decode3WaveSplit decode3_wave_split(int lb, int wave) {
    const int P = 16 / lb, li = wave / P, wl = wave - li * P;
    if (li >= lb) return Decode3WaveSplit{-1, 0, 0};
    return Decode3WaveSplit{li, wl * 16 / P, (wl + 1) * 16 / P};
}
struct Decode3GroupGeometry {
    int tb, grid_x, grid_y;
    bool span;
};
GL_HD Decode3GroupGeometry decode3_group_geometry(int tiles, int members, int64_t resident, int tb_want, bool span) {
    for (int tb = tb_want >= 4 ? 4 : (tb_want >= 2 ? 2 : 1); tb > 1; tb >>= 1) {
        if (tiles % tb) continue;
        const int y = decode3_group_grid_y(tiles / tb, members, resident);
        if ((members + y - 1) / y * tb <= 16) return Decode3GroupGeometry{tb, tiles / tb, y, span};
    }
    return Decode3GroupGeometry{1, tiles, decode3_group_grid_y(tiles, members, resident), span};
}
GL_HD int decode3_group_first_tile(int block, int groups, int tb, bool span, bool pair) {
    const int xcd = block & 7, idx = block >> 3;
    int grp = block;
    if (span) {
        if ((groups & 7) == 0) grp = xcd * (groups >> 3) + idx;
    } else if (pair && tb == 1) {
        grp = (((idx >> 1) << 3) + xcd) * 2 + (idx & 1);
    }
    return grp * tb;
}
struct Decode3TilesWanted {
    int tb;
    bool span;
};
GL_HD int64_t decode3_group_busiest_cu(int tiles, int members, int64_t resident, int tb) {
    const Decode3GroupGeometry geo = decode3_group_geometry(tiles, members, resident, tb, false);
    if (geo.tb != tb) return -1;
    const int64_t blocks = (int64_t)geo.grid_x * geo.grid_y, cus = resident > 0 ? resident : 1;
    return (blocks + cus - 1) / cus * ((members + geo.grid_y - 1) / geo.grid_y) * tb;
}
inline Decode3TilesWanted decode3_group_tiles_default(int tiles, int members, int64_t resident) {
    const int64_t one = decode3_group_busiest_cu(tiles, members, resident, 1);
    for (int tb = 4; tb > 1; tb >>= 1) {
        const int64_t c = decode3_group_busiest_cu(tiles, members, resident, tb);
        if (c >= 0 && c * 4 <= one * 5) return Decode3TilesWanted{tb, false};
    }
    return Decode3TilesWanted{1, false};
}

#ifndef DECODE3_GROUP_WAVES_PER_SIMD
#define DECODE3_GROUP_WAVES_PER_SIMD 4
#endif

struct Rows5Args {
    const char *w, *x, *s, *z;
    uint16_t* out;
    uint32_t sw4, mstride2;
    int nch_total;
    uint32_t modes;
    int M;
    uint32_t sxm2, som;
};

constexpr int ROWS5_GMAX = DECODE3_GMAX;
struct Rows5Member {
    const char *w, *x, *s, *z;
    uint16_t* out;
};
struct Rows5GroupTable {
    Rows5Member m[ROWS5_GMAX - 1];
};
struct Rows5BiasGroupTable {
    Rows5Member m[ROWS5_GMAX - 1];
    const uint16_t* bias[ROWS5_GMAX];
};

struct LaunchPlan {
    const void* fn;
    const char* name;
    dim3 grid, block;
    size_t lds_bytes;
    uint64_t ws_bytes;
    uint64_t slab_bytes;
    int arg_kind;
    Decode3Args d3;
    Rows5Args r5;
    const void* fn_bias = nullptr;
    const void* bias_of = nullptr;
    const uint16_t* bias = nullptr;
    const void* fn_group = nullptr;
    const void* fn_bias_group = nullptr;
};

}
```

include/gemlite_hip.h:

```cpp
#ifndef GEMLITE_HIP_H
#define GEMLITE_HIP_H

#include <stddef.h>
#include <stdint.h>

#ifdef __cplusplus
extern "C" {
#endif

#define GEMLITE_HIP_ABI_VERSION 1

typedef enum gemlite_dtype_t {
    GEMLITE_DT_FP32 = 0,
    GEMLITE_DT_FP16 = 1,
    GEMLITE_DT_BF16 = 2,
    GEMLITE_DT_FP8E4 = 3,
    GEMLITE_DT_INT8 = 4,
    GEMLITE_DT_UINT8 = 5,
    GEMLITE_DT_INT32 = 6,
    GEMLITE_DT_UINT32 = 7,
    GEMLITE_DT_FP8E5 = 8,
    GEMLITE_DT_INT16 = 9,
    GEMLITE_DT_UINT16 = 10,
    GEMLITE_DT_INT64 = 11,
    GEMLITE_DT_FP8E4NUZ = 12,
    GEMLITE_DT_FP8E5NUZ = 13,
    GEMLITE_DT_MXFP16 = 14,
    GEMLITE_DT_MXBF16 = 15,
    GEMLITE_DT_MXFP8 = 16,
    GEMLITE_DT_MXFP4 = 17,
    GEMLITE_DT_NVFP4 = 18,
    GEMLITE_DT_E8M0 = 19
} gemlite_dtype_t;

typedef enum gemlite_matmul_type_t {
    GEMLITE_MATMUL_AUTO = -1,
    GEMLITE_MATMUL_GEMV = 0,
    GEMLITE_MATMUL_GEMV_REVSPLITK = 1,
    GEMLITE_MATMUL_GEMV_SPLITK = 2,
    GEMLITE_MATMUL_GEMM_SPLITK = 3,
    GEMLITE_MATMUL_GEMM = 4
} gemlite_matmul_type_t;

typedef enum gemlite_status_t {
    GEMLITE_OK = 0,
    GEMLITE_ERR_BAD_ARGUMENT = -1,
    GEMLITE_ERR_UNSUPPORTED = -2,
    GEMLITE_ERR_BAD_SHAPE = -3,
    GEMLITE_ERR_WORKSPACE = -4,
    GEMLITE_ERR_LAUNCH = -5,
    GEMLITE_ERR_NO_DEVICE = -6,
    GEMLITE_ERR_NO_FUSED_QUANT = -7
} gemlite_status_t;

typedef struct gemlite_hip_forward_args {
    uint32_t struct_size;
    int32_t matmul_type;

    const void* x;
    const void* w_q;
    const void* scales;
    const void* zeros;
    const void* scales_x;
    void* out;
    void* workspace;
    uint64_t workspace_bytes;

    int64_t M, N, K;

    int32_t W_nbits;
    int32_t group_size;
    int32_t unpack_mask;
    int32_t elements_per_sample;
    int32_t w_pack_bits;
    int32_t w_dtype;

    int32_t input_dtype;
    int32_t output_dtype;
    int32_t acc_dtype;
    int32_t meta_dtype;
    int32_t zeros_dtype;

    int32_t channel_scale_mode;
    int32_t W_group_mode;
    int32_t zero_is_scalar;
    int32_t data_contiguous;
    int32_t type_id;

    int64_t stride_xm, stride_xk;
    int64_t stride_wk, stride_wn;
    int64_t stride_om, stride_on;
    int64_t stride_meta_g, stride_meta_n;
    int64_t stride_sx_m;

    int32_t tuning[4];
} gemlite_hip_forward_args;

enum gemlite_hip_tuning0 {
    GEMLITE_T0_AUTO = 0,
    GEMLITE_T0_GEMV_TILE16 = 2, GEMLITE_T0_GEMV_TILE32 = 3, GEMLITE_T0_GEMV_TILE64 = 4,
    GEMLITE_T0_MFMA_GEMV_TILE16 = 21, GEMLITE_T0_MFMA_GEMV_TILE32 = 22, GEMLITE_T0_MFMA_GEMV_TILE64 = 24,
    GEMLITE_T0_FEWROWS_TILE16 = 1, GEMLITE_T0_FEWROWS_TILE32 = 2, GEMLITE_T0_FEWROWS_TILE64 = 4, GEMLITE_T0_FEWROWS_USE_TILES = 3,
    GEMLITE_T0_ROWS_KERNEL = 9,
    GEMLITE_T0_TILED_STREAM = 1, GEMLITE_T0_TILED_ROUND1 = 2,
    GEMLITE_T0_A8W8_STREAM = 1, GEMLITE_T0_A8W8_ROUND1 = 2, GEMLITE_T0_A8W8_ROWS = 4, GEMLITE_T0_A8W8_SQ64 = 5, GEMLITE_T0_A8W8_ROUND3 = 6,
    GEMLITE_T0_A8W8_M1_ROUND2 = 7, GEMLITE_T0_A8W8_M1_DECODE_FP8_WIDE = 8, GEMLITE_T0_A8W8_SQ128 = 10,
    GEMLITE_T0_MX_COVERAGE = 1, GEMLITE_T0_MX_TILES = 2, GEMLITE_T0_MX_TILES_256 = 3, GEMLITE_T0_MX_ROWS = 4, GEMLITE_T0_MX_STREAM = 5, GEMLITE_T0_MX_SQ64 = 6,
    GEMLITE_T0_A8WN_ROWS = 4, GEMLITE_T0_A8WN_GEMV = 7, GEMLITE_T0_A16W8_ROWS = 4, GEMLITE_T0_A16W8_STREAM = 7
};
enum gemlite_hip_tuning2 {
    GEMLITE_T2_AUTO = 0,
    GEMLITE_T2_ROWS32 = 1, GEMLITE_T2_ROWS64 = 2, GEMLITE_T2_ROWS128 = 4, GEMLITE_T2_ROWS256 = 8,
    GEMLITE_T2_WIDE_128x256 = 20, GEMLITE_T2_WIDE_256x256 = 24,
    GEMLITE_T2_NARROW_64x64 = 32, GEMLITE_T2_NARROW_64x64_K512 = 33, GEMLITE_T2_NARROW_128x64 = 34, GEMLITE_T2_NARROW_128x64_RING6 = 35,
    GEMLITE_T2_GEMV_8WAVES_2ROWS = 82, GEMLITE_T2_GEMV_4WAVES_8ROWS = 48
};
enum gemlite_hip_tuning_flags {
    GEMLITE_TF_GEMV_X_THROUGH_LDS = 1, GEMLITE_TF_GEMV_X_DIRECT = 2,
    GEMLITE_TF_GEMV_X_MODE_MASK = 3,
    GEMLITE_TF_MX_GEMV_WAVES_MASK = 3, GEMLITE_TF_MX_GEMV_4_WAVES = 1, GEMLITE_TF_MX_GEMV_16_WAVES = 2,
    GEMLITE_TF_TILED_SETPRIO = 1,
    GEMLITE_TF_TIMELINE = 4,
    GEMLITE_TF_XCD_SLICE_MAP = 8,
    GEMLITE_TF_GEMV_ROUND2_KERNEL = 16, GEMLITE_TF_GEMV_DEFAULT_POLICY_LOADS = 32,
    GEMLITE_TF_MX_PLAIN_TILE_ORDER = 16,
    GEMLITE_TF_A8W8_WEIGHTS_FROM_MEMORY = 64,
    GEMLITE_TF_COMBINE_TICKET = 128, GEMLITE_TF_COMBINE_HANDOVER_TEST = 256,
    GEMLITE_TF_NO_MFMA_GEMV = 512, GEMLITE_TF_FORCE_MFMA_GEMV = 1024,
    GEMLITE_TF_COMBINE_REDUCE_SCATTER_2 = 2048,
    GEMLITE_TF_GEMV_ROUND3_DECODE = 4096,
    GEMLITE_TF_NO_NARROW_TILES = 16384,
    GEMLITE_TF_MX_NO_SLICE_RULE = 16384,
    GEMLITE_TF_QUANT_NO_PRODUCER_TEST = 32768,
    GEMLITE_TF_NO_ROWS_KERNEL = 65536,
    GEMLITE_TF_WORDS_AS_REGISTER_LOADS = 131072,
    GEMLITE_TF_ROUND5_TILE_EPILOGUE = 262144,
    GEMLITE_TF_W8_ROWS_X_FROM_REGISTERS = 524288,
    GEMLITE_TF_W8_ROWS_LDS_BELOW_4_ROWS = 1048576,
    GEMLITE_TF_A8W8_TILE_REQUESTS_FIRST = 2097152,
    GEMLITE_TF_NO_K_ROTATION = 4194304,
    GEMLITE_TF_K_ORDER_GROUP_MASK = 0x0F000000,
    GEMLITE_TF_PUBLIC_MASK = 0x0FFFDFFF
};

int gemlite_hip_abi_version(void);
const char* gemlite_hip_build_info(void);
const char* gemlite_hip_status_string(int status);
int gemlite_hip_last_hip_error(void);

int gemlite_hip_query(const gemlite_hip_forward_args* args);

uint64_t gemlite_hip_workspace_bytes(const gemlite_hip_forward_args* args);

int gemlite_hip_forward(const gemlite_hip_forward_args* args, void* stream);

const char* gemlite_hip_kernel_name(const gemlite_hip_forward_args* args);

void gemlite_hip_set_profile_events(void* start_event, void* stop_event);

int gemlite_hip_launch_noop(int32_t blocks, int32_t threads, void* stream);

int gemlite_hip_capture_group_max(void);
void gemlite_hip_capture_group_stats(uint64_t* seen, uint64_t* joined);
int gemlite_hip_capture_group_compatible(const gemlite_hip_forward_args* a, const gemlite_hip_forward_args* b);
int gemlite_hip_capture_group_grid_y(int32_t tiles, int32_t members);
void gemlite_hip_capture_group_wave_split(int32_t layers_in_block, int32_t wave, int32_t out[3]);
int gemlite_hip_capture_group_last_form(void);
int gemlite_hip_capture_group_form(int32_t members, int32_t same_x, int64_t K);
int64_t gemlite_hip_capture_group_shared_x_lds_bytes(int64_t K);
int gemlite_hip_capture_group_geometry(int32_t tiles, int32_t members, int32_t resident, int32_t tb_want, int32_t span_want, int32_t out[4]);
int gemlite_hip_capture_group_tile_of(int32_t tiles, int32_t tb, int32_t span, int32_t block);

typedef struct gemlite_hip_forward_ext {
    uint32_t struct_size;
    int32_t bias_dtype;
    const void* bias;
} gemlite_hip_forward_ext;
#define GEMLITE_BIAS_NOT_ADDED 1
int gemlite_hip_forward_ex(const gemlite_hip_forward_args* args, const gemlite_hip_forward_ext* ext, void* stream);
int gemlite_hip_bias_fused(const gemlite_hip_forward_args* args, const gemlite_hip_forward_ext* ext);
const char* gemlite_hip_kernel_name_ex(const gemlite_hip_forward_args* args, const gemlite_hip_forward_ext* ext);
int gemlite_hip_capture_group_compatible_ex(const gemlite_hip_forward_args* a, const gemlite_hip_forward_ext* ea,
                                             const gemlite_hip_forward_args* b, const gemlite_hip_forward_ext* eb);

int gemlite_hip_scale_activations_per_token(const void* x, void* y, float* scales, int64_t M,
                                            int64_t K, int64_t stride_xm, int32_t in_dtype,
                                            int32_t out_dtype, void* stream);

int gemlite_hip_scale_activations_mxfp8(const void* x, void* y, uint8_t* scales, int64_t M, int64_t K,
                                        int64_t stride_xm, int32_t in_dtype, void* stream);
int gemlite_hip_scale_activations_mxfp4(const void* x, uint8_t* y, uint8_t* scales, int64_t M, int64_t K,
                                        int64_t stride_xm, int32_t in_dtype, void* stream);
int gemlite_hip_scale_activations_nvfp4(const void* x, uint8_t* y, uint8_t* scales, int64_t M, int64_t K,
                                        int64_t stride_xm, int32_t in_dtype, void* stream);

int gemlite_hip_pack_over_cols(const uint8_t* w_q, void* out, int64_t N, int64_t K, int64_t ld_in,
                               int32_t W_nbits, int32_t pack_bits, void* stream);
int gemlite_hip_unpack_over_cols(const void* packed, uint8_t* out, int64_t N, int64_t K,
                                 int32_t W_nbits, int32_t pack_bits, void* stream);

typedef struct gemlite_hip_quantize_args {
    uint32_t struct_size;
    int32_t w_dtype;
    const void* w;
    int64_t N, K, ld_w;
    int32_t W_nbits;
    int32_t group_size;
    int32_t pack_bits;
    int32_t meta_dtype;
    void* q_out;
    int64_t ld_q;
    void* scales;
    void* zeros;
    int64_t stride_meta_g, stride_meta_n;
    int32_t fold_zeros;
    int32_t reserved;
} gemlite_hip_quantize_args;
int gemlite_hip_quantize_groups(const gemlite_hip_quantize_args* args, void* stream);

typedef struct gemlite_hip_quantize_hqq_args {
    uint32_t struct_size;
    int32_t iters;
    gemlite_hip_quantize_args q;
    float lp_norm, beta, kappa;
    int32_t reserved;
} gemlite_hip_quantize_hqq_args;
int gemlite_hip_quantize_groups_hqq(const gemlite_hip_quantize_hqq_args* args, void* stream);

typedef struct gemlite_hip_quantize_mx_args {
    uint32_t struct_size;
    int32_t w_dtype;
    const void* w;
    int64_t N, K, ld_w;
    int32_t format;
    int32_t pack_nibbles;
    void* q_out;
    int64_t ld_q;
    void* scales;
    int64_t stride_scale_g, stride_scale_n;
    int64_t reserved;
} gemlite_hip_quantize_mx_args;
int gemlite_hip_quantize_mx(const gemlite_hip_quantize_mx_args* args, void* stream);

typedef struct gemlite_hip_dequantize_args {
    uint32_t struct_size;
    int32_t out_dtype;
    const void* w_q;
    const void* scales;
    const void* zeros;
    void* out;
    int64_t N, K;
    int64_t stride_wk, stride_wn;
    int64_t stride_meta_g, stride_meta_n;
    int64_t ld_out;
    int32_t W_nbits, group_size, elements_per_sample, w_pack_bits, w_dtype;
    int32_t input_dtype;
    int32_t meta_dtype, zeros_dtype, zero_is_scalar;
    int32_t W_group_mode, channel_scale_mode;
    float post_scale;
    int64_t reserved;
} gemlite_hip_dequantize_args;
int gemlite_hip_dequantize(const gemlite_hip_dequantize_args* args, void* stream);

#define GEMLITE_QUANT_ROWS_WAVE_MAX_K 1024
#define GEMLITE_QUANT_ROWS_RESIDENT_MAX_K 16384
typedef struct gemlite_hip_quantize_rows_args {
    uint32_t struct_size;
    int32_t w_dtype;
    const void* w;
    int64_t N, K, ld_w;
    int32_t format;
    int32_t scale_rule;
    void* q_out;
    int64_t ld_q;
    void* scales;
    int64_t stride_s;
    int32_t scale_dtype;
    int32_t reserved;
} gemlite_hip_quantize_rows_args;
int gemlite_hip_quantize_rows(const gemlite_hip_quantize_rows_args* args, void* stream);

#ifdef __cplusplus
}
#endif
#endif
```

Baseline: 4404 GB/s.

## Split each grouped decode wave across multiple tiles with K-pass interleaving

Adds a 'lines' parameter (H=1/2/4) to the captured-group W4 decode GEMV. Each wave now covers H tiles at once, with lane sub-groups per tile, and walks K in H passes per chunk so fewer waves cover the same work. Kernels are templated on the line count, and a default heuristic picks H from the tiles-per-block and layers-per-block geometry, with an env override. The aim is better load balance and memory-level parallelism per wave in the cache-cold grouped replay. The cost is narrower per-tile loads per lane and more complex index math.

```diff
diff --git a/gemlite_amd/_hip.py b/gemlite_amd/_hip.py
--- a/gemlite_amd/_hip.py
+++ b/gemlite_amd/_hip.py
@@ -236,6 +236,10 @@
         lib.gemlite_hip_capture_group_geometry.argtypes = [C.c_int32, C.c_int32, C.c_int32, C.c_int32, C.c_int32, C.POINTER(C.c_int32 * 4)]
         lib.gemlite_hip_capture_group_tile_of.restype = C.c_int
         lib.gemlite_hip_capture_group_tile_of.argtypes = [C.c_int32, C.c_int32, C.c_int32, C.c_int32]
+        lib.gemlite_hip_capture_group_lines.restype = C.c_int
+        lib.gemlite_hip_capture_group_lines.argtypes = [C.c_int32, C.c_int32, C.c_int32, C.c_int32, C.c_int32]
+        lib.gemlite_hip_capture_group_last_lines.restype = C.c_int
+        lib.gemlite_hip_capture_group_last_lines.argtypes = []
         lib.gemlite_hip_capture_group_form.restype = C.c_int
         lib.gemlite_hip_capture_group_form.argtypes = [C.c_int32, C.c_int32, C.c_int64]
         lib.gemlite_hip_capture_group_shared_x_lds_bytes.restype = C.c_int64
@@ -290,6 +294,7 @@
     "gemlite_hip_capture_group_grid_y", "gemlite_hip_capture_group_wave_split",
     "gemlite_hip_capture_group_last_form", "gemlite_hip_capture_group_form", "gemlite_hip_capture_group_shared_x_lds_bytes",
     "gemlite_hip_capture_group_geometry", "gemlite_hip_capture_group_tile_of",
+    "gemlite_hip_capture_group_lines", "gemlite_hip_capture_group_last_lines",
     "gemlite_hip_forward_ex", "gemlite_hip_bias_fused", "gemlite_hip_kernel_name_ex", "gemlite_hip_capture_group_compatible_ex",
     "gemlite_hip_quantize_groups", "gemlite_hip_quantize_mx", "gemlite_hip_dequantize", "gemlite_hip_quantize_groups_hqq",
     "gemlite_hip_quantize_rows",
diff --git a/gemlite_amd/csrc/api.hip b/gemlite_amd/csrc/api.hip
--- a/gemlite_amd/csrc/api.hip
+++ b/gemlite_amd/csrc/api.hip
@@ -61,6 +61,8 @@
 bool capture_group_try_join(const gemlite_hip_forward_args& a, const LaunchPlan& lp, hipStream_t st, int resident, int dev);
 bool capture_group_shared_x_enabled();
 int capture_group_last_form();
+int capture_group_last_lines();
+int capture_group_lines_wanted(int tiles, int members, int resident, int tb);
 Decode3TilesWanted capture_group_tiles_wanted(int tiles, int members, int resident);
 int ensure_lds(const void* fn, size_t lds, int dev);
 void capture_group_note_launch(const gemlite_hip_forward_args& a, const LaunchPlan& lp, hipStream_t st);
@@ -821,6 +823,15 @@
     return 0;
 }
 
+int gemlite_hip_capture_group_last_lines(void) { return capture_group_last_lines(); }
+
+int gemlite_hip_capture_group_lines(int32_t tiles, int32_t members, int32_t resident, int32_t tb, int32_t h_want) {
+    if (tiles < 1 || members < 1 || members > DECODE3_GMAX || resident < 1 || (tb != 1 && tb != 2 && tb != 4) || tiles % tb || h_want < 0 ||
+        h_want > 4 || h_want == 3)
+        return -1;
+    return decode3_group_lines(tb, h_want == 0 ? capture_group_lines_wanted(tiles, members, resident, tb) : h_want);
+}
+
 int gemlite_hip_capture_group_tile_of(int32_t tiles, int32_t tb, int32_t span, int32_t block) {
     if (tiles < 1 || (tb != 1 && tb != 2 && tb != 4) || tiles % tb || block < 0 || block >= tiles / tb) return -1;
     return decode3_group_first_tile(block, tiles / tb, tb, span != 0, (tiles & 15) == 0);
diff --git a/gemlite_amd/csrc/capture_group.hip b/gemlite_amd/csrc/capture_group.hip
--- a/gemlite_amd/csrc/capture_group.hip
+++ b/gemlite_amd/csrc/capture_group.hip
@@ -7,10 +7,10 @@
 namespace gl {
 
 const void* gemv_w4_decode3_fn(int tag, bool nt);
-const void* gemv_w4_decode3_group_fn(int tag);
+const void* gemv_w4_decode3_group_fn(int tag, int h);
 const void* gemv_w4_decode3_bias_fn(int tag, bool nt);
-const void* gemv_w4_decode3_bias_group_fn(int tag);
-const void* gemv_w4_decode3_group_sx_fn(int tag, bool biased);
+const void* gemv_w4_decode3_bias_group_fn(int tag, int h);
+const void* gemv_w4_decode3_group_sx_fn(int tag, bool biased, int h);
 int ensure_lds(const void* fn, size_t lds, int dev);
 
 namespace {
@@ -76,21 +76,21 @@
     return lp.bias ? (lp.fn == lp.fn_bias ? lp.fn_bias_group : nullptr) : (lp.fn == lp.bias_of ? lp.fn_group : nullptr);
 }
 
-const void* group_fn_of(const void* fn) {
+const void* group_fn_of(const void* fn, int h = 1) {
     for (int tag = 0; tag < 2; ++tag)
         for (int nt = 0; nt < 2; ++nt)
-            if (fn == gemv_w4_decode3_fn(tag, nt != 0)) return gemv_w4_decode3_group_fn(tag);
+            if (fn == gemv_w4_decode3_fn(tag, nt != 0)) return gemv_w4_decode3_group_fn(tag, h);
     for (int tag = 0; tag < 2; ++tag)
         for (int nt = 0; nt < 2; ++nt)
-            if (fn == gemv_w4_decode3_bias_fn(tag, nt != 0)) return gemv_w4_decode3_bias_group_fn(tag);
+            if (fn == gemv_w4_decode3_bias_fn(tag, nt != 0)) return gemv_w4_decode3_bias_group_fn(tag, h);
     return nullptr;
 }
 
-const void* group_sx_fn_of(const void* fn) {
+const void* group_sx_fn_of(const void* fn, int h = 1) {
     for (int tag = 0; tag < 2; ++tag)
         for (int nt = 0; nt < 2; ++nt) {
-            if (fn == gemv_w4_decode3_fn(tag, nt != 0)) return gemv_w4_decode3_group_sx_fn(tag, false);
-            if (fn == gemv_w4_decode3_bias_fn(tag, nt != 0)) return gemv_w4_decode3_group_sx_fn(tag, true);
+            if (fn == gemv_w4_decode3_fn(tag, nt != 0)) return gemv_w4_decode3_group_sx_fn(tag, false, h);
+            if (fn == gemv_w4_decode3_bias_fn(tag, nt != 0)) return gemv_w4_decode3_group_sx_fn(tag, true, h);
         }
     return nullptr;
 }
@@ -121,6 +121,7 @@
 };
 thread_local Group tl_group;
 thread_local int tl_last_form = 0;
+thread_local int tl_last_lines = 0;
 
 bool capture_state(hipStream_t st, unsigned long long* id, hipGraph_t* graph, hipGraphNode_t* only_dep) {
     hipStreamCaptureStatus status = hipStreamCaptureStatusNone;
@@ -167,7 +168,16 @@
     return forced.tb ? forced : decode3_group_tiles_default(tiles, members, resident);
 }
 
+int capture_group_lines_wanted(int tiles, int members, int resident, int tb) {
+    static const int forced = [] {
+        const int h = env_int("GEMLITE_HIP_CAPTURE_GROUP_LINES", 0);
+        return h >= 4 ? 4 : (h >= 2 ? 2 : (h == 1 ? 1 : 0));
+    }();
+    return forced ? forced : decode3_group_lines_default(tiles, members, resident, tb);
+}
+
 int capture_group_last_form() { return tl_last_form; }
+int capture_group_last_lines() { return tl_last_lines; }
 
 void capture_group_stats(uint64_t* seen, uint64_t* joined) {
     if (seen) *seen = g_seen.load(std::memory_order_relaxed);
@@ -226,6 +236,7 @@
         }
         g.fp[g.members++] = fb;
         tl_last_form = 3;
+        tl_last_lines = 0;
         g_joined.fetch_add(1, std::memory_order_relaxed);
         return true;
     }
@@ -236,16 +247,19 @@
     const int members = g.members + 1, tiles = (int)g.lp.grid.x;
     const Decode3TilesWanted want = capture_group_tiles_wanted(tiles, members, resident);
     const Decode3GroupGeometry geo = decode3_group_geometry(tiles, members, resident, want.tb, want.span);
+    const int lines = decode3_group_lines(geo.tb, capture_group_lines_wanted(tiles, members, resident, geo.tb));
     uint32_t modes = decode3_group_modes(d.modes, members, geo.grid_y, geo.tb, geo.span);
+    const void* fn_g = group_fn_of(g.lp.fn, lines);
+    const void* fn_sx = g.fn_group_sx ? group_sx_fn_of(g.lp.fn, lines) : nullptr;
     void* kargs[] = {(void*)&d.w, (void*)&d.x, (void*)&d.s, (void*)&d.z, (void*)&d.out, (void*)&d.sw4, (void*)&d.mstride2,
                      (void*)&d.nch_total, (void*)&modes, biased ? (void*)&g.tabb : (void*)&g.tab};
     const bool same_x = g.same_x && lp.d3.x == d.x;
     int form = decode3_group_form(members, same_x, d.nch_total, capture_group_shared_x_enabled() && g.fn_group_sx != nullptr);
     const size_t lds = form == 2 ? (size_t)decode3_shared_x_lds_bytes(d.nch_total) : 0;
-    if (form == 2 && ensure_lds(g.fn_group_sx, (size_t)DECODE3_SHARED_X_MAX_LDS, dev) != GEMLITE_OK) form = 1;
+    if (form == 2 && ensure_lds(fn_sx, (size_t)DECODE3_SHARED_X_MAX_LDS, dev) != GEMLITE_OK) form = 1;
     hipKernelNodeParams np;
     memset(&np, 0, sizeof(np));
-    np.func = (void*)(form == 2 ? g.fn_group_sx : g.fn_group);
+    np.func = (void*)(form == 2 ? fn_sx : fn_g);
     np.gridDim = dim3((unsigned)geo.grid_x, (unsigned)geo.grid_y, 1);
     np.blockDim = g.lp.block;
     np.sharedMemBytes = form == 2 ? (unsigned)lds : 0;
@@ -259,6 +273,7 @@
     g.fp[g.members++] = fb;
     g.same_x = same_x;
     tl_last_form = form;
+    tl_last_lines = lines;
     g_joined.fetch_add(1, std::memory_order_relaxed);
     return true;
 }
@@ -285,6 +300,7 @@
     g.fn_group_sx = lp.arg_kind == 1 ? group_sx_fn_of(lp.fn) : nullptr;
     g.same_x = true;
     tl_last_form = 0;
+    tl_last_lines = 0;
     memset(&g.tab, 0, sizeof(g.tab));
     memset(&g.tabb, 0, sizeof(g.tabb));
     g.tabb.bias[0] = lp.bias;
diff --git a/gemlite_amd/csrc/gemv_decode.hip b/gemlite_amd/csrc/gemv_decode.hip
--- a/gemlite_amd/csrc/gemv_decode.hip
+++ b/gemlite_amd/csrc/gemv_decode.hip
@@ -27,8 +27,15 @@
 
 }
 
-template <typename Tail>
+template <typename T>
+__device__ __forceinline__ const T& decode3_table(const T& t) { return t; }
+template <typename T, int HL>
+__device__ __forceinline__ const T& decode3_table(const Decode3Lines<T, HL>& w) { return w.t; }
+
+template <typename TailArg>
 struct Decode3TailKind {
+    using Tail = typename Decode3LinesOf<TailArg>::table;
+    static constexpr int hl = Decode3LinesOf<TailArg>::hl;
     static constexpr bool shared_x = std::is_same<Tail, Decode3GroupTableSX>::value || std::is_same<Tail, Decode3BiasGroupTableSX>::value;
     static constexpr bool grouped = std::is_same<Tail, Decode3GroupTable>::value || std::is_same<Tail, Decode3BiasGroupTable>::value || shared_x;
     static constexpr bool biased = std::is_same<Tail, Decode3BiasTail>::value || std::is_same<Tail, Decode3BiasGroupTable>::value ||
@@ -54,16 +61,17 @@
     const int c = lane & 3, g = lane >> 2;
     int tile = blockIdx.x;
     [[maybe_unused]] int g_members = 0, g_Y = 1, g_slots = 1, g_tbl = 0, g_tile0 = 0;
+    [[maybe_unused]] constexpr int g_hl = Decode3TailKind<Tail>::hl;
     [[maybe_unused]] Decode3WaveSplit g_split{0, 0, 16};
     if constexpr (GROUPED) {
         g_members = (int)((modes >> 16) & DECODE3_M_MEMBERS);
         g_Y = (int)(modes >> 24);
         g_tbl = (int)((modes >> DECODE3_M_TB_SHIFT) & 3u);
         g_slots = ((g_members - (int)blockIdx.y + g_Y - 1) / g_Y) << g_tbl;
-        g_split = decode3_wave_split(g_slots, wave);
+        g_split = decode3_wave_split(g_slots >> g_hl, wave);
         const bool span = (modes & DECODE3_M_SPAN) != 0u;
         g_tile0 = decode3_group_first_tile(tile, span ? (int)gridDim.x : 0, 1 << g_tbl, span, (modes & M_PAIR) != 0u);
-        tile = g_tile0 + ((g_split.layer < 0 ? 0 : g_split.layer) & ((1 << g_tbl) - 1));
+        tile = g_tile0 + ((((g_split.layer < 0 ? 0 : g_split.layer) << g_hl) & ((1 << g_tbl) - 1)) + (lane >> (6 - g_hl)));
     } else if (modes & M_PAIR) {
         const int xcd = tile & 7, idx = tile >> 3;
         tile = (((idx >> 1) << 3) + xcd) * 2 + (idx & 1);
@@ -224,22 +232,26 @@
     } else {
         const int Y = g_Y, y = (int)blockIdx.y, slots = g_slots;
         const Decode3WaveSplit split = g_split;
-        const int slot = split.layer < 0 ? 0 : split.layer, li = slot >> g_tbl, v0 = split.v0, v1 = split.v1;
+        constexpr int hl = g_hl, H = 1 << hl;
+        const int lq = lane & ((64 >> hl) - 1), gl = lq >> 2;
+        const int slot = (split.layer < 0 ? 0 : split.layer) << hl, li = slot >> g_tbl, v0 = split.v0, v1 = split.v1;
         const int L = y + li * Y;
         const char *w_ = wb, *x_ = xb, *s_ = sp, *z_ = zp;
         if (L > 0) {
-            const Decode3Member& m = counters.m[L - 1];
+            const Decode3Member& m = decode3_table(counters).m[L - 1];
             w_ = m.w; x_ = m.x; s_ = m.s; z_ = m.z;
         }
         if (modes & M_ZSCALAR) scalar_zero = (float)((const int32_t*)z_)[0];
-        const uint32_t vw0 = (uint32_t)(g * R) * sw4 + n0 * 4u, vw1 = vw0 + sw4, vx = (uint32_t)lane * 8u;
-        const uint32_t vm = (gs_shift < 8 ? (uint32_t)(g * R * 8) >> gs_shift : 0u) * mstride2 + n0 * 2u;
+        const uint32_t vw0 = (uint32_t)(gl * R) * sw4 + n0 * 4u, vw1 = vw0 + sw4, vx = (uint32_t)lq * 8u;
+        const uint32_t vm = (gs_shift < 8 ? (uint32_t)(gl * R * 8) >> gs_shift : 0u) * mstride2 + n0 * 2u;
+        const uint32_t pass_w = (uint32_t)(CHUNK >> hl) * sw4, pass_x = (uint32_t)(CHUNK * 16) >> hl;
+        const int pass_ms = gs_shift < 8 ? gs_shift : 31;
         const uint32_t vs = need_s ? vm : 0u, vz = need_z ? vm : 0u, ms_s = need_s ? mstride2 : 0u, ms_z = need_z ? mstride2 : 0u;
         const char *sb = need_s ? s_ : w_, *zb = need_z ? z_ : w_;
         const int shl = gs_shift < 8 ? 8 - gs_shift : 0, shr = gs_shift > 8 ? gs_shift - 8 : 0;
         const uint32_t chunk_w = (uint32_t)CHUNK * sw4;
         const int nv = v1 - v0, rem = (nch_total & (NW - 1)) - v0;
-        const int n = (nch_total / NW) * nv + (rem < 0 ? 0 : (rem > nv ? nv : rem));
+        const int n = ((nch_total / NW) * nv + (rem < 0 ? 0 : (rem > nv ? nv : rem))) << hl;
         float* redg;
         uint32_t* xpairs = nullptr;
         float* xsums = nullptr;
@@ -252,27 +264,31 @@
         } else {
             redg = red;
         }
-        float* rd = redg + slot * RED;
+        float* rd = redg + ((slot + (lane >> (6 - hl))) * RED + (lq >> 4) * TC + c * 4);
 
         constexpr int NLC = SX ? 4 : 5;
-        int rv = v0, rgc = v0;
+        int rv = v0, rp = 0, rgc = v0;
         auto request = [&](Chunk& ck, int ri) __attribute__((always_inline)) {
 #if GL_DECODE3_ABLATION == 2
-            const int keep = rgc;
-            if (ri >= 2) rgc = v0;
-#endif
-            const char* wq = w_ + (uint32_t)rgc * chunk_w;
+            const int keep = rgc, keep_p = rp;
+            if (ri >= 2) { rgc = v0; rp = 0; }
+#endif
+            const char* wq = w_ + ((uint32_t)rgc * chunk_w + (uint32_t)rp * pass_w);
             gvw::gld128<NT>(ck.w[0], wq, vw0);
             gvw::gld128<NT>(ck.w[1], wq, vw1);
-            if constexpr (!SX) gvw::gld64(ck.xq, x_ + (uint32_t)rgc * (uint32_t)(CHUNK * 16), vx);
-            const uint32_t grp = ((uint32_t)rgc << shl) >> shr;
+            if constexpr (!SX) gvw::gld64(ck.xq, x_ + ((uint32_t)rgc * (uint32_t)(CHUNK * 16) + (uint32_t)rp * pass_x), vx);
+            const uint32_t grp = (((uint32_t)rgc << shl) >> shr) + (((uint32_t)rp << (8 - hl)) >> pass_ms);
             gvw::gld64(ck.s, sb + grp * ms_s, vs);
             gvw::gld64(ck.z, zb + grp * ms_z, vz);
 #if GL_DECODE3_ABLATION == 2
             rgc = keep;
+            rp = keep_p;
 #endif
             rgc += NW;
-            if (rgc >= nch_total) rgc = ++rv;
+            if (rgc >= nch_total) {
+                if (++rp == H) { rp = 0; ++rv; }
+                rgc = rv;
+            }
         };
         auto tie_chunk = [&](Chunk& ck) __attribute__((always_inline)) {
             gvw::tie(ck.w[0]);
@@ -281,7 +297,7 @@
             gvw::tie(ck.s);
             gvw::tie(ck.z);
         };
-        auto flush = [&](int v) {
+        auto flush = [&](int v, int p) {
 #pragma unroll
             for (int j = 0; j < 4; ++j) {
                 float t = tot[j];
@@ -289,11 +305,11 @@
                 t += dpp_movf<0x128>(t);
                 tot[j] = t;
             }
-            if ((lane & 12) == 0) *(f32x4*)(rd + ((v * 4 + (lane >> 4)) * TC + c * 4)) = (f32x4){tot[0], tot[1], tot[2], tot[3]};
+            if ((lane & 12) == 0) *(f32x4*)(rd + (v * 4 + (p << (2 - hl))) * TC) = (f32x4){tot[0], tot[1], tot[2], tot[3]};
 #pragma unroll
             for (int j = 0; j < 4; ++j) tot[j] = 0.f;
         };
-        int cv = v0, cgc = v0;
+        int cv = v0, cp = 0, cgc = v0;
         auto stage_unit = [&](int u, const u32x4& lo, const u32x4& hi) __attribute__((always_inline)) {
             u32x4 pr[R];
             float xsum = 0.f;
@@ -315,8 +331,8 @@
         };
         auto stage_off = [&](int u) { return (uint32_t)(u < units ? u : units - 1) * 32u; };
         constexpr int STRIPS = (int)((DECODE3_SHARED_X_MAX_UNITS + 1023) / 1024);
-        const uint32_t* xp_lane = xpairs + g * 8;
-        const float* xs_lane = xsums + g;
+        const uint32_t* xp_lane = xpairs + gl * 8;
+        const float* xs_lane = xsums + gl;
         auto run = [&](auto full) {
             Chunk A, B;
             if constexpr (SX) {
@@ -349,10 +365,11 @@
             }
             gvw::ring2_run_pre<NLC>(n, A, B, request, tie_chunk, [&](int) __attribute__((always_inline)) {
                 if constexpr (SX) {
-                    const uint32_t* xp = xp_lane + cgc * 128;
+                    const int unit = cgc * 16 + (cp << (4 - hl));
+                    const uint32_t* xp = xp_lane + unit * 8;
                     xs.p[0] = *(const u32x4*)xp;
                     xs.p[1] = *(const u32x4*)(xp + 4);
-                    xs.sum = xs_lane[cgc * 16];
+                    xs.sum = xs_lane[unit];
                 }
             }, [&](const Chunk& ck, int) __attribute__((always_inline)) {
 #if GL_DECODE3_ABLATION == 1
@@ -366,15 +383,17 @@
 #endif
                 cgc += NW;
                 if (cgc >= nch_total) {
-                    flush(cv);
-                    cgc = ++cv;
+                    flush(cv, cp);
+                    if (++cp == H) { cp = 0; ++cv; }
+                    cgc = cv;
                 }
             });
         };
         if (need_s && need_z) run(std::true_type{}); else run(std::false_type{});
         if (split.layer >= 0) {
 #pragma unroll 1
-            for (int v = cv; v < v1; ++v) flush(v);
+            for (int v = cv; v < v1; ++v)
+                for (int p = 0; p < H; ++p) flush(v, p);
         }
 
         const bool fin = wave < slots;
@@ -383,9 +402,9 @@
         uint16_t braw = 0;
         if (fin) {
             const int Lf = y + (wave >> g_tbl) * Y;
-            if (Lf > 0) o_ = counters.m[Lf - 1].out;
+            if (Lf > 0) o_ = decode3_table(counters).m[Lf - 1].out;
             if constexpr (BIASED) {
-                if (lane < 16) braw = counters.bias[Lf][ftile * TC + lane];
+                if (lane < 16) braw = decode3_table(counters).bias[Lf][ftile * TC + lane];
             }
         }
         __syncthreads();
@@ -412,21 +431,22 @@
     return (const void*)k;
 }
 
-const void* gemv_w4_decode3_group_fn(int tag) {
-    typedef void (*kfn)(const char*, const char*, const char*, const char*, uint16_t*, uint32_t, uint32_t, int, uint32_t, const Decode3GroupTable);
-    kfn k = tag == 0 ? gemv_w4_decode3_kernel<half_tag, false, Decode3GroupTable> : gemv_w4_decode3_kernel<bf16_tag, false, Decode3GroupTable>;
+template <typename Table, int HL>
+static const void* decode3_group_fn_of(int tag) {
+    using Tail = typename std::conditional<HL == 0, Table, Decode3Lines<Table, HL>>::type;
+    typedef void (*kfn)(const char*, const char*, const char*, const char*, uint16_t*, uint32_t, uint32_t, int, uint32_t, const Tail);
+    kfn k = tag == 0 ? gemv_w4_decode3_kernel<half_tag, false, Tail> : gemv_w4_decode3_kernel<bf16_tag, false, Tail>;
     return (const void*)k;
 }
-
-const void* gemv_w4_decode3_group_sx_fn(int tag, bool biased) {
-    typedef void (*kfn)(const char*, const char*, const char*, const char*, uint16_t*, uint32_t, uint32_t, int, uint32_t, const Decode3GroupTableSX);
-    typedef void (*kfnb)(const char*, const char*, const char*, const char*, uint16_t*, uint32_t, uint32_t, int, uint32_t, const Decode3BiasGroupTableSX);
-    if (biased) {
-        kfnb k = tag == 0 ? gemv_w4_decode3_kernel<half_tag, false, Decode3BiasGroupTableSX> : gemv_w4_decode3_kernel<bf16_tag, false, Decode3BiasGroupTableSX>;
-        return (const void*)k;
-    }
-    kfn k = tag == 0 ? gemv_w4_decode3_kernel<half_tag, false, Decode3GroupTableSX> : gemv_w4_decode3_kernel<bf16_tag, false, Decode3GroupTableSX>;
-    return (const void*)k;
+template <typename Table>
+static const void* decode3_group_fn_of(int tag, int h) {
+    return h == 4 ? decode3_group_fn_of<Table, 2>(tag) : (h == 2 ? decode3_group_fn_of<Table, 1>(tag) : decode3_group_fn_of<Table, 0>(tag));
+}
+
+const void* gemv_w4_decode3_group_fn(int tag, int h) { return decode3_group_fn_of<Decode3GroupTable>(tag, h); }
+
+const void* gemv_w4_decode3_group_sx_fn(int tag, bool biased, int h) {
+    return biased ? decode3_group_fn_of<Decode3BiasGroupTableSX>(tag, h) : decode3_group_fn_of<Decode3GroupTableSX>(tag, h);
 }
 
 const void* gemv_w4_decode3_bias_fn(int tag, bool nt) {
@@ -436,10 +456,6 @@
     return (const void*)k;
 }
 
-const void* gemv_w4_decode3_bias_group_fn(int tag) {
-    typedef void (*kfn)(const char*, const char*, const char*, const char*, uint16_t*, uint32_t, uint32_t, int, uint32_t, const Decode3BiasGroupTable);
-    kfn k = tag == 0 ? gemv_w4_decode3_kernel<half_tag, false, Decode3BiasGroupTable> : gemv_w4_decode3_kernel<bf16_tag, false, Decode3BiasGroupTable>;
-    return (const void*)k;
-}
-
-}
+const void* gemv_w4_decode3_bias_group_fn(int tag, int h) { return decode3_group_fn_of<Decode3BiasGroupTable>(tag, h); }
+
+}
diff --git a/gemlite_amd/csrc/gl_common.h b/gemlite_amd/csrc/gl_common.h
--- a/gemlite_amd/csrc/gl_common.h
+++ b/gemlite_amd/csrc/gl_common.h
@@ -524,6 +524,20 @@
     Decode3Member m[DECODE3_GMAX - 1];
     const uint16_t* bias[DECODE3_GMAX];
 };
+template <typename Table, int HL>
+struct Decode3Lines {
+    Table t;
+};
+template <typename T>
+struct Decode3LinesOf {
+    using table = T;
+    static constexpr int hl = 0;
+};
+template <typename T, int HL>
+struct Decode3LinesOf<Decode3Lines<T, HL>> {
+    using table = T;
+    static constexpr int hl = HL;
+};
 constexpr int64_t DECODE3_RED_BYTES = (int64_t)DECODE3_GMAX * 16 * 4 * 16 * 4, DECODE3_LDS_LIMIT = 160 * 1024;
 constexpr int64_t DECODE3_SHARED_X_MAX_UNITS = ((DECODE3_LDS_LIMIT - DECODE3_RED_BYTES) / 36) & ~(int64_t)15;
 constexpr int64_t DECODE3_SHARED_X_MAX_LDS = DECODE3_RED_BYTES + DECODE3_SHARED_X_MAX_UNITS * 36;
@@ -574,6 +588,17 @@
         grp = (((idx >> 1) << 3) + xcd) * 2 + (idx & 1);
     }
     return grp * tb;
+}
+GL_HD int decode3_group_lines(int tb, int h_want) {
+    int h = h_want >= 4 ? 4 : (h_want >= 2 ? 2 : 1);
+    while (h > tb) h >>= 1;
+    return h;
+}
+inline int decode3_group_lines_default(int tiles, int members, int64_t resident, int tb) {
+    if (tb < 2) return 1;
+    const Decode3GroupGeometry geo = decode3_group_geometry(tiles, members, resident, tb, false);
+    const int lb = (members + geo.grid_y - 1) / geo.grid_y;
+    return (geo.tb == 4 && lb >= 4) ? 4 : 2;
 }
 struct Decode3TilesWanted {
     int tb;
diff --git a/include/gemlite_hip.h b/include/gemlite_hip.h
--- a/include/gemlite_hip.h
+++ b/include/gemlite_hip.h
@@ -170,6 +170,8 @@
 int64_t gemlite_hip_capture_group_shared_x_lds_bytes(int64_t K);
 int gemlite_hip_capture_group_geometry(int32_t tiles, int32_t members, int32_t resident, int32_t tb_want, int32_t span_want, int32_t out[4]);
 int gemlite_hip_capture_group_tile_of(int32_t tiles, int32_t tb, int32_t span, int32_t block);
+int gemlite_hip_capture_group_lines(int32_t tiles, int32_t members, int32_t resident, int32_t tb, int32_t h_want);
+int gemlite_hip_capture_group_last_lines(void);
 
 typedef struct gemlite_hip_forward_ext {
     uint32_t struct_size;
```

Result: faster. 4761 GB/s, median of 6 (+8.1%).
